# pedrosecchi67/ImmersedBoundary.jl

Measured on AMD Instinct MI355X. Metric: Mcells*iters/s residual sweep (advection-JST-MUSCL), 2D RAE2822, higher is better.
Workload: dtype f32

## Files before the change

### immersedboundary.jl_amd/_lib.py

```python
import ctypes as C
import os

_here = os.path.dirname(os.path.abspath(__file__))
LIB_PATH = os.environ.get("IBHIP_LIB") or os.path.join(_here, "libibhip.so")

c_i32p = C.POINTER(C.c_int32)
c_f32p = C.POINTER(C.c_float)
c_vp = C.c_void_p
c_i64 = C.c_int64
c_int = C.c_int


class IbhError(RuntimeError):
    pass


class ibh_fluid(C.Structure):
    _fields_ = [("R", C.c_float), ("gamma", C.c_float), ("mu_ref", C.c_float), ("Tref", C.c_float),
                ("S", C.c_float), ("nk", C.c_int32), ("k", C.c_float * 4)]


class ibh_flow_bc_spec(C.Structure):
    _fields_ = [("normal_flow", C.c_int32), ("p_inf", C.c_float), ("T_inf", C.c_float), ("u_inf", C.c_float * 3),
                ("transpiration", C.c_float), ("wall_function", C.c_int32), ("wall_params", C.c_float * 8),
                ("n_iter", C.c_int32)]


_SIGS = {
    "ibh_init": [c_int],
    "ibh_set_stream": [c_vp],
    "ibh_sync": [],
    "ibh_version": [],
    "ibh_malloc": [C.POINTER(c_vp), C.c_size_t],
    "ibh_free": [c_vp],
    "ibh_h2d": [c_vp, c_vp, C.c_size_t],
    "ibh_d2h": [c_vp, c_vp, C.c_size_t],
    "ibh_memset": [c_vp, c_int, C.c_size_t],
    "ibh_owned_device_memory": [C.POINTER(c_i64), C.POINTER(c_i64)],
    "ibh_partition_create": [C.POINTER(c_vp), c_int, C.c_int32, c_vp, c_vp, c_vp,
                             C.POINTER(c_vp), C.POINTER(c_vp), C.POINTER(c_vp), C.POINTER(c_vp),
                             C.POINTER(c_vp), C.POINTER(c_vp), C.c_int32, c_vp, c_vp, c_int, c_int],
    "ibh_partition_destroy": [c_vp],
    "ibh_partition_info": [c_vp, C.POINTER(c_i64), c_int],
    "ibh_analyze2_host": [C.POINTER(c_vp), C.c_int32, c_vp, c_vp, C.POINTER(c_vp), C.POINTER(c_vp), C.POINTER(c_vp),
                          C.POINTER(c_vp), C.POINTER(c_vp), C.POINTER(c_vp), C.c_int32, c_vp, c_vp, c_int],
    "ibh_host2d_get": [c_vp, c_int, c_int, c_vp, c_i64, C.POINTER(c_i64)],
    "ibh_host2d_destroy": [c_vp],
    "ibh_at_owners": [c_vp, c_int, c_vp, c_int, c_i64, c_vp, c_i64],
    "ibh_at_neighbors": [c_vp, c_int, c_vp, c_int, c_i64, c_vp, c_i64],
    "ibh_at_faces": [c_vp, c_int, c_vp, c_int, c_i64, c_vp, c_i64],
    "ibh_green_gauss": [c_vp, c_int, c_vp, c_int, c_i64, c_vp, c_i64, c_int],
    "ibh_cell_gradient": [c_vp, c_int, c_vp, c_int, c_i64, c_vp, c_i64],
    "ibh_cell_gradient_all": [c_vp, c_vp, c_int, c_i64, c_vp, c_i64],
    "ibh_cell_gradient_nd": [c_vp, c_vp, c_int, c_i64, c_vp, c_i64, c_vp, c_i64],
    "ibh_cell_gradient_fields": [c_vp, c_vp, c_int, c_i64, c_vp],
    "ibh_face_distance": [c_vp, c_int, c_vp],
    "ibh_owner_distance": [c_vp, c_int, c_vp],
    "ibh_neighbor_distance": [c_vp, c_int, c_vp],
    "ibh_face_gradient": [c_vp, c_int, c_vp, c_int, c_i64, c_vp, c_i64],
    "ibh_jst_sensor": [c_vp, c_int, c_vp, c_int, c_i64, c_vp, c_i64],
    "ibh_muscl": [c_vp, c_int, c_vp, c_vp, c_int, c_i64, c_vp, c_int, c_vp, c_vp, c_i64],
    "ibh_acc_create": [C.POINTER(c_vp), C.c_int32, C.c_int32, c_vp, c_vp, c_vp, c_int],
    "ibh_acc_destroy": [c_vp],
    "ibh_accumulate": [c_vp, c_vp, c_int, c_i64, c_vp, c_i64],
    "ibh_accumulate_diff_add": [c_vp, c_vp, c_vp, c_int, c_i64, c_vp, c_i64],
    "ibh_bc_create": [C.POINTER(c_vp), C.c_int32, c_vp, c_vp, c_vp, C.c_int32, c_vp, c_vp, c_vp, c_vp, c_int],
    "ibh_bc_destroy": [c_vp],
    "ibh_bc_interp": [c_vp, c_vp, c_int, c_i64, c_vp, c_i64],
    "ibh_bc_blend": [c_vp, c_vp, c_int, c_i64, c_vp, c_i64, c_vp, c_i64, c_vp],
    "ibh_bc_apply": [c_vp, c_vp, c_int, c_i64, c_int, c_vp],
    "ibh_bc_flow_info": [c_vp, C.POINTER(C.c_int32)],
    "ibh_bc_flow": [c_vp, C.POINTER(ibh_fluid), c_int, c_vp, c_i64, c_vp, c_vp, c_i64, C.POINTER(ibh_flow_bc_spec), c_int,
                    C.POINTER(c_vp), c_vp, c_vp, c_vp],
    "ibh_gather_rows": [c_vp, C.c_int32, c_vp, c_int, c_i64, c_vp, c_i64],
    "ibh_scatter_rows": [c_vp, C.c_int32, c_vp, c_int, c_i64, c_vp, c_i64],
    "ibh_copy_rows": [c_vp, c_vp, C.c_int32, c_vp, c_int, c_i64, c_vp, c_i64],
    "ibh_residual_advection": [c_vp, c_vp, c_vp, c_i64, c_vp, c_int],
    "ibh_residual_advection_n": [c_vp, c_vp, c_vp, c_i64, c_vp, c_int, c_int],
    "ibh_shear_rate_of_velocity": [c_vp, c_vp, c_i64, c_vp],
    "ibh_shear_rate_of_velocity_grad": [c_vp, c_vp, c_i64, c_vp, c_vp, c_i64],
    "ibh_wray_agarwal_of": [c_vp, c_vp, c_vp, C.c_float, C.c_float, C.c_float, c_vp, c_vp, c_vp],
    "ibh_les_of": [c_vp, c_vp, c_i64, c_vp, c_int, C.c_float, c_vp, c_vp, c_vp, c_vp, c_vp, c_i64],
    "ibh_k_epsilon_rhs": [c_vp, c_vp, c_i64, c_vp, c_vp, C.c_float, c_vp, c_vp, c_vp, c_vp, c_vp, c_vp, c_i64],
    "ibh_scalar_transport": [c_vp, c_vp, c_vp, C.c_float, c_vp, c_i64, c_vp, c_vp],
    "ibh_bcset_create": [C.POINTER(c_vp), c_int, C.POINTER(c_vp), c_vp, c_vp],
    "ibh_bcset_destroy": [c_vp],
    "ibh_bcset_info": [c_vp, C.POINTER(C.c_int32), C.POINTER(C.c_int32)],
    "ibh_bcset_apply": [c_vp, c_vp],
    "ibh_timestep_advection": [c_vp, c_vp, c_i64, C.c_float, c_vp],
    "ibh_update_dev": [c_i64, c_vp, c_vp, c_vp, c_vp],
    "ibh_step_advection": [c_vp, c_vp, c_vp, c_vp, c_i64, c_vp, c_vp],
    "ibh_step_advection_dt": [c_vp, c_vp, c_vp, c_vp, c_i64, c_vp, c_vp, C.c_float, c_vp],
    "ibh_timestep_euler": [c_vp, C.POINTER(ibh_fluid), c_vp, c_i64, C.c_float, c_vp, c_vp],
    "ibh_update_euler": [C.POINTER(ibh_fluid), c_int, c_i64, c_vp, c_i64, c_vp, c_i64, c_vp, c_int, c_vp, c_i64],
    "ibh_step_euler": [c_vp, C.POINTER(ibh_fluid), c_int, c_vp, c_i64, c_vp, c_i64, c_vp, c_int, c_vp, c_i64, c_int],
    "ibh_update_euler_stage": [C.POINTER(ibh_fluid), c_int, c_i64, c_vp, c_i64, c_vp, c_i64, c_vp, c_int, C.c_float, c_vp,
                               c_i64],
    "ibh_stage_euler": [c_vp, C.POINTER(ibh_fluid), c_int, c_vp, c_i64, c_vp, c_i64, c_vp, c_i64, c_vp, c_int, C.c_float,
                        c_vp, c_i64, c_int],
    "ibh_update_euler_ssp": [C.POINTER(ibh_fluid), c_int, c_i64, c_vp, c_i64, c_vp, c_i64, c_vp, c_i64, c_vp, c_int, C.c_float,
                             C.c_float, C.c_float, c_vp, c_i64],
    "ibh_stage_euler_ssp": [c_vp, C.POINTER(ibh_fluid), c_int, c_vp, c_i64, c_vp, c_i64, c_vp, c_i64, c_vp, c_int, C.c_float,
                            C.c_float, C.c_float, c_vp, c_i64, c_int],
    "ibh_dual_source": [C.POINTER(ibh_fluid), c_int, c_i64, c_vp, c_i64, c_vp, c_i64, C.c_float, C.c_float, c_vp, c_i64],
    "ibh_update_euler_dual": [C.POINTER(ibh_fluid), c_int, c_i64, c_vp, c_i64, c_vp, c_i64, c_vp, c_i64, c_vp, c_int, C.c_float,
                              C.c_float, c_vp, c_i64],
    "ibh_stage_euler_dual": [c_vp, C.POINTER(ibh_fluid), c_int, c_vp, c_i64, c_vp, c_i64, c_vp, c_i64, c_vp, c_i64, c_vp, c_int,
                             C.c_float, C.c_float, c_vp, c_i64, c_int],
    "ibh_restrict_euler": [c_vp, C.POINTER(ibh_fluid), c_int, c_vp, c_i64, c_vp, c_i64, c_vp, c_i64, c_vp, c_i64, c_vp, c_i64],
    "ibh_prolong_euler": [c_vp, C.POINTER(ibh_fluid), c_int, c_vp, c_vp, c_i64, c_vp, c_vp, c_i64, c_vp, c_i64],
    "ibh_restrict_euler_roles": [c_vp, C.POINTER(ibh_fluid), c_int, c_vp, c_i64, c_vp, c_i64, c_vp, c_i64, c_vp, c_vp, c_i64,
                                 c_vp, c_i64],
    "ibh_forcing_roles": [c_i64, c_int, c_vp, c_i64, c_vp, c_i64, c_vp],
    "ibh_sumsq_roles": [c_i64, c_int, c_vp, c_i64, c_vp, c_vp],
    "ibh_smooth_residual": [c_vp, c_vp, c_int, c_i64, C.c_float, c_int, c_vp, c_i64, c_vp, c_i64],
    "ibh_update_euler_smoothed": [c_vp, C.POINTER(ibh_fluid), c_int, c_vp, c_i64, c_vp, c_i64, c_vp, c_i64, c_vp, c_i64,
                                  C.c_float, c_vp, c_int, C.c_float, C.c_float, C.c_float, c_vp, c_i64],
    "ibh_ew_binary": [c_int, c_i64, c_int, c_vp, c_int, C.c_float, c_vp, c_int, C.c_float, c_vp],
    "ibh_ew_unary": [c_int, c_i64, c_vp, c_vp],
    "ibh_ew_fill": [c_i64, C.c_float, c_vp],
    "ibh_ew_reduce": [c_int, c_i64, c_vp, c_vp],
    "ibh_ew_eval": [c_i64, c_int, c_int, c_vp, c_int, c_vp, c_vp, c_int, c_vp, c_vp],
    "ibh_ew_reduce_rows": [c_i64, c_int, c_vp, c_vp],
    "ibh_set_tuning": [C.c_char_p, c_int],
    "ibh_debug_buffer": [c_vp],
    "ibh_probe_dispatch": [c_int, c_int, c_int],
    "ibh_probe_sweep": [c_vp, c_vp, c_vp, c_i64, c_vp, c_int],
    "ibh_residual_euler_hll": [c_vp, c_vp, c_i64, c_vp, c_i64, C.POINTER(ibh_fluid), c_int],
    "ibh_residual_euler_sensor": [c_vp, c_vp, c_i64, c_vp, c_vp, c_i64, C.POINTER(ibh_fluid), c_int],
    "ibh_cfd_speed_of_sound": [C.POINTER(ibh_fluid), c_i64, c_vp, c_vp],
    "ibh_cfd_dynamic_viscosity": [C.POINTER(ibh_fluid), c_i64, c_vp, c_vp],
    "ibh_cfd_heat_conductivity": [C.POINTER(ibh_fluid), c_i64, c_vp, c_vp],
    "ibh_cfd_primitive2state": [C.POINTER(ibh_fluid), c_int, c_i64, c_vp, c_i64, c_vp, c_i64],
    "ibh_cfd_state2primitive": [C.POINTER(ibh_fluid), c_int, c_i64, c_vp, c_i64, c_vp, c_i64],
    "ibh_cfd_inviscid_fluxes_hll": [C.POINTER(ibh_fluid), c_int, c_int, c_i64, c_vp, c_vp, c_i64, c_vp, c_i64],
    "ibh_cfd_inviscid_fluxes_sensor": [C.POINTER(ibh_fluid), c_int, c_int, c_i64, c_vp, c_vp, c_i64, c_vp, c_vp,
                                       c_vp, c_i64],
    "ibh_cfd_jst_sensor3": [c_i64, c_vp, c_vp, c_vp, c_vp],
    "ibh_cfd_shock_sensor": [c_int, c_i64, C.POINTER(c_vp), c_vp],
    "ibh_cfd_viscous_fluxes": [C.POINTER(ibh_fluid), c_int, c_int, c_i64, c_vp, c_i64, C.POINTER(c_vp), c_i64, c_vp,
                               C.c_float, c_vp, c_i64],
    "ibh_viscous_residual": [c_vp, C.POINTER(ibh_fluid), c_vp, c_i64, C.POINTER(c_vp), c_i64, c_int, c_vp, c_vp, c_i64],
    "ibh_cfd_flow_bc": [C.POINTER(ibh_fluid), c_int, c_i64, c_vp, c_i64, c_vp, c_i64, C.c_float, C.c_float, c_vp, c_int,
                        c_vp, c_vp, C.c_float, c_vp, c_vp, c_i64],
    "ibh_ipc_alloc": [C.POINTER(c_vp), C.c_size_t, c_int],
    "ibh_ipc_free": [c_vp],
    "ibh_ipc_export": [c_vp, c_vp],
    "ibh_ipc_import": [c_vp, C.POINTER(c_vp)],
    "ibh_ipc_close": [c_vp],
    "ibh_flag_signal": [c_vp, c_vp, c_int],
    "ibh_flag_wait": [c_vp, c_vp, c_int, C.c_uint32, c_vp],
    "ibh_halo_push": [c_vp, c_int, c_i64, c_vp, c_int, c_vp, c_vp, c_vp, c_vp],
    "ibh_halo_pull": [c_vp, c_int, c_i64, c_vp, c_vp, c_int, c_vp, c_vp, c_vp, C.c_uint32],
    "ibh_halo_exchange": [c_vp, c_int, c_i64, c_vp, c_int, c_vp, c_vp, c_vp, c_vp, c_vp, c_vp, c_vp, c_int, c_vp, c_vp,
                          c_vp, C.c_uint32],
    "ibh_step_advection_xgmi": [c_vp, c_vp, c_vp, c_i64, c_vp, c_vp, c_int, c_vp, c_vp, c_vp, c_vp, c_vp, c_vp, c_vp, c_int,
                                c_vp, c_vp, c_vp, C.c_uint32, c_vp],
    "ibh_axpy_clamped": [c_i64, C.c_float, c_vp, c_vp],
    "ibh_axpy_clamped_sumsq": [c_i64, C.c_float, c_vp, c_vp, c_vp],
    "ibh_fas_update": [c_i64, C.c_float, c_vp, c_vp, c_vp, c_vp],
    "ibh_axpy": [c_i64, C.c_float, c_vp, c_vp],
    "ibh_sumsq": [c_i64, c_vp, c_vp],
    "ibh_time_average_push": [c_i64, c_int, c_vp, c_i64, c_vp, c_vp, c_int, c_vp, c_i64, c_i64, C.c_double, C.c_double,
                              c_int],
    "ibh_domain_plan_create": [C.POINTER(c_vp), c_int, C.POINTER(c_vp), c_vp, C.POINTER(c_vp), C.POINTER(c_vp), c_vp,
                               c_i64, c_int],
    "ibh_domain_plan_destroy": [c_vp],
    "ibh_domain_plan_info": [c_vp, C.POINTER(c_i64), c_int],
    "ibh_domain_gather": [c_vp, c_int, C.POINTER(c_vp), c_vp, c_vp, C.POINTER(c_vp)],
    "ibh_domain_scatter": [c_vp, c_int, C.POINTER(c_vp), c_vp, c_vp, C.POINTER(c_vp)],
    "ibh_turb_wall_function_rey": [c_i64, c_vp, c_vp, c_int, c_vp, c_vp, c_vp, c_vp, c_vp],
    "ibh_turb_wall_function": [c_i64, c_vp, c_vp, c_vp, c_vp, c_int, c_vp, c_vp, c_vp, c_vp, c_vp, c_vp],
    "ibh_turb_shear_rate": [c_int, c_i64, c_vp, c_vp],
    "ibh_turb_smagorinsky": [c_i64, c_vp, c_vp, C.c_float, c_vp],
    "ibh_turb_k_epsilon": [c_i64, c_vp, c_vp, c_vp, c_vp, c_vp, c_vp, c_vp, c_vp, c_vp],
    "ibh_turb_wray_agarwal": [c_int, c_i64, c_vp, c_vp, c_vp, c_i64, c_vp, c_i64, C.c_float, C.c_float, C.c_float, c_vp,
                              c_vp, c_vp],
    "ibh_turb_ducros": [c_int, c_i64, c_vp, c_vp],
    "ibh_turb_wale": [c_i64, c_vp, c_vp, C.c_float, c_vp],
    "ibh_pi_rademacher": [c_i64, C.c_uint64, c_vp],
    "ibh_pi_perturb": [c_i64, c_vp, c_vp, C.c_float, c_vp],
    "ibh_pi_fd": [c_i64, c_vp, c_vp, C.c_float, c_vp],
    "ibh_pi_hutch_accum": [c_i64, c_int, c_vp, c_vp, c_vp, C.c_float, c_vp],
    "ibh_pi_div_scalar": [c_i64, C.c_float, c_vp],
    "ibh_pi_invert_blocks": [c_i64, c_int, c_vp],
    "ibh_pi_apply_blocks": [c_i64, c_int, c_vp, c_vp, c_vp],
    "ibh_dot": [c_i64, c_vp, c_vp, c_vp],
    "ibh_maxabs": [c_i64, c_vp, c_vp],
    "ibh_pi_update": [c_i64, c_vp, C.c_float, c_vp, c_vp, c_vp, c_vp],
    "ibh_pi_normalize": [c_i64, c_vp, c_vp, C.c_float, c_vp],
}

EXPORTS = sorted(list(_SIGS) + ["ibh_last_error"])

_lib = None


def load():
    global _lib
    if _lib is not None:
# ... 28 lines not shown
```

### immersedboundary.jl_amd/backend.py

```python
from __future__ import annotations

import ctypes as C

import numpy as np
import torch

from . import _lib
from ._lib import call, c_vp
from .accumulator import Accumulator
from .domain import Boundary, Partition, Surface

IBH_FORCE_GENERAL = 1
IBH_IMAGE_ONLY = 2
IBH_PASS_A_ONLY = 4
IBH_PASS_B_ONLY = 8
IBH_EXACT = 16
IBH_PHASE_INTERIOR = 32
IBH_PHASE_BOUNDARY = 64
IBH_NO_FUSE = 128
IBH_SWEEP_ONLY = 256
IBH_FORCE_MIXED = 512
IBH_NO_QUAD = 1024

_initialised = {}
# ... 37 lines not shown

def colmajor_empty(n, nv=None, dtype=torch.float32):
    dev = _dev()
    if nv is None:
        return torch.empty(n, dtype=dtype, device=dev)
    return torch.empty((nv, n), dtype=dtype, device=dev).T


def hip(a):
    dev = _dev()
    if isinstance(a, torch.Tensor):
        a = a.detach().cpu().numpy()
    a = np.asarray(a)
    if a.dtype == np.float64:
        a = a.astype(np.float32)
    if a.ndim == 1:
        return torch.from_numpy(np.ascontiguousarray(a)).to(dev)
    if a.ndim == 2:
        return torch.from_numpy(np.ascontiguousarray(a.T)).to(dev).T
    raise ValueError("hip(): only 1-D and 2-D fields are supported")


def to_host(t):
    if not isinstance(t, torch.Tensor):
        t = t.t
    return np.ascontiguousarray(t.detach().cpu().numpy())


def _hipaware(fn):
    import functools

    H = {}

    @functools.wraps(fn)
    def wrapper(*args, **kwargs):
        if not H:
            from . import hiparray
            H["A"], H["rewrap"] = hiparray.HipArray, hiparray.rewrap
        HipArray = H["A"]
        hit = False

        def un(x):
            nonlocal hit
            if isinstance(x, HipArray):
                hit = True
                return x.t
            if isinstance(x, tuple):
                return tuple(un(v) for v in x)
            return x
        if kwargs and isinstance(kwargs.get("out"), HipArray):
            kwargs["out"]._flush_readers()
        a = [un(x) for x in args]
        k = {key: un(v) for key, v in kwargs.items()} if kwargs else kwargs
        out = fn(*a, **k)
        return H["rewrap"](out, True) if hit else out
    return wrapper


def _field(t, n=None):
    if not isinstance(t, torch.Tensor) or not t.is_cuda:
        raise TypeError("expected a device array (convert with ibamd.hip); there is no CPU path")
    if t.dtype != torch.float32:
        raise TypeError("fields must be Float32")
    if t.ndim == 1:
        if t.stride(0) != 1:
            t = t.contiguous()
        nv, ld = 1, t.shape[0]
    elif t.ndim == 2:
        if t.stride(0) != 1 or (t.shape[1] > 1 and t.stride(1) < t.shape[0]):
            t = t.T.contiguous().T
        nv, ld = t.shape[1], (t.stride(1) if t.shape[1] > 1 else t.shape[0])
    else:
        raise ValueError("fields are (n,) or (n, nv)")
    if n is not None and t.shape[0] != n:
        raise ValueError(f"field has {t.shape[0]} rows, expected {n}")
    return t, nv, ld


def _field_inplace(t, n=None, what="destination"):
    f, nv, ld = _field(t, n)
    if f.data_ptr() != t.data_ptr() or f.stride() != t.stride():
        raise TypeError(f"{what} must be a column-major Float32 device array (cell index fastest, e.g. ibamd.hip(a) or "
                        f"colmajor_empty(n, nv)); got strides {tuple(t.stride())} for shape {tuple(t.shape)}: it would "
                        "be copied and the update lost")
    return f, nv, ld


def _like(t, n):
    return colmajor_empty(n) if t.ndim == 1 else colmajor_empty(n, t.shape[1])


class _Handle:
    _destroy = None
    handle = None

    def __del__(self):
        try:
            if self.handle:
                h, self.handle = self.handle, None
                getattr(_lib.load(), self._destroy)(h)
        except Exception:
            pass


class DevicePartition(_Handle):
    _destroy = "ibh_partition_destroy"

    def __init__(self, part: Partition):
        dev = _dev()
        self.host = part
        self.id = part.id
        self.nd = part.ndims
        self.nc = part.spacing.shape[0]
        nd, nc = self.nd, self.nc
        spacing = np.asfortranarray(part.spacing, dtype=np.float32)
        centers = np.asfortranarray(part.centers, dtype=np.float32)
        self.nf = [int(part.face_owners_neighbors[d + 1][0].shape[0]) for d in range(nd)]
        nf = np.array(self.nf, dtype=np.int32)
        keep = []

        def parr(arrs):
            arrs = [np.ascontiguousarray(a, dtype=np.int32) for a in arrs]
            keep.append(arrs)
            return (c_vp * nd)(*[a.ctypes.data for a in arrs])

        owners = parr([part.face_owners_neighbors[d + 1][0] for d in range(nd)])
        neighbors = parr([part.face_owners_neighbors[d + 1][1] for d in range(nd)])
        loff = parr([part.face_accumulators[(d + 1, False)].off for d in range(nd)])
        lidx = parr([part.face_accumulators[(d + 1, False)].idx for d in range(nd)])
        roff = parr([part.face_accumulators[(d + 1, True)].off for d in range(nd)])
        ridx = parr([part.face_accumulators[(d + 1, True)].idx for d in range(nd)])
        iid = np.ascontiguousarray(part.image_in_domain, dtype=np.int32)
        dom = np.ascontiguousarray(part.domain, dtype=np.int32)
        h = c_vp()
        call("ibh_partition_create", C.byref(h), nd, nc, spacing.ctypes.data_as(c_vp), centers.ctypes.data_as(c_vp),
             nf.ctypes.data_as(c_vp), owners, neighbors, loff, lidx, roff, ridx, int(iid.size), _hptr(iid),
             _hptr(dom), int(getattr(part, "block_size", 0)), 0)
        self.handle = h
        self.spacing = hip(part.spacing)
        self.centers = hip(part.centers)
        self.domain = torch.from_numpy(dom).to(dev)
        self.image = torch.from_numpy(np.ascontiguousarray(part.image, dtype=np.int32)).to(dev)
        self.image_in_domain = torch.from_numpy(iid).to(dev)
        info = (C.c_int64 * 24)()
        call("ibh_partition_info", h, info, 24)
        self.info = dict(full_blocks=info[0], irregular_cells=info[1], sides_same=info[2], sides_mirror=info[3],
                         sides_coarse=info[4], sides_fine=info[5], sides_general=info[6], interior_blocks=info[7],
                         fusable_blocks=info[8], workspace_blocks=info[9],
                         image_blocks_all_eligible=bool(info[10]), image_blocks=info[11],
                         quads=info[12] if self.nd == 2 else 0, quad_singles=info[13], image_quads=info[14],
                         image_quad_singles=info[15], row_sweep=bool(info[16]), direct_sides=info[17],
                         quad_pairs=info[18] if self.nd == 2 else 0,
                         quad_arith_half_sides=info[19] if self.nd == 2 else 0,
                         tiled=bool(info[20]),
                         rim4_rows=info[12] if self.nd == 3 else 0)

    @property
    def ndims(self):
        return self.nd


class DeviceAccumulator(_Handle):
    _destroy = "ibh_acc_destroy"

    def __init__(self, acc: Accumulator):
        _dev()
        self.n_output, self.n_input = acc.n_output, acc.n_input
        self.first_index = acc.first_index
        h = c_vp()
        w = None if acc.w is None else np.ascontiguousarray(acc.w, dtype=np.float32)
        call("ibh_acc_create", C.byref(h), acc.n_output, acc.n_input, _hptr(acc.off), _hptr(acc.idx),
             _hptr(w) if w is not None else c_vp(None), 0)
        self.handle = h

    def __call__(self, v):
        from .hiparray import HipArray
        if isinstance(v, HipArray):
            return HipArray(self(v.t))
        v, nv, ld = _field(v, self.n_input)
        out = _like(v, self.n_output)
        _stream()
        call("ibh_accumulate", self.handle, _ptr(v), nv, ld, _ptr(out), self.n_output)
        return out

    def diff_add(self, out, a, b):
        a, nv, ld = _field(a, self.n_input)
        b, nvb, ldb = _field(b, self.n_input)
        o, nvo, ldo = _field_inplace(out, self.n_output, "out")
        if nvb != nv or nvo != nv or ldb != ld:
            out += self(a - b)
            return out
        _stream()
        call("ibh_accumulate_diff_add", self.handle, _ptr(a), _ptr(b), nv, ld, _ptr(o), ldo)
        return out


class DeviceBoundary(_Handle):
    _destroy = "ibh_bc_destroy"

    def __init__(self, b: Boundary):
        self.host = b
        self.ng = int(b.ghost_indices.shape[0])
        acc = b.image_interpolator
        h = c_vp()
        gi = np.ascontiguousarray(b.ghost_indices, dtype=np.int32)
        idm = np.ascontiguousarray(b.image_domain, dtype=np.int32)
        gd = np.ascontiguousarray(b.ghost_distances, dtype=np.float32)
        idist = np.ascontiguousarray(b.image_distances, dtype=np.float32)
        _dev()
        call("ibh_bc_create", C.byref(h), self.ng, _hptr(gi), _hptr(gd), _hptr(idist), int(idm.size), _hptr(idm),
             _hptr(acc.off), _hptr(acc.idx), _hptr(np.ascontiguousarray(acc.w, dtype=np.float32)), 0)
        self.handle = h
        self.ghost_indices = torch.from_numpy(gi).to(_dev())
        self.projections = hip(b.projections)
        self.normals = hip(b.normals)
        self.image_distances = hip(b.image_distances)
        self.ghost_distances = hip(b.ghost_distances)


class DeviceSurface:

    def __init__(self, s: Surface):
        self.host = s
        self.n = int(s.points.shape[0])
        self.interpolator = DeviceAccumulator(s.interpolator)
        self.offset_interpolator = DeviceAccumulator(s.offset_interpolator)
        self.points, self.normals = hip(s.points), hip(s.normals)
        self.offsets, self.areas = hip(s.offsets), hip(s.areas)

    def __call__(self, u):
        return self.interpolator(u)


def at_offset(surf, u):
    return to_backend(surf).offset_interpolator(u)


def surface_integral(surf, u):
    from .hiparray import HipArray
    surf = to_backend(surf)
    U = u if isinstance(u, HipArray) else HipArray(u)
    if U.n != surf.n:
        raise ValueError(f"field has {U.n} rows, the surface {surf.n} control points")
    prod = U * HipArray(surf.areas)
    if U.ndim == 1:
        return np.float32(prod.sum())
    return np.array([HipArray(prod.t[:, v]).sum() for v in range(U.nv)], dtype=np.float32)


def volume_integral(dom, A):
    from .hiparray import HipArray
    U = A if isinstance(A, HipArray) else HipArray(A)
    if U.n != len(dom):
        raise ValueError("volume_integral takes a global array (one row per cell of the domain)")
    wd = getattr(dom, "_device_widths", None)
    if wd is None:
        from .mesher import get_cells
        _, widths = get_cells(dom.mesh)
        wd = dom._device_widths = [HipArray(np.ascontiguousarray(widths[d], dtype=np.float32))
                                   for d in range(widths.shape[0])]
    prod = U * wd[0]
    for w in wd[1:]:
        prod *= w
    if U.ndim == 1:
        return np.float32(prod.sum())
    return np.array([HipArray(prod.t[:, v]).sum() for v in range(U.nv)], dtype=np.float32)


def to_backend(x, converter=hip):
    if isinstance(x, (DevicePartition, DeviceAccumulator, DeviceBoundary, DeviceSurface)):
        return x
    if isinstance(x, Surface):
        if getattr(x, "_device", None) is None:
            x._device = DeviceSurface(x)
        return x._device
    if isinstance(x, Partition):
        if getattr(x, "_device", None) is None:
            x._device = DevicePartition(x)
        return x._device
    if isinstance(x, Accumulator):
        if getattr(x, "_device", None) is None:
            x._device = DeviceAccumulator(x)
        return x._device
    if isinstance(x, Boundary):
        if getattr(x, "_device", None) is None:
            x._device = DeviceBoundary(x)
        return x._device
    if isinstance(x, tuple):
        return tuple(to_backend(v, converter) for v in x)
    if isinstance(x, dict):
        return {k: to_backend(v, converter) for k, v in x.items()}
    if isinstance(x, (np.ndarray, torch.Tensor)):
        return converter(x)
    return x


def _part(p):
    if not isinstance(p, DevicePartition):
        raise TypeError("operators run on a device Partition (to_backend(part, hip)); there is no CPU path")
    return p


def _cell_to_face(name, part, u, dim):
    part = _part(part)
    u, nv, ld = _field(u, part.nc)
    out = _like(u, part.nf[dim - 1])
# ... 963 lines not shown
```

### immersedboundary.jl_amd/csrc/ibh_analyze.cpp

```cpp
#include <algorithm>
#include <array>
#include <unordered_map>

#include "ibh_common.h"

namespace {

inline int pos_own(int s, int t) { return s == 0 ? 8 * t : s == 1 ? 7 + 8 * t : s == 2 ? t : t + 56; }
inline int pos_opp(int s, int tt) { return s == 0 ? 7 + 8 * tt : s == 1 ? 8 * tt : s == 2 ? tt + 56 : tt; }
inline int tang_of_pos(int s, int pos) { return s < 2 ? pos / 8 : pos % 8; }
inline bool on_opp_edge(int s, int pos) {
    return s == 0 ? (pos % 8 == 7) : s == 1 ? (pos % 8 == 0) : s == 2 ? (pos / 8 == 7) : (pos / 8 == 0);
}

}

void ibh_analyze_blocks2(const HostPartView& v, std::vector<BlockDesc2>& blocks, std::vector<int32_t>& irr,
                         int64_t* info, const int32_t* image_in_domain, int32_t n_image, int32_t* n_phase1,
                         std::vector<int32_t>& htab, std::vector<int32_t>& etab, std::vector<char>& fus,
                         std::vector<char>& needg, std::vector<int32_t>& dtab) {
    const int32_t nc = v.nc;
    const int NPB = 64;
    const float* hx = v.spacing;
    const float* hy = v.spacing + nc;
// ... 178 lines not shown
            bool ok = a1[b];
            for (int s = 0; s < 4 && ok; ++s) {
                int ty = blocks[b].type[s];
                if (ty == SIDE_MIRROR) continue;
                if (ty == SIDE_GENERAL) { ok = false; break; }
                int nn = ty == SIDE_FINE ? 2 : 1;
                for (int k = 0; k < nn && ok; ++k) {
                    auto it = base2a1.find(blocks[b].nb[s][k]);
                    ok = it != base2a1.end() && it->second;
                }
            }
            b1[b] = ok;
        }
        std::vector<BlockDesc2> ordered;
        std::vector<std::array<int32_t, 64>> hordered;
        ordered.reserve(blocks.size());
        hordered.reserve(blocks.size());
        auto take = [&](size_t b) { ordered.push_back(blocks[b]); hordered.push_back(halos[b]); };
        for (size_t b = 0; b < blocks.size(); ++b) if (b1[b]) take(b);
        n_phase1[1] = (int32_t)ordered.size();
        for (size_t b = 0; b < blocks.size(); ++b) if (a1[b] && !b1[b]) take(b);
        n_phase1[0] = (int32_t)ordered.size();
        for (size_t b = 0; b < blocks.size(); ++b) if (!a1[b]) take(b);
        blocks.swap(ordered);
        halos.swap(hordered);
    }
    htab.resize(blocks.size() * 64);
    for (size_t bi = 0; bi < blocks.size(); ++bi)
        for (int k = 0; k < 64; ++k) htab[bi * 64 + k] = halos[bi][k];
    etab.assign(blocks.size() * 16, 0);
    fus.assign(blocks.size(), 0);
    dtab.clear();
    {
        auto faces_of = [&](int32_t c, int dim, bool right, int32_t* out) -> int {
            const std::vector<int32_t>& off = right ? v.roff[dim] : v.loff[dim];
            const std::vector<int32_t>& idx = right ? v.ridx[dim] : v.lidx[dim];
            const int n = off[c + 1] - off[c];
            if (n < 1 || n > 2) return -1;
            for (int k = 0; k < n; ++k) {
                const int32_t f = idx[off[c] + k];
                const int32_t o = v.owners[dim][f], nn = v.neighbors[dim][f];
                if ((right ? o : nn) != c) return -1;
                out[k] = right ? nn : o;
            }
            return n;
        };
        int64_t nfus = 0;
        for (size_t bi = 0; bi < blocks.size(); ++bi) {
            BlockDesc2& b = blocks[bi];
            b.dt = -1;
            bool ok = true;
            for (int k = 0; k < NPB && ok; ++k) ok = !cell_irr[b.base + k];
            int32_t deep[64];
            bool arithmetic = true;
            for (int s = 0; s < 4; ++s) {
                int32_t* e = &etab[bi * 16 + s * 4];
                e[0] = e[1] = e[2] = e[3] = b.base + pos_own(s, 0);
                for (int k = 0; k < 16; ++k) deep[s * 16 + k] = halos[bi][s * 16 + k];
                if (!ok) continue;
                const int ty = b.type[s];
                if (ty == SIDE_MIRROR) continue;
                if (ty == SIDE_GENERAL) { ok = false; continue; }
                const int d = s / 2, td = 1 - d;
                const bool low = (s % 2) == 0;
                const float* hn = d == 0 ? hx : hy;
                const float* ht = d == 0 ? hy : hx;
                const float rt = b.rt[s];
                const int delta = s == 0 ? -1 : s == 1 ? 1 : s == 2 ? -8 : 8;
                const int step = ty == SIDE_FINE ? 1 : ty == SIDE_COARSE ? 4 : 2;
                const int ncell = 16 / step;
                const int near_expected = ty == SIDE_COARSE ? 2 : 1;
                for (int q = 0; q < ncell && ok; ++q) {
                    const int32_t h = halos[bi][s * 16 + q * step];
                    if (hn[h] != hn[b.base] * rt || ht[h] != ht[b.base] * rt) { ok = false; break; }
                    int32_t cells[2];
                    int n = faces_of(h, d, low, cells);
                    if (n != near_expected) { ok = false; break; }
                    for (int k = 0; k < n; ++k)
                        if (cells[k] < b.base || cells[k] >= b.base + NPB) ok = false;
                    n = faces_of(h, d, !low, cells);
                    if (!ok || n != 1 || cells[0] == h || hn[cells[0]] != hn[h]) { ok = false; break; }
                    for (int k = 0; k < step; ++k) deep[s * 16 + q * step + k] = cells[0];
                    if (cells[0] != h + delta) arithmetic = false;
                    for (int side = 0; side < 2 && ok; ++side) {
                        n = faces_of(h, td, side == 1, cells);
                        if (n < 1) { ok = false; break; }
                        const int qn = q + (side ? 1 : -1);
                        if (qn >= 0 && qn < ncell) {
                            if (n != 1 || cells[0] != halos[bi][s * 16 + qn * step]) ok = false;
                        } else {
                            e[side * 2] = cells[0];
                            e[side * 2 + 1] = n == 2 ? cells[1] : cells[0];
                        }
                    }
                }
            }
            if (ok && !arithmetic) {
                b.dt = (int32_t)(dtab.size() / 64);
                dtab.insert(dtab.end(), deep, deep + 64);
            }
            fus[bi] = ok;
            nfus += ok;
        }
        info[8] = nfus;
    }
    needg.assign(blocks.size(), 0);
    {
        std::vector<char> mark(nc, 0);
        for (int32_t c : irr) {
            mark[c] = 1;
            for (int d = 0; d < v.nd; ++d) {
                for (int32_t k = v.loff[d][c]; k < v.loff[d][c + 1]; ++k) mark[v.owners[d][v.lidx[d][k]]] = 1;
                for (int32_t k = v.roff[d][c]; k < v.roff[d][c + 1]; ++k) mark[v.neighbors[d][v.ridx[d][k]]] = 1;
            }
        }
        for (size_t bi = 0; bi < blocks.size(); ++bi)
            if (!fus[bi])
                for (int k = 0; k < 64; ++k) mark[htab[bi * 64 + k]] = 1;
        for (size_t bi = 0; bi < blocks.size(); ++bi) {
            bool need = !fus[bi];
            for (int k = 0; k < NPB && !need; ++k) need = mark[blocks[bi].base + k];
            needg[bi] = need;
        }
    }
    info[7] = n_phase1[1];
    info[0] = (int64_t)blocks.size();
    info[1] = (int64_t)irr.size();
    for (int k = 0; k < 5; ++k) info[2 + k] = counts[k];
}

static void quad_aux_row(const int32_t* row, uint32_t cls, std::vector<int32_t>& aux) {
    const size_t a0 = aux.size();
    aux.resize(a0 + IBH_QAUX);
    for (int e = 0; e < 32; ++e) aux[a0 + e] = row[128 + e];
    for (int l = 0; l < 8; ++l) {
        const int g = l >> 1, half = l & 1;
        const uint32_t ty = (cls >> (4 * l)) & 15u;
        const int stride = (g == 0 || g == 3) ? 8 : 1;
        const int32_t* ids = row + 2 * (16 * g + 8 * half);
        int32_t orig = -1;
        if (ty == SIDE_SAME || ty == SIDE_COARSE) {
            orig = ids[0];
            for (int t = 0; t < 8 && orig >= 0; ++t) {
                const int32_t want = ids[0] + stride * (ty == SIDE_COARSE ? (t >> 1) : t);
                if (ids[2 * t] != want || ids[2 * t + 1] != want) orig = -1;
            }
        }
        aux[a0 + 32 + l] = orig;
    }
}

void ibh_build_quads2(const std::vector<BlockDesc2>& blocks, const std::vector<int32_t>& htab,
                      const std::vector<int32_t>& etab, const std::vector<char>& cand, int32_t nB1, QuadSet2& out,
                      int32_t nc) {
    out = QuadSet2();
    const int32_t nb = (int32_t)blocks.size();
    std::unordered_map<int32_t, int32_t> bybase;
    bybase.reserve(nb * 2);
    for (int32_t b = 0; b < nb; ++b) bybase[blocks[b].base] = b;
    std::vector<int32_t> order(nb);
    for (int32_t b = 0; b < nb; ++b) order[b] = b;
    std::sort(order.begin(), order.end(), [&](int32_t a, int32_t b) { return blocks[a].base < blocks[b].base; });
    std::vector<char> used(nb, 0);
    struct Q { int32_t b[4]; bool interior; };
    std::vector<Q> quads;
    auto same_to = [&](const BlockDesc2& a, int s, int32_t base) {
        return a.type[s] == SIDE_SAME && a.nb[s][0] == base;
    };
    static const int outer[4][2] = {{0, 2}, {1, 2}, {0, 3}, {1, 3}};
    for (int32_t o : order) {
        if (used[o] || !cand[o]) continue;
        const BlockDesc2& b0 = blocks[o];
        int32_t idx[4] = {o, -1, -1, -1};
        bool ok = true;
        for (int k = 1; k < 4 && ok; ++k) {
            auto it = bybase.find(b0.base + 64 * k);
            ok = it != bybase.end() && !used[it->second] && cand[it->second];
            if (ok) idx[k] = it->second;
        }
        if (!ok) continue;
        const BlockDesc2 &b1 = blocks[idx[1]], &b2 = blocks[idx[2]], &b3 = blocks[idx[3]];
        ok = same_to(b0, 1, b1.base) && same_to(b1, 0, b0.base) && same_to(b0, 3, b2.base) && same_to(b2, 2, b0.base) &&
             same_to(b1, 3, b3.base) && same_to(b3, 2, b1.base) && same_to(b2, 1, b3.base) && same_to(b3, 0, b2.base);
        for (int k = 0; k < 4 && ok; ++k) {
            const BlockDesc2& b = blocks[idx[k]];
            ok = b.dt < 0 && b.h[0] == b0.h[0] && b.h[1] == b0.h[1];
            for (int e = 0; e < 2 && ok; ++e) {
                const int s = outer[k][e];
                const int ty = b.type[s];
                ok = ty == SIDE_SAME || ty == SIDE_COARSE || ty == SIDE_FINE;
                if (ok && s >= 2)
                    for (int t = 0; t < 8 && ok; ++t) {
                        const int32_t h0 = htab[(size_t)idx[k] * 64 + (s * 8 + t) * 2], h1 = htab[(size_t)idx[k] * 64 + (s * 8 + t) * 2 + 1];
                        const int32_t dl = s == 2 ? -8 : 8;
                        ok = h0 + 1 < nc && h0 + dl >= 0 && h0 + dl + 1 < nc && (ty != SIDE_FINE || h1 == h0 + 1);
                    }
            }
        }
        if (!ok) continue;
        Q q;
        q.interior = true;
        for (int k = 0; k < 4; ++k) {
            q.b[k] = idx[k];
            used[idx[k]] = 1;
            q.interior = q.interior && idx[k] < nB1;
        }
        quads.push_back(q);
    }
    static const int side_of_g[4] = {0, 2, 3, 1};
    static const int blk_of[4][2] = {{0, 2}, {0, 1}, {2, 3}, {1, 3}};
    for (int pass = 0; pass < 2; ++pass)
        for (const Q& q : quads) {
            if (q.interior != (pass == 0)) continue;
            QuadDesc2 d;
            d.base = blocks[q.b[0]].base;
            d.rh[0] = blocks[q.b[0]].rh[0];
            d.rh[1] = blocks[q.b[0]].rh[1];
            d.cls = 0;
            const size_t row = out.qtab.size();
            out.qtab.resize(row + IBH_QROW);
            for (int g = 0; g < 4; ++g)
                for (int half = 0; half < 2; ++half) {
                    const int s = side_of_g[g], l = 2 * g + half;
                    const int32_t bi = q.b[blk_of[g][half]];
                    d.cls |= (uint32_t)blocks[bi].type[s] << (4 * l);
                    for (int t = 0; t < 8; ++t)
                        for (int k = 0; k < 2; ++k)
                            out.qtab[row + 2 * (16 * g + 8 * half + t) + k] = htab[(size_t)bi * 64 + (s * 8 + t) * 2 + k];
                    for (int e = 0; e < 4; ++e) out.qtab[row + 128 + 4 * l + e] = etab[(size_t)bi * 16 + s * 4 + e];
                }
            out.qd.push_back(d);
            quad_aux_row(out.qtab.data() + row, d.cls, out.qaux);
            if (pass == 0) out.nq_int++;
        }
    for (int pass = 0; pass < 2; ++pass)
        for (int32_t b = 0; b < nb; ++b)
            if (cand[b] && !used[b] && (b < nB1) == (pass == 0)) {
                out.singles.push_back(b);
                if (pass == 0) out.ns_int++;
            }
    if (nB1 != nb) {
        out.singles2 = out.singles;
        return;
    }
    std::vector<char> paired(nb, 0);
    auto side_ok = [&](int32_t bi, int s) {
        const BlockDesc2& b = blocks[bi];
        const int ty = b.type[s];
        bool ok = ty == SIDE_SAME || ty == SIDE_COARSE || ty == SIDE_FINE;
        if (ok && s >= 2)
            for (int t = 0; t < 8 && ok; ++t) {
                const int32_t h0 = htab[(size_t)bi * 64 + (s * 8 + t) * 2], h1 = htab[(size_t)bi * 64 + (s * 8 + t) * 2 + 1];
                const int32_t dl = s == 2 ? -8 : 8;
                ok = h0 + 1 < nc && h0 + dl >= 0 && h0 + dl + 1 < nc && (ty != SIDE_FINE || h1 == h0 + 1);
            }
        return ok;
    };
    for (int32_t o : order) {
        if (used[o] || paired[o] || !cand[o]) continue;
        const BlockDesc2& b0 = blocks[o];
        auto it = bybase.find(b0.base + 64);
        if (it == bybase.end()) continue;
        const int32_t i1 = it->second;
        if (used[i1] || paired[i1] || !cand[i1]) continue;
        const BlockDesc2& b1 = blocks[i1];
        bool ok = same_to(b0, 1, b1.base) && same_to(b1, 0, b0.base) && b0.dt < 0 && b1.dt < 0 && b1.h[0] == b0.h[0] &&
                  b1.h[1] == b0.h[1];
        ok = ok && side_ok(o, 0) && side_ok(o, 2) && side_ok(o, 3) && side_ok(i1, 1) && side_ok(i1, 2) && side_ok(i1, 3);
        if (!ok) continue;
        paired[o] = paired[i1] = 1;
        const int32_t blk_of_pair[4][2] = {{o, o}, {o, i1}, {o, i1}, {i1, i1}};
        QuadDesc2 d;
        d.base = b0.base;
        d.rh[0] = b0.rh[0];
        d.rh[1] = b0.rh[1];
        d.cls = 0;
        const size_t row = out.ptab.size();
        out.ptab.resize(row + IBH_QROW);
        for (int g = 0; g < 4; ++g)
            for (int half = 0; half < 2; ++half) {
                const int s = side_of_g[g], l = 2 * g + half;
                const int32_t bi = blk_of_pair[g][half];
                d.cls |= (uint32_t)blocks[bi].type[s] << (4 * l);
                for (int t = 0; t < 8; ++t)
                    for (int k = 0; k < 2; ++k)
                        out.ptab[row + 2 * (16 * g + 8 * half + t) + k] = htab[(size_t)bi * 64 + (s * 8 + t) * 2 + k];
                for (int e = 0; e < 4; ++e) out.ptab[row + 128 + 4 * l + e] = etab[(size_t)bi * 16 + s * 4 + e];
            }
        out.pd.push_back(d);
        quad_aux_row(out.ptab.data() + row, d.cls, out.paux);
    }
    for (int32_t b : out.singles)
        if (!paired[b]) out.singles2.push_back(b);
}
```

### immersedboundary.jl_amd/csrc/ibh_api.hip

```cpp
#include <string.h>

#include <memory>

#include "ibh_common.h"

thread_local std::string ibh_err;
thread_local hipStream_t ibh_stream = nullptr;

int ibh_fail(int code, const char* what, const char* file, int line) {
    ibh_err = std::string(what) + " (" + file + ":" + std::to_string(line) + ")";
    return code ? code : -1;
}

static std::vector<int32_t> rebased(const int32_t* p, size_t n, int base) {
    std::vector<int32_t> v(n);
    for (size_t i = 0; i < n; ++i) v[i] = p[i] - base;
    return v;
}

struct Host2D {
    std::vector<BlockDesc2> blocks;
    std::vector<int32_t> irr, htab, etab, dtab, img, fz, ng, nf;
    std::vector<char> fus, needg;
    int32_t nph[2] = {0, 0};
    int32_t n_img_int = 0, img_all_fz = 0, fuse_all = 0, rows_ok = 0, n_fz_int = 0, n_ng_int = 0, n_nf_int = 0;
    int64_t info[12] = {0};
    QuadSet2 quads[2];
};
struct ibh_host2d {
    Host2D H;
};

static void analyze2_host(const HostPartView& v, int32_t n_image, const int32_t* image_in_domain, int index_base,
                          Host2D& H) {
    const int32_t nc = v.nc;
    const bool have_img = n_image > 0 && image_in_domain;
    std::vector<int32_t> none;
    ibh_analyze_blocks2(v, H.blocks, H.irr, H.info, have_img ? image_in_domain : none.data(), have_img ? n_image : 0,
                        H.nph, H.htab, H.etab, H.fus, H.needg, H.dtab);
    const int32_t nb = (int32_t)H.blocks.size();
    H.fuse_all = nb > 0 && H.irr.empty() && H.info[8] == (int64_t)nb;
    std::vector<char> is_imgblk(nb, 0);
    if (have_img) {
        std::vector<char> is_img(nc, 0);
        for (int32_t k = 0; k < n_image; ++k) is_img[image_in_domain[k] - index_base] = 1;
        bool all = true;
        for (int32_t b = 0; b < nb; ++b)
            if (is_img[H.blocks[b].base]) {
                H.img.push_back(b);
                is_imgblk[b] = 1;
                H.n_img_int += b < H.nph[1];
                all = all && H.fus[b];
            }
        H.img_all_fz = all && (int64_t)H.img.size() * 64 == (int64_t)n_image;
        H.info[10] = H.img_all_fz;
        H.info[11] = (int64_t)H.img.size();
    }
    if (!H.fuse_all && H.info[8] > 0)
        for (int32_t b = 0; b < nb; ++b) {
            if (H.fus[b]) { H.fz.push_back(b); H.n_fz_int += b < H.nph[1]; }
            else { H.nf.push_back(b); H.n_nf_int += b < H.nph[1]; }
            if (H.needg[b]) { H.ng.push_back(b); H.n_ng_int += b < H.nph[0]; }
        }
    H.info[9] = H.fuse_all ? 0 : (int64_t)H.ng.size();
    if (H.fuse_all) ibh_build_quads2(H.blocks, H.htab, H.etab, H.fus, H.nph[1], H.quads[0], nc);
    if (H.fuse_all && H.dtab.empty()) {
        bool ok = true;
        for (int32_t b = 0; b < nb && ok; ++b) {
            const BlockDesc2& B = H.blocks[b];
            for (int s = 0; s < 4 && ok; ++s) {
                const int d = s >> 1, sd = d == 0 ? 1 : 8, st = d == 0 ? 8 : 1;
                const bool low = (s & 1) == 0;
                const int opp = low ? 7 * sd : 0, own = low ? 0 : 7 * sd;
                const int ty = B.type[s];
                if (ty == SIDE_GENERAL) { ok = false; break; }
                if (ty != SIDE_MIRROR && (B.nb[s][0] < 0 || (ty == SIDE_FINE && B.nb[s][1] < 0))) { ok = false; break; }
                for (int t = 0; t < 8 && ok; ++t)
                    for (int k = 0; k < 2; ++k) {
                        const int tt = ty == SIDE_COARSE ? (t >> 1) + 4 * B.sub[s] : ty == SIDE_FINE ? 2 * (t & 3) + k : t;
                        const int32_t nbb = (ty == SIDE_FINE && (t >> 2)) ? B.nb[s][1] : B.nb[s][0];
                        const int32_t id = ty == SIDE_MIRROR ? B.base + own + t * st : nbb + opp + tt * st;
                        if (id != H.htab[(size_t)b * 64 + (s * 8 + t) * 2 + k]) { ok = false; break; }
                    }
            }
        }
        H.rows_ok = ok;
    }
    if (H.img_all_fz && !H.fuse_all) ibh_build_quads2(H.blocks, H.htab, H.etab, is_imgblk, H.nph[1], H.quads[1], nc);
}

static int make_view(HostPartView& v, int nd, int32_t nc, const float* spacing, const int32_t* nf,
                     const int32_t* const* owners, const int32_t* const* neighbors, const int32_t* const* left_off,
                     const int32_t* const* left_idx, const int32_t* const* right_off, const int32_t* const* right_idx,
                     const int32_t* domain, int block_size, int index_base) {
    v.nd = nd;
    v.nc = nc;
    v.spacing = spacing;
    v.nf = nf;
    v.domain = domain;
    v.index_base = index_base;
    v.bs = block_size;
    v.owners.resize(nd); v.neighbors.resize(nd);
    v.loff.resize(nd); v.lidx.resize(nd); v.roff.resize(nd); v.ridx.resize(nd);
    for (int d = 0; d < nd; ++d) {
        IBH_REQUIRE(nf[d] >= 0, "ibh_partition_create: negative face count");
        v.owners[d] = rebased(owners[d], nf[d], index_base);
        v.neighbors[d] = rebased(neighbors[d], nf[d], index_base);
        int32_t ob = left_off[d][0];
        v.loff[d] = rebased(left_off[d], (size_t)nc + 1, ob);
        v.lidx[d] = rebased(left_idx[d], v.loff[d][nc], index_base);
        ob = right_off[d][0];
        v.roff[d] = rebased(right_off[d], (size_t)nc + 1, ob);
        v.ridx[d] = rebased(right_idx[d], v.roff[d][nc], index_base);
        for (int32_t f = 0; f < nf[d]; ++f)
            IBH_REQUIRE(v.owners[d][f] >= 0 && v.owners[d][f] < nc && v.neighbors[d][f] >= 0 && v.neighbors[d][f] < nc,
                        "ibh_partition_create: owner/neighbour index out of range");
        for (int32_t c = 0; c < nc; ++c)
            IBH_REQUIRE(v.loff[d][c + 1] >= v.loff[d][c] && v.roff[d][c + 1] >= v.roff[d][c],
                        "ibh_partition_create: CSR offsets not monotone");
        for (int32_t x : v.lidx[d]) IBH_REQUIRE(x >= 0 && x < nf[d], "ibh_partition_create: left face id out of range");
        for (int32_t x : v.ridx[d]) IBH_REQUIRE(x >= 0 && x < nf[d], "ibh_partition_create: right face id out of range");
    }
    return 0;
}

extern "C" {

int ibh_version(void) { return 100; }

const char* ibh_last_error(void) { return ibh_err.c_str(); }

int ibh_init(int device) {
    IBH_HIP(hipSetDevice(device));
    hipDeviceProp_t prop;
    IBH_HIP(hipGetDeviceProperties(&prop, device));
    if (strncmp(prop.gcnArchName, "gfx950", 6) != 0)
        return ibh_fail(-2, (std::string("libibhip is built for gfx950 only, device is ") + prop.gcnArchName).c_str(),
                        __FILE__, __LINE__);
    return 0;
}

int ibh_set_stream(void* s) {
    ibh_stream = (hipStream_t)s;
    return 0;
}

int ibh_sync(void) {
    IBH_HIP(hipStreamSynchronize(ibh_stream));
    return 0;
}

int ibh_malloc(void** p, size_t bytes) {
    IBH_HIP(hipMalloc(p, bytes ? bytes : 4));
    return 0;
}
int ibh_free(void* p) {
    if (p) IBH_HIP(hipFree(p));
    return 0;
}
int ibh_owned_device_memory(int64_t* bytes, int64_t* buffers) {
    if (bytes) *bytes = ibh_owned_bytes;
    if (buffers) *buffers = ibh_owned_buffers;
    return 0;
}
int ibh_h2d(void* dst, const void* src, size_t bytes) {
    IBH_HIP(hipMemcpyAsync(dst, src, bytes, hipMemcpyHostToDevice, ibh_stream));
    IBH_HIP(hipStreamSynchronize(ibh_stream));
    return 0;
}
int ibh_d2h(void* dst, const void* src, size_t bytes) {
    IBH_HIP(hipMemcpyAsync(dst, src, bytes, hipMemcpyDeviceToHost, ibh_stream));
    IBH_HIP(hipStreamSynchronize(ibh_stream));
    return 0;
}
int ibh_memset(void* dst, int value, size_t bytes) {
    IBH_HIP(hipMemsetAsync(dst, value, bytes, ibh_stream));
    return 0;
}


int ibh_partition_create(ibh_part** out, int nd, int32_t nc, const float* spacing, const float* centers,
                         const int32_t* nf, const int32_t* const* owners, const int32_t* const* neighbors,
                         const int32_t* const* left_off, const int32_t* const* left_idx,
                         const int32_t* const* right_off, const int32_t* const* right_idx, int32_t n_image,
                         const int32_t* image_in_domain, const int32_t* domain, int block_size, int index_base) {
    IBH_REQUIRE(out && spacing && nf && owners && neighbors && left_off && left_idx && right_off && right_idx,
                "ibh_partition_create: null argument");
    *out = nullptr;
    IBH_REQUIRE(nd == 2 || nd == 3, "ibh_partition_create: nd must be 2 or 3");
    IBH_REQUIRE(nc >= 0 && (index_base == 0 || index_base == 1), "ibh_partition_create: bad nc/index_base");
    HostPartView v;
    IBH_TRY(make_view(v, nd, nc, spacing, nf, owners, neighbors, left_off, left_idx, right_off, right_idx, domain,
                      block_size, index_base));
    std::unique_ptr<ibh_part> p(new ibh_part());
    p->nd = nd;
    p->nc = nc;
    IBH_TRY(p->own.upload(&p->spacing, spacing, (size_t)nc * nd));
    if (centers) IBH_TRY(p->own.upload(&p->centers, centers, (size_t)nc * nd));
    for (int d = 0; d < nd; ++d) {
        DimData& D = p->dim[d];
        D.nf = nf[d];
        IBH_TRY(p->own.upload(&D.owners, v.owners[d]));
        IBH_TRY(p->own.upload(&D.neighbors, v.neighbors[d]));
        IBH_TRY(p->own.upload(&D.loff, v.loff[d]));
        IBH_TRY(p->own.upload(&D.lidx, v.lidx[d]));
        IBH_TRY(p->own.upload(&D.roff, v.roff[d]));
        IBH_TRY(p->own.upload(&D.ridx, v.ridx[d]));
    }
    {
        std::vector<int32_t> side((size_t)2 * nd * nc);
        int64_t direct = 0;
        for (int d = 0; d < nd; ++d)
            for (int s = 0; s < 2; ++s) {
                const std::vector<int32_t>& off = s ? v.roff[d] : v.loff[d];
                const std::vector<int32_t>& idx = s ? v.ridx[d] : v.lidx[d];
                int32_t* T = side.data() + (size_t)(2 * d + s) * nc;
                for (int32_t c = 0; c < nc; ++c) {
                    const int32_t b = off[c], e = off[c + 1];
                    int32_t t = -1;
                    if (e == b) t = -2;
                    else if (e == b + 1) {
                        const int32_t f = idx[b];
                        const int32_t o = v.owners[d][f], n = v.neighbors[d][f];
                        if (s ? (o == c) : (n == c)) t = s ? n : o;
                    }
                    T[c] = t;
                    direct += t >= 0;
                }
            }
        IBH_TRY(p->own.upload(&p->side, side));
        p->info[17] = direct;
    }
    p->n_image = n_image;
    if (n_image > 0 && image_in_domain) {
        std::vector<int32_t> iid = rebased(image_in_domain, n_image, index_base);
        for (int32_t x : iid) IBH_REQUIRE(x >= 0 && x < nc, "ibh_partition_create: image_in_domain out of range");
        IBH_TRY(p->own.upload(&p->image_in_domain, iid));
    }
    p->bs = 0;
    if (domain && block_size > 0 && nd == 2 && block_size == 8) {
        Host2D H;
        analyze2_host(v, n_image, image_in_domain, index_base, H);
        for (int i = 0; i < 12; ++i) p->info[i] = H.info[i];
        IBH_TRY(p->own.upload(&p->htab, H.htab));
        IBH_TRY(p->own.upload(&p->etab, H.etab));
        IBH_TRY(p->own.upload(&p->dtab, H.dtab));
        p->n_dt = (int32_t)(H.dtab.size() / 64);
        p->fuse_all = H.fuse_all;
        p->rows_ok = H.rows_ok;
        p->info[16] = H.rows_ok;
        p->n_img = (int32_t)H.img.size();
        p->n_img_int = H.n_img_int;
        p->img_all_fz = H.img_all_fz;
        if (p->img_all_fz) IBH_TRY(p->own.upload(&p->img_list, H.img));
        if (!p->fuse_all && H.info[8] > 0) {
            p->n_fz = (int32_t)H.fz.size();
            p->n_ng = (int32_t)H.ng.size();
            p->n_nf = (int32_t)H.nf.size();
            p->n_fz_int = H.n_fz_int;
            p->n_ng_int = H.n_ng_int;
            p->n_nf_int = H.n_nf_int;
            IBH_TRY(p->own.upload(&p->fz_list, H.fz));
            IBH_TRY(p->own.upload(&p->ng_list, H.ng));
            IBH_TRY(p->own.upload(&p->nf_list, H.nf));
        }
        for (int k = 0; k < 2; ++k) {
            const QuadSet2& Q = H.quads[k];
            p->nq[k] = (int32_t)Q.qd.size();
            p->nq_int[k] = Q.nq_int;
            p->nqs[k] = (int32_t)Q.singles.size();
            p->nqs_int[k] = Q.ns_int;
            p->info[12 + 2 * k] = p->nq[k];
            p->info[13 + 2 * k] = p->nqs[k];
            if (k == 0 && !Q.pd.empty()) {
                std::vector<QuadDesc2> qd(Q.qd);
                qd.insert(qd.end(), Q.pd.begin(), Q.pd.end());
                std::vector<int32_t> qt(Q.qtab);
                qt.insert(qt.end(), Q.ptab.begin(), Q.ptab.end());
                p->npair = (int32_t)Q.pd.size();
                p->nqs2 = (int32_t)Q.singles2.size();
                p->info[18] = p->npair;
                IBH_TRY(p->own.upload(&p->qd[k], qd));
                IBH_TRY(p->own.upload(&p->qtab[k], qt));
                IBH_TRY(p->own.upload(&p->qsingles2, Q.singles2));
                std::vector<int32_t> qa(Q.qaux);
                qa.insert(qa.end(), Q.paux.begin(), Q.paux.end());
                IBH_TRY(p->own.upload(&p->qaux[k], qa));
            } else {
                IBH_TRY(p->own.upload(&p->qd[k], Q.qd));
                IBH_TRY(p->own.upload(&p->qtab[k], Q.qtab));
                IBH_TRY(p->own.upload(&p->qaux[k], Q.qaux));
            }
            {
                int64_t arith = 0;
                for (size_t i = 0; i < Q.qaux.size(); i += IBH_QAUX)
                    for (int l = 0; l < 8; ++l) arith += Q.qaux[i + 32 + l] >= 0;
                if (k == 0) p->info[19] = arith;
            }
            IBH_TRY(p->own.upload(&p->qsingles[k], Q.singles));
        }
        p->nA1 = H.nph[0];
        p->nB1 = H.nph[1];
        p->bs = block_size;
        p->nblk = (int32_t)H.blocks.size();
        p->n_irr = (int32_t)H.irr.size();
        {
            bool tiled = !H.blocks.empty() && H.irr.empty() && (int64_t)H.blocks.size() * 64 == (int64_t)nc;
            for (size_t b = 0; tiled && b < H.blocks.size(); ++b) tiled = H.blocks[b].base == (int32_t)(64 * b);
            p->info[20] = tiled ? 1 : 0;
        }
        IBH_TRY(p->own.upload(&p->blocks2, H.blocks));
        IBH_TRY(p->own.upload(&p->irr_cells, H.irr));
    } else if (domain && block_size == 8 && nd == 3) {
        std::vector<BlockDesc3> blocks;
        std::vector<int32_t> irr, htab, ftab;
        int32_t nph[2] = {0, 0};
        std::vector<int32_t> none;
        const bool have_img = n_image > 0 && image_in_domain;
        Sweep3Host sw;
        ibh_analyze_blocks3(v, blocks, irr, p->info, have_img ? image_in_domain : none.data(), have_img ? n_image : 0,
                            nph, htab, ftab, &sw);
        p->sweep3 = sw.all ? 1 : 0;
        p->info[8] = sw.all ? (int64_t)blocks.size() : 0;
        p->info[9] = sw.all ? 0 : (int64_t)blocks.size();
        p->info[12] = (int64_t)(sw.r4tab.size() / 4);
        if (sw.r4tab.empty()) sw.r4tab.assign(4, 0);
        IBH_TRY(p->own.upload(&p->rtab3, sw.rtab));
        IBH_TRY(p->own.upload(&p->r4tab3, sw.r4tab));
        IBH_TRY(p->own.upload(&p->ftab3, ftab));
        p->nA1 = nph[0];
        p->nB1 = nph[1];
        p->bs = block_size;
        p->nblk = (int32_t)blocks.size();
        p->n_irr = (int32_t)irr.size();
        {
            bool tiled = !blocks.empty() && irr.empty() && (int64_t)blocks.size() * 512 == (int64_t)nc;
            for (size_t b = 0; tiled && b < blocks.size(); ++b) tiled = blocks[b].base == (int32_t)(512 * b);
            p->info[20] = tiled ? 1 : 0;
        }
        IBH_TRY(p->own.upload(&p->blocks3, blocks));
        IBH_TRY(p->own.upload(&p->htab3, htab));
        if (have_img && !sw.all) {
            Image3Host im;
            ibh_analyze_image3(v, image_in_domain, n_image, im);
            if (im.all) {
                if (im.r4tab.empty()) im.r4tab.assign(4, 0);
                if (im.ftab.empty()) im.ftab.assign(4, 0);
                IBH_TRY(p->own.upload(&p->iblocks3, im.blocks));
                IBH_TRY(p->own.upload(&p->ihtab3, im.htab));
                IBH_TRY(p->own.upload(&p->iftab3, im.ftab));
                IBH_TRY(p->own.upload(&p->irtab3, im.rtab));
                IBH_TRY(p->own.upload(&p->ir4tab3, im.r4tab));
                IBH_TRY(p->own.upload(&p->idtab3, im.dtab));
                p->n_img3 = (int32_t)im.blocks.size();
                p->img_all3 = 1;
            }
        }
        p->info[10] = p->img_all3 || sw.all;
        p->info[11] = p->img_all3 ? p->n_img3 : (sw.all ? (int64_t)blocks.size() : 0);
        IBH_TRY(p->own.upload(&p->irr_cells, irr));
    } else {
        p->info[0] = 0;
        p->info[1] = nc;
    }
    if (p->n_irr > 0) {
        std::vector<int32_t> irr(p->n_irr);
        IBH_HIP(hipMemcpy(irr.data(), p->irr_cells, sizeof(int32_t) * p->n_irr, hipMemcpyDeviceToHost));
        const size_t n = (size_t)p->n_irr;
        std::vector<int32_t> rec((size_t)nd * 2 * 5 * n, 0);
        bool ok = true;
        for (size_t t = 0; t < n && ok; ++t) {
            const int32_t cc = irr[t];
            for (int d = 0; d < nd && ok; ++d)
                for (int side = 0; side < 2 && ok; ++side) {
                    const std::vector<int32_t>& off = side ? v.roff[d] : v.loff[d];
                    const std::vector<int32_t>& idx = side ? v.ridx[d] : v.lidx[d];
                    const int cnt = off[cc + 1] - off[cc];
                    if (cnt > 4) { ok = false; break; }
                    const size_t q = (size_t)(2 * d + side);
                    rec[(q * 5) * n + t] = cnt;
                    for (int k = 0; k < cnt; ++k) {
                        const int32_t f = idx[off[cc] + k];
                        const int32_t o = v.owners[d][f], nn = v.neighbors[d][f];
                        if ((side ? o : nn) != cc) { ok = false; break; }
                        rec[(q * 5 + 1 + k) * n + t] = side ? nn : o;
                    }
                }
        }
        if (ok) IBH_TRY(p->own.upload(&p->irr_rec, rec));
    }
    *out = p.release();
    return 0;
}

int ibh_analyze2_host(ibh_host2d** out, int32_t nc, const float* spacing, const int32_t* nf,
                      const int32_t* const* owners, const int32_t* const* neighbors, const int32_t* const* left_off,
                      const int32_t* const* left_idx, const int32_t* const* right_off, const int32_t* const* right_idx,
                      int32_t n_image, const int32_t* image_in_domain, const int32_t* domain, int index_base) {
    IBH_REQUIRE(out && spacing && nf && owners && neighbors && left_off && left_idx && right_off && right_idx && domain,
                "ibh_analyze2_host: null argument");
    HostPartView v;
    IBH_TRY(make_view(v, 2, nc, spacing, nf, owners, neighbors, left_off, left_idx, right_off, right_idx, domain, 8,
                      index_base));
    ibh_host2d* h = new ibh_host2d();
    analyze2_host(v, n_image, image_in_domain, index_base, h->H);
    *out = h;
    return 0;
}

int ibh_host2d_get(const ibh_host2d* h, int what, int set, void* dst, int64_t cap_bytes, int64_t* nbytes) {
    IBH_REQUIRE(h && nbytes && (set == 0 || set == 1), "ibh_host2d_get: bad argument");
    const Host2D& H = h->H;
    const QuadSet2& Q = H.quads[set];
    const void* src = nullptr;
    int64_t n = 0;
    int64_t counts[8] = {(int64_t)H.blocks.size(), (int64_t)Q.qd.size(), Q.nq_int, (int64_t)Q.singles.size(), Q.ns_int,
                         H.fuse_all, H.img_all_fz, H.nph[1]};
    switch (what) {
        case IBH_H2D_BLOCKS: src = H.blocks.data(); n = (int64_t)(H.blocks.size() * sizeof(BlockDesc2)); break;
        case IBH_H2D_HTAB: src = H.htab.data(); n = (int64_t)(H.htab.size() * 4); break;
        case IBH_H2D_ETAB: src = H.etab.data(); n = (int64_t)(H.etab.size() * 4); break;
        case IBH_H2D_FUSABLE: src = H.fus.data(); n = (int64_t)H.fus.size(); break;
        case IBH_H2D_QUAD_DESC: src = Q.qd.data(); n = (int64_t)(Q.qd.size() * sizeof(QuadDesc2)); break;
        case IBH_H2D_QUAD_TAB: src = Q.qtab.data(); n = (int64_t)(Q.qtab.size() * 4); break;
        case IBH_H2D_SINGLES: src = Q.singles.data(); n = (int64_t)(Q.singles.size() * 4); break;
        case IBH_H2D_PAIR_DESC: src = Q.pd.data(); n = (int64_t)(Q.pd.size() * sizeof(QuadDesc2)); break;
        case IBH_H2D_PAIR_TAB: src = Q.ptab.data(); n = (int64_t)(Q.ptab.size() * 4); break;
        case IBH_H2D_SINGLES2: src = Q.singles2.data(); n = (int64_t)(Q.singles2.size() * 4); break;
        case IBH_H2D_QUAD_AUX: src = Q.qaux.data(); n = (int64_t)(Q.qaux.size() * 4); break;
        case IBH_H2D_PAIR_AUX: src = Q.paux.data(); n = (int64_t)(Q.paux.size() * 4); break;
        case IBH_H2D_COUNTS: src = counts; n = (int64_t)sizeof(counts); break;
        case IBH_H2D_INFO: src = H.info; n = (int64_t)sizeof(H.info); break;
        default: return ibh_fail(-1, "ibh_host2d_get: unknown item", __FILE__, __LINE__);
    }
    *nbytes = n;
    if (dst) {
        IBH_REQUIRE(cap_bytes >= n, "ibh_host2d_get: destination too small");
        if (n) memcpy(dst, src, (size_t)n);
    }
    return 0;
}

int ibh_host2d_destroy(ibh_host2d* h) {
    delete h;
    return 0;
}

int ibh_partition_destroy(ibh_part* p) {
    delete p;
    return 0;
}

int ibh_partition_info(const ibh_part* p, int64_t* info, int n) {
    IBH_REQUIRE(p && info, "ibh_partition_info: null argument");
    for (int i = 0; i < n && i < 24; ++i) info[i] = p->info[i];
    return 0;
}

static int acc_fill(ibh_acc* a, int32_t n_output, int32_t n_input, const int32_t* off, const int32_t* idx,
                    const float* w, int index_base) {
    IBH_REQUIRE(off && (n_output >= 0), "ibh_acc_create: null offsets");
    int32_t ob = off[0];
    std::vector<int32_t> o = rebased(off, (size_t)n_output + 1, ob);
    for (int32_t r = 0; r < n_output; ++r) IBH_REQUIRE(o[r + 1] >= o[r], "ibh_acc_create: offsets not monotone");
    size_t nnz = o[n_output];
    IBH_REQUIRE(nnz == 0 || idx, "ibh_acc_create: null indices");
    std::vector<int32_t> ix = rebased(idx, nnz, index_base);
    for (int32_t x : ix) IBH_REQUIRE(x >= 0 && x < n_input, "ibh_acc_create: donor index out of range");
    a->n_out = n_output;
    a->n_in = n_input;
    IBH_TRY(a->own.upload(&a->off, o));
    IBH_TRY(a->own.upload(&a->idx, ix));
    if (w) IBH_TRY(a->own.upload(&a->w, w, nnz));
    return 0;
}

int ibh_acc_create(ibh_acc** out, int32_t n_output, int32_t n_input, const int32_t* off, const int32_t* idx,
                   const float* w, int index_base) {
    IBH_REQUIRE(out, "ibh_acc_create: null out");
    *out = nullptr;
    std::unique_ptr<ibh_acc> a(new ibh_acc());
    IBH_TRY(acc_fill(a.get(), n_output, n_input, off, idx, w, index_base));
    *out = a.release();
    return 0;
}

int ibh_acc_destroy(ibh_acc* a) {
    delete a;
    return 0;
}

int ibh_bc_create(ibh_bc** out, int32_t ng, const int32_t* ghost_indices, const float* ghost_distances,
                  const float* image_distances, int32_t nid, const int32_t* image_domain,
                  const int32_t* interp_off, const int32_t* interp_idx, const float* interp_w, int index_base) {
    IBH_REQUIRE(out && ghost_indices && ghost_distances && image_distances && image_domain,
                "ibh_bc_create: null argument");
    *out = nullptr;
    std::unique_ptr<ibh_bc> b(new ibh_bc());
    b->ng = ng;
    b->nid = nid;
    std::vector<int32_t> g = rebased(ghost_indices, ng, index_base);
    std::vector<int32_t> idm = rebased(image_domain, nid, index_base);
    std::vector<float> eta(ng);
    for (int32_t i = 0; i < ng; ++i) eta[i] = ghost_distances[i] / image_distances[i];
    IBH_TRY(b->own.upload(&b->ghost, g));
    IBH_TRY(b->own.upload(&b->image_domain, idm));
    IBH_TRY(b->own.upload(&b->eta, eta));
    IBH_TRY(acc_fill(&b->interp, ng, nid, interp_off, interp_idx, interp_w, index_base));
    b->h_ghost = g;
    b->h_eta = eta;
    if (ng > 0 && interp_off && interp_idx) {
        const int32_t ob = interp_off[0];
        b->h_off.resize((size_t)ng + 1);
        for (int32_t i = 0; i <= ng; ++i) b->h_off[i] = interp_off[i] - ob;
        const size_t nnz = (size_t)b->h_off[ng];
        b->h_donor.resize(nnz);
        b->h_w.resize(nnz);
        for (size_t k = 0; k < nnz; ++k) {
            const int32_t j = interp_idx[k] - index_base;
            IBH_REQUIRE(j >= 0 && j < nid, "ibh_bc_create: stencil index out of range");
            b->h_donor[k] = idm[j];
            b->h_w[k] = interp_w ? interp_w[k] : 1.0f;
        }
    }
    *out = b.release();
    return 0;
}

int ibh_bc_destroy(ibh_bc* b) {
    delete b;
    return 0;
}

}
```

### immersedboundary.jl_amd/csrc/ibh_common.h

```cpp
#pragma once
#include <hip/hip_runtime.h>
#include <stdint.h>
#include <string>
#include <type_traits>
#include <vector>

#include "../../include/ibhip.h"
#include "ibh_owner.h"

#define IBH_MAXD 3

enum : int32_t { SIDE_SAME = 0, SIDE_MIRROR = 1, SIDE_COARSE = 2, SIDE_FINE = 3, SIDE_GENERAL = 4 };

struct BlockDesc2 {
    int32_t base;
    int32_t type[4];
    int32_t nb[4][2];
    int32_t sub[4];
    float h[2];
    float rh[2];
    float q[4];
    float rt[4];
    int32_t dt;
};

struct QuadDesc2 {
    int32_t base;
    uint32_t cls;
    float rh[2];
};
#define IBH_QROW 160
#define IBH_QAUX 40
struct QuadSet2 {
    std::vector<QuadDesc2> qd;
    std::vector<int32_t> qtab;
    std::vector<int32_t> qaux, paux;
    std::vector<int32_t> singles;
    int32_t nq_int = 0, ns_int = 0;
    std::vector<QuadDesc2> pd;
    std::vector<int32_t> ptab;
    std::vector<int32_t> singles2;
};

struct BlockDesc3 {
    int32_t base;
    int32_t fine;
    int32_t type[6];
    int32_t nb[6];
    int32_t sub[6];
    float h[3];
    float rh[3];
    float q[6];
    float rt[6];
};

struct DimData {
    int32_t nf = 0;
    int32_t *owners = nullptr, *neighbors = nullptr;
    int32_t *loff = nullptr, *lidx = nullptr;
    int32_t *roff = nullptr, *ridx = nullptr;
};
static_assert(std::is_trivially_copyable<DimData>::value, "DimData is passed to kernels by value");

struct ibh_part {
    int nd = 0;
    int32_t nc = 0;
    float* spacing = nullptr;
    float* centers = nullptr;
    DimData dim[IBH_MAXD];
    int32_t* side = nullptr;
    int32_t n_image = 0;
    int32_t* image_in_domain = nullptr;
    int bs = 0;
    int32_t nblk = 0;
    int32_t nA1 = 0, nB1 = 0;
    BlockDesc2* blocks2 = nullptr;
    int32_t* htab = nullptr;
    int32_t* etab = nullptr;
    int32_t* dtab = nullptr;
    int32_t n_dt = 0;
    int32_t* img_list = nullptr;
    int32_t n_img = 0, n_img_int = 0, img_all_fz = 0;
    int32_t fuse_all = 0;
    int32_t rows_ok = 0;
    QuadDesc2* qd[2] = {nullptr, nullptr};
    int32_t* qtab[2] = {nullptr, nullptr};
    int32_t* qaux[2] = {nullptr, nullptr};
    int32_t* qsingles[2] = {nullptr, nullptr};
    int32_t nq[2] = {0, 0}, nq_int[2] = {0, 0}, nqs[2] = {0, 0}, nqs_int[2] = {0, 0};
    int32_t npair = 0, nqs2 = 0;
    int32_t* qsingles2 = nullptr;
    int32_t* fz_list = nullptr;
    int32_t* ng_list = nullptr;
    int32_t* nf_list = nullptr;
    int32_t n_fz = 0, n_fz_int = 0, n_ng = 0, n_ng_int = 0, n_nf = 0, n_nf_int = 0;
    BlockDesc3* blocks3 = nullptr;
    int32_t* htab3 = nullptr;
    int32_t* ftab3 = nullptr;
    int32_t *rtab3 = nullptr, *r4tab3 = nullptr;
    int32_t sweep3 = 0;
    BlockDesc3* iblocks3 = nullptr;
    int32_t *ihtab3 = nullptr, *iftab3 = nullptr, *irtab3 = nullptr, *ir4tab3 = nullptr, *idtab3 = nullptr;
    int32_t n_img3 = 0, img_all3 = 0;
    int32_t n_irr = 0;
    int32_t* irr_cells = nullptr;
    int32_t* irr_rec = nullptr;
    int64_t info[24] = {0};
    float* G = nullptr;
    float* march_tmp = nullptr;
    size_t march_tmp_n = 0;
    size_t G_bytes = 0;
    ibh_owner own;
};

struct ibh_acc {
    int32_t n_out = 0, n_in = 0;
    int32_t *off = nullptr, *idx = nullptr;
    float* w = nullptr;
    float* packed = nullptr;
    ibh_owner own;
};

struct ibh_bc {
    int32_t ng = 0, nid = 0;
    int32_t *ghost = nullptr, *image_domain = nullptr;
    float* eta = nullptr;
    ibh_acc interp;
    std::vector<int32_t> h_ghost, h_off, h_donor;
    std::vector<float> h_eta, h_w;
    mutable int flow_direct = -1;
    ibh_owner own;
};

#define IBH_MAX_BC 8
struct ibh_bcset {
    int nbc = 0, nlev = 0;
    int32_t ng = 0;
    int32_t seg[IBH_MAX_BC + 1] = {0};
    bool direct[IBH_MAX_BC] = {false};
    int32_t *ghost = nullptr, *off = nullptr, *donor = nullptr, *bidx = nullptr;
    float *eta = nullptr, *w = nullptr, *gval = nullptr, *value = nullptr;
    int32_t* mode = nullptr;
    ibh_owner own;
};

extern "C" int ibh_bcset_apply_with_dt(const ibh_bcset* s, float* a, ibh_part* p, const float* C, int64_t ldc, float scale,
                                       float* dt_next, int partials_done);

extern "C" {
extern int ibh_viscous_per_cell;
extern int ibh_ew_scalar_only;
extern int ibh_time_average_nt;
}

enum EulerScheme : int { EULER_HLL = 0, EULER_SENSOR = 1 };

extern thread_local std::string ibh_err;
extern thread_local hipStream_t ibh_stream;

int ibh_fail(int code, const char* what, const char* file, int line);

#define IBH_HIP(call)                                                        \
    do {                                                                     \
        hipError_t e__ = (call);                                             \
        if (e__ != hipSuccess) return ibh_fail((int)e__, hipGetErrorString(e__), __FILE__, __LINE__); \
    } while (0)
#define IBH_REQUIRE(cond, msg)                                               \
    do {                                                                     \
        if (!(cond)) return ibh_fail(-1, msg, __FILE__, __LINE__);           \
    } while (0)
#define IBH_LAUNCH_CHECK() IBH_HIP(hipGetLastError())
#define IBH_TRY(call)                                                        \
    do {                                                                     \
        if (const int rc__ = (call)) return rc__;                            \
    } while (0)

struct HostPartView {
    int nd;
    int32_t nc;
    const float* spacing;
    const int32_t* nf;
    std::vector<std::vector<int32_t>> owners, neighbors, loff, lidx, roff, ridx;
    const int32_t* domain;
    int index_base;
    int bs;
};
void ibh_analyze_blocks2(const HostPartView& v, std::vector<BlockDesc2>& blocks,
                         std::vector<int32_t>& irr_cells, int64_t* info, const int32_t* image_in_domain,
                         int32_t n_image, int32_t* n_phase1, std::vector<int32_t>& htab,
                         std::vector<int32_t>& etab, std::vector<char>& fusable, std::vector<char>& needg,
                         std::vector<int32_t>& dtab);

void ibh_build_quads2(const std::vector<BlockDesc2>& blocks, const std::vector<int32_t>& htab,
                      const std::vector<int32_t>& etab, const std::vector<char>& cand, int32_t nB1, QuadSet2& out,
                      int32_t nc);

struct Sweep3Host {
    bool all = false;
    std::vector<int32_t> rtab;
    std::vector<int32_t> r4tab;
};
struct Image3Host {
    bool all = false;
    std::vector<BlockDesc3> blocks;
    std::vector<int32_t> htab, ftab, rtab, r4tab;
    std::vector<int32_t> dtab;
};
void ibh_analyze_image3(const HostPartView& v, const int32_t* image_in_domain, int32_t n_image, Image3Host& out);
void ibh_analyze_blocks3(const HostPartView& v, std::vector<BlockDesc3>& blocks, std::vector<int32_t>& irr_cells,
                         int64_t* info, const int32_t* image_in_domain, int32_t n_image, int32_t* n_phase1,
                         std::vector<int32_t>& htab, std::vector<int32_t>& ftab, Sweep3Host* sw);

static inline int ibh_grid(int64_t n, int block) {
    int64_t g = (n + block - 1) / block;
    if (g < 1) g = 1;
    if (g > 65535 * 16) g = 65535 * 16;
    return (int)g;
}
static inline int ibh_grid_cap(int64_t n, int block, int cap) {
    const int g = ibh_grid(n, block);
    return g > cap ? cap : g;
}

enum ibh_red_region {
    IBH_RED_FAS, IBH_RED_SUMSQ, IBH_RED_DOT, IBH_RED_MAXABS, IBH_RED_EW, IBH_RED_SUMSQ_ROLES, IBH_RED_REGIONS
};
#define IBH_RED_BYTES (2048 * sizeof(double))
#define IBH_SUMSQ_ROLES_MAX_NV 8
void* ibh_red_scratch(ibh_red_region region);
void ibh_launch_sum_partials(int n, const double* part, double* out, int ncols = 1);

#ifdef __HIPCC__
__device__ __forceinline__ int32_t ibh_xcd_chunk(int32_t wg, int32_t nwg) {
    const int32_t q = nwg >> 3, r = nwg & 7, xcd = wg & 7, idx = wg >> 3;
    return (xcd < r ? xcd * (q + 1) : r * (q + 1) + (xcd - r) * q) + idx;
}
__device__ __forceinline__ int32_t xcd_remap(int32_t wg, int32_t nwg) {
#ifdef IBH_NO_XCD_REMAP
    return wg;
#else
    return ibh_xcd_chunk(wg, nwg);
#endif
}
#ifdef IBH_NO_XCD_CELLS
#define IBH_WG_X() ((int64_t)blockIdx.x)
#else
#define IBH_WG_X() ((int64_t)ibh_xcd_chunk((int32_t)blockIdx.x, (int32_t)gridDim.x))
#endif

__device__ __forceinline__ float ibh_max(float a, float b) { return (a != a || b != b) ? a + b : fmaxf(a, b); }
__device__ __forceinline__ float ibh_min(float a, float b) { return (a != a || b != b) ? a + b : fminf(a, b); }
__device__ __forceinline__ float ibh_clamp(float x, float lo, float hi) { return ibh_min(ibh_max(x, lo), hi); }
#endif
```

### immersedboundary.jl_amd/csrc/ibh_fused.hip

```cpp
#include <float.h>
#include <string.h>

#include "ibh_common.h"
#include "ibh_fused_int.h"

using namespace fused;

Tuning fused::T;

static AdvPath advection_path(const ibh_part* p, int flags) {
    if (tuned3(p, flags)) return image3(p, flags) ? ADV3_IMAGE_COLS : single3(p, flags) ? ADV3_SINGLE : ADV3_BLOCKS;
    if (fused2(p, flags)) {
        if ((flags & IBH_IMAGE_ONLY) && p->img_all_fz && !p->fuse_all) return ADV2_IMAGE;
        if (p->fuse_all) return ADV2_FUSE_ALL;
        const bool mixed_pays = p->n_fz >= 12000 || (flags & (IBH_FORCE_MIXED | IBH_SWEEP_ONLY));
        if (p->fz_list && 4 * (int64_t)p->n_fz >= p->nblk && mixed_pays) return ADV2_MIXED;
    }
    return p->nd != 2 ? ADV_GENERAL_3D : (flags & IBH_EXACT) ? ADV_GENERAL_2D_EXACT : ADV_GENERAL_2D;
}

static EulerPath euler_path(const ibh_part* p, int flags, const EulerArgs& e) {
    const bool sensor = e.scheme == EULER_SENSOR;
    if (!(sensor && e.nu)) {
        if (fused2(p, flags) && (p->fuse_all || ((flags & IBH_IMAGE_ONLY) && p->img_all_fz))) return EUL2_SINGLE;
        if (image3(p, flags)) return EUL3_IMAGE_COLS;
        if (single3(p, flags)) return EUL3_SINGLE;
    }
    if (sensor) return p->nd == 2 ? EUL2_FACE_LIST : EUL3_FACE_LIST;
    if (p->nd == 2) return tuned2(p, flags) ? EUL2_FAST : EUL2_FACE_LIST;
    return tuned3(p, flags) ? EUL3_BLOCKS : EUL3_FACE_LIST;
}

extern "C" {

int ibh_debug_buffer(void* buf) {
    unsigned long long* b = (unsigned long long*)buf;
    const int rc = debug_buffer2d(b);
    return rc ? rc : debug_buffer3d(b);
}

int ibh_set_tuning(const char* key, int value) {
    static const struct { const char* key; int* value; } keys[] = {
        {"viscous_per_cell", &ibh_viscous_per_cell}, {"ew_scalar", &ibh_ew_scalar_only},
        {"time_average_nt", &ibh_time_average_nt},
        {"quad_variant", &T.quad_variant}, {"quad_parts", &T.quad_parts}, {"quad_singles_first", &T.quad_singles_first},
        {"quad_singles_iters", &T.quad_singles_iters}, {"rows", &T.rows}, {"rows_singles", &T.rows_singles},
        {"transport_blocks", &T.transport_blocks}, {"pairs", &T.pairs}, {"arith_ids", &T.arith_ids}};
    IBH_REQUIRE(key, "ibh_set_tuning: null key");
    for (const auto& k : keys)
        if (!strcmp(key, k.key)) {
            IBH_REQUIRE(k.value != &T.quad_variant || quad_variant_known(value),
                        "ibh_set_tuning: quad_variant takes 0, 4 (wave time stamps) or 512 (thread per cell)");
            *k.value = value;
            return 0;
        }
    return ibh_fail(-1, "ibh_set_tuning: unknown key", __FILE__, __LINE__);
}

int ibh_residual_advection(ibh_part* p, const float* u, const float* C, int64_t ldc, float* ud, int flags) {
    IBH_REQUIRE(p && u && C && ud, "ibh_residual_advection: null argument");
    if (p->nc == 0) return 0;
    const Phase ph(flags);
    IBH_REQUIRE(ph.valid(), IBH_PHASES_EXCLUSIVE);
    const AdvArgs a{u, C, ldc, ud};
    const AdvPath path = advection_path(p, flags);
    int rc = 0;
    switch (path) {
    case ADV3_IMAGE_COLS: adv3_image_cols(p, a); break;
    case ADV3_SINGLE: adv3_single(p, a); break;
    case ADV3_BLOCKS: rc = adv3_blocks(p, a, flags, ph); break;
    case ADV2_IMAGE: adv2_single(p, a, flags, ph, 1); break;
    case ADV2_FUSE_ALL: adv2_single(p, a, flags, ph, 0); break;
    case ADV2_MIXED: rc = adv2_mixed(p, a, flags, ph); break;
    default: rc = adv_general(p, a, flags, ph, path);
    }
    if (!rc) IBH_LAUNCH_CHECK();
    return rc;
}

int ibh_residual_advection_n(ibh_part* p, const float* u, const float* C, int64_t ldc, float* ud, int flags, int n) {
    int rc = 0;
    for (int i = 0; i < n && !rc; ++i) rc = ibh_residual_advection(p, u, C, ldc, ud, flags);
    return rc;
}

static int residual_euler(ibh_part* p, const EulerArgs& e, int flags, const char* phase_msg) {
    if (p->nc == 0) return 0;
    const Phase ph(flags);
    const EulerPath path = euler_path(p, flags, e);
    if (path == EUL2_SINGLE) IBH_REQUIRE(ph.valid(), IBH_PHASES_EXCLUSIVE);
    else
        IBH_REQUIRE(!ph.any(), phase_msg);
    IBH_REQUIRE(!(e.scheme == EULER_SENSOR && path == EUL3_SINGLE && T.quad_variant != 0),
                "ibh_residual_euler_sensor: quad_variant 4 (wave time stamps) and 512 (thread per cell) are forms of the "
                "HLL sweep only; set quad_variant 0");
    int rc = 0;
    switch (path) {
    case EUL2_SINGLE: euler2_single(p, e, flags, ph); break;
    case EUL3_IMAGE_COLS: euler3_image_cols(p, e); break;
    case EUL3_SINGLE: euler3_single(p, e); break;
    case EUL3_BLOCKS: rc = euler3_blocks(p, e, flags); break;
    default: rc = euler_general(p, e, flags, path);
    }
    if (!rc) IBH_LAUNCH_CHECK();
    return rc;
}

int ibh_residual_euler_hll(ibh_part* p, const float* P, int64_t ldp, float* R, int64_t ldr, const ibh_fluid* fluid,
                           int flags) {
    IBH_REQUIRE(p && P && R && fluid, "ibh_residual_euler_hll: null argument");
    return residual_euler(p, EulerArgs{P, ldp, R, ldr, fluid}, flags,
                          "ibh_residual_euler_hll: overlap phases need a partition whose (image) blocks are all "
                          "eligible for the single-kernel sweep; run the sweep unphased after the exchange");
}

int ibh_residual_euler_sensor(ibh_part* p, const float* P, int64_t ldp, const float* nu, float* R, int64_t ldr,
                              const ibh_fluid* fluid, int flags) {
    IBH_REQUIRE(p && P && R && fluid, "ibh_residual_euler_sensor: null argument");
    return residual_euler(p, EulerArgs{P, ldp, R, ldr, fluid, EULER_SENSOR, nu}, flags,
                          "ibh_residual_euler_sensor: overlap phases need a partition whose (image) blocks are all "
                          "eligible for the single-kernel sweep; run the sweep unphased after the exchange");
}

static int euler_form(const char* name, ibh_part* p, int scheme, EulerArgs e, int dt_per_cell, float* work, int64_t ldw,
                      int flags) {
    const bool step = e.form == FORM_STEP, dual = e.form == FORM_DUAL;
    const char* const update = step ? "ibh_update_euler" : e.form == FORM_STAGE ? "ibh_update_euler_stage"
                               : dual ? "ibh_update_euler_dual" : "ibh_update_euler_ssp";
#define FORM_REQUIRE(cond, ...) IBH_REQUIRE(cond, (std::string(name) + __VA_ARGS__).c_str())
    FORM_REQUIRE(p && e.fluid && e.P && e.P0 && e.R && e.dt && (!dual || e.S), ": null argument");
    FORM_REQUIRE(scheme == EULER_HLL || scheme == EULER_SENSOR, ": scheme must be 0 (HLL) or 1 (sensor)");
    FORM_REQUIRE(!(flags & IBH_IMAGE_ONLY), ": IBH_IMAGE_ONLY is not taken: the update would read skirt rows that the sweep never "
                                            "wrote (the multi-GPU step is out of scope)");
    FORM_REQUIRE(!(flags & F_PHASES), ": the overlap phases IBH_PHASE_INTERIOR / IBH_PHASE_BOUNDARY are not taken: the update "
                                      "would read rows that the phase never wrote");
    FORM_REQUIRE(!(flags & (IBH_PASS_A_ONLY | IBH_PASS_B_ONLY)), ": a single pass of the sweep is no " + (step ? "step" : "stage"));
    FORM_REQUIRE(p->nd == 2 || p->nd == 3, ": nd must be 2 or 3");
    FORM_REQUIRE(e.ldp >= p->nc && e.ld0 >= p->nc && e.ldr >= p->nc, ": a leading dimension is smaller than the number of cells");
    FORM_REQUIRE(!work || (work != e.P && work != e.P0 && work != e.R && work != e.S),
                 ": work may not alias " + (step ? "P or P_out" : dual ? "P, P0, S or P_out" : "P, P0 or P_out"));
    if (dual) {
        FORM_REQUIRE(e.lds >= p->nc, ": lds is smaller than the number of cells");
        FORM_REQUIRE(e.g >= 0.0f && e.g <= FLT_MAX, ": g must be finite and >= 0");
        FORM_REQUIRE(e.S != e.R, ": S may not alias P_out");
    }
    if (p->nc == 0) return 0;
    e.scheme = scheme == EULER_SENSOR ? EULER_SENSOR : EULER_HLL;
    e.dt_cells = dt_per_cell != 0;
    if (euler_path(p, flags, e) == EUL2_SINGLE && p->fuse_all && !(step && e.dt_cells) && e.R != e.P) {
        euler2_single(p, e, flags, Phase(0));
        IBH_LAUNCH_CHECK();
        return 0;
    }
    FORM_REQUIRE(work, ": this partition / these arguments take the two-launch form (sweep into `work`, then " + update +
                           "): work must be nc x (nd + 2) floats");
    FORM_REQUIRE(ldw >= p->nc, ": ldw is smaller than the number of cells");
#undef FORM_REQUIRE
    const int rc = scheme == EULER_SENSOR ? ibh_residual_euler_sensor(p, e.P, e.ldp, nullptr, work, ldw, e.fluid, flags)
                                          : ibh_residual_euler_hll(p, e.P, e.ldp, work, ldw, e.fluid, flags);
    if (rc) return rc;
    if (step) return ibh_update_euler(e.fluid, p->nd, p->nc, e.P, e.ldp, work, ldw, e.dt, dt_per_cell, e.R, e.ldr);
    if (e.form == FORM_STAGE)
        return ibh_update_euler_stage(e.fluid, p->nd, p->nc, e.P0, e.ld0, work, ldw, e.dt, dt_per_cell, e.c, e.R, e.ldr);
    if (dual)
        return ibh_update_euler_dual(e.fluid, p->nd, p->nc, e.P0, e.ld0, work, ldw, e.S, e.lds, e.dt, dt_per_cell, e.c, e.g, e.R,
                                     e.ldr);
    return ibh_update_euler_ssp(e.fluid, p->nd, p->nc, e.P0, e.ld0, e.P, e.ldp, work, ldw, e.dt, dt_per_cell, e.a, e.b, e.c, e.R,
                                e.ldr);
}

int ibh_step_euler(ibh_part* p, const ibh_fluid* fluid, int scheme, const float* P, int64_t ldp, float* P_out, int64_t ldo,
                   const float* dt, int dt_per_cell, float* work, int64_t ldw, int flags) {
    EulerArgs e{P, ldp, P_out, ldo, fluid};
    e.form = FORM_STEP, e.dt = dt;
    e.P0 = P, e.ld0 = ldp;
    return euler_form("ibh_step_euler", p, scheme, e, dt_per_cell, work, ldw, flags);
}

int ibh_stage_euler(ibh_part* p, const ibh_fluid* fluid, int scheme, const float* P, int64_t ldp, const float* P0, int64_t ld0,
                    float* P_out, int64_t ldo, const float* dt, int dt_per_cell, float alpha, float* work, int64_t ldw,
                    int flags) {
    EulerArgs e{P, ldp, P_out, ldo, fluid};
    e.form = FORM_STAGE, e.dt = dt;
    e.P0 = P0, e.ld0 = ld0, e.c = alpha;
    return euler_form("ibh_stage_euler", p, scheme, e, dt_per_cell, work, ldw, flags);
}

int ibh_stage_euler_ssp(ibh_part* p, const ibh_fluid* fluid, int scheme, const float* P, int64_t ldp, const float* P0,
                        int64_t ld0, float* P_out, int64_t ldo, const float* dt, int dt_per_cell, float a, float b, float c,
                        float* work, int64_t ldw, int flags) {
    EulerArgs e{P, ldp, P_out, ldo, fluid};
    e.form = FORM_SSP, e.dt = dt;
    e.P0 = P0, e.ld0 = ld0, e.c = c, e.a = a, e.b = b;
    return euler_form("ibh_stage_euler_ssp", p, scheme, e, dt_per_cell, work, ldw, flags);
}

int ibh_stage_euler_dual(ibh_part* p, const ibh_fluid* fluid, int scheme, const float* P, int64_t ldp, const float* P0,
                         int64_t ld0, const float* S, int64_t lds, float* P_out, int64_t ldo, const float* dt, int dt_per_cell,
                         float alpha, float g, float* work, int64_t ldw, int flags) {
    EulerArgs e{P, ldp, P_out, ldo, fluid};
// ... 80 lines not shown
```

### immersedboundary.jl_amd/csrc/ibh_fused2d.hip

```cpp
#include <algorithm>

#include <string.h>

#include "ibh_block2d.h"
#include "ibh_sweep2d.h"
#include "ibh_quad2d.h"
#include "ibh_quad2d_euler.h"
#include "ibh_rows2d.h"
#include "ibh_halo_dev.h"
#include "ibh_fused_int.h"

using namespace fused;

namespace {

#ifndef IBH_SWEEP_WAVES
#define IBH_SWEEP_WAVES 5
#endif
template <bool DT>
__global__ __launch_bounds__(64 * WPB) __attribute__((amdgpu_waves_per_eu(IBH_SWEEP_WAVES, IBH_SWEEP_WAVES))) void k_sweep_adv(const float* __restrict__ u, const float* __restrict__ C,
                                                        uint32_t ldc, float* __restrict__ ud,
                                                        const BlockDesc2* __restrict__ blocks,
                                                        const int32_t* __restrict__ htab,
                                                        const int32_t* __restrict__ etab,
                                                        const int32_t* __restrict__ dtab, int32_t nblk, int32_t nwg,
                                                        int32_t iters, const int32_t* __restrict__ blist) {
    __shared__ float lds[WPB * BLK2_SWEEP_LDS];
    const int wave = __builtin_amdgcn_readfirstlane(threadIdx.x >> 6), lane = threadIdx.x & 63;
    const int32_t first = __builtin_amdgcn_readfirstlane(xcd_remap(blockIdx.x, nwg) * (WPB * iters) + wave);
    if (first >= nblk) return;
    const int32_t nb = __builtin_amdgcn_readfirstlane(min(iters, (nblk - first + WPB - 1) / WPB));
    blk2::sweep_adv<DT>(blocks, htab, etab, dtab, blist, first, WPB, nb, u, C, ldc, ud, lds + wave * BLK2_SWEEP_LDS, lane);
}

#define QUAD_WG_LDS (WPB * (QUAD_LDS > BLK2_SWEEP_LDS ? QUAD_LDS : BLK2_SWEEP_LDS))
__device__ unsigned long long* ibh_dbg_buf = nullptr;
__device__ __forceinline__ void dbg_stamp(int32_t slot, int k, unsigned long long v) {
    if (ibh_dbg_buf && threadIdx.x % 64 == 0) ibh_dbg_buf[(size_t)slot * 8 + k] = v;
}

template <bool DT, bool STAMP, bool STEP = false, bool RS = false>
#ifndef QS_WAVES
#define QS_WAVES 5
#endif
__global__ __launch_bounds__(64 * WPB) __attribute__((amdgpu_waves_per_eu(QS_WAVES, QS_WAVES))) void k_sweep_quad(const float* __restrict__ u, const float* __restrict__ C,
                                                         uint32_t ldc, float* __restrict__ ud,
                                                         const QuadDesc2* __restrict__ qd,
                                                         const int32_t* __restrict__ qtab, int32_t nq, int32_t nwgq,
                                                         const BlockDesc2* __restrict__ blocks,
                                                         const int32_t* __restrict__ htab,
                                                         const int32_t* __restrict__ etab,
                                                         const int32_t* __restrict__ dtab,
                                                         const int32_t* __restrict__ singles, int32_t ns, int32_t nwgs,
                                                         int32_t singles_first, int32_t siters,
                                                         const float* __restrict__ dtp = nullptr, int32_t npair = 0,
                                                         const int32_t* __restrict__ qaux = nullptr) {
    __shared__ __attribute__((aligned(16))) float lds[RS && WPB * ROWS_LDS > QUAD_WG_LDS ? WPB * ROWS_LDS : QUAD_WG_LDS];
    float dt = 0.0f;
    if constexpr (STEP) dt = *dtp;
    const int wave = __builtin_amdgcn_readfirstlane(threadIdx.x >> 6), lane = threadIdx.x & 63;
    const int32_t slot = blockIdx.x * WPB + wave;
    if constexpr (STAMP) {
        dbg_stamp(slot, 0, __builtin_amdgcn_s_memrealtime());
        dbg_stamp(slot, 2, __builtin_amdgcn_s_getreg((4 << 0) | (0 << 6) | (31 << 11)));
    }
    const int32_t wgq = singles_first ? (int32_t)blockIdx.x - nwgs : (int32_t)blockIdx.x;
    const bool isq = wgq >= 0 && wgq < nwgq;
    if (isq) {
        const int32_t q = __builtin_amdgcn_readfirstlane(xcd_remap(wgq, nwgq) * WPB + wave);
        if (q < nq)
            quad2::sweep_quad<STAMP, STEP>(qd, qtab, q, u, C, ldc, ud, lds + wave * QUAD_LDS, lane,
                                           STAMP && ibh_dbg_buf ? ibh_dbg_buf + (size_t)slot * 8 : nullptr, dt, qaux);
        else if (q < nq + npair)
            quad2::sweep_quad<STAMP, STEP, true>(qd, qtab, q, u, C, ldc, ud, lds + wave * QUAD_LDS, lane,
                                                 STAMP && ibh_dbg_buf ? ibh_dbg_buf + (size_t)slot * 8 : nullptr, dt, qaux);
    } else {
        const int32_t wgs = singles_first ? (int32_t)blockIdx.x : (int32_t)blockIdx.x - nwgq;
        if constexpr (RS) {
            const int32_t first8 = __builtin_amdgcn_readfirstlane((xcd_remap(wgs, nwgs) * WPB + wave) * 8);
            if (first8 < ns) {
                __builtin_amdgcn_s_setprio(3);
                rows2::sweep_rows(blocks, etab, first8, ns, u, C, ldc, ud, lds + wave * ROWS_LDS, lane, singles);
            }
            return;
        }
        const int32_t first = __builtin_amdgcn_readfirstlane(xcd_remap(wgs, nwgs) * (WPB * siters) + wave);
        if (first < ns) {
            const int32_t nb = __builtin_amdgcn_readfirstlane(min(siters, (ns - first + WPB - 1) / WPB));
            blk2::sweep_adv<DT, STEP>(blocks, htab, etab, dtab, singles, first, WPB, nb, u, C, ldc, ud,
                                      lds + wave * BLK2_SWEEP_LDS, lane, dt);
        }
    }
    if constexpr (STAMP) {
        __builtin_amdgcn_s_waitcnt(0);
        dbg_stamp(slot, 1, __builtin_amdgcn_s_memrealtime());
        dbg_stamp(slot, 3, (unsigned long long)isq);
    }
}

#ifndef WPBR
#define WPBR 4
#endif
__global__ __launch_bounds__(64 * WPBR) void k_sweep_rows(const float* __restrict__ u, const float* __restrict__ C,
                                                          uint32_t ldc, float* __restrict__ ud,
                                                          const BlockDesc2* __restrict__ blocks,
                                                          const int32_t* __restrict__ etab, int32_t b0, int32_t n,
                                                          int32_t nwg, const int32_t* __restrict__ list) {
    __shared__ __attribute__((aligned(16))) float lds[WPBR * ROWS_LDS];
    const int wave = __builtin_amdgcn_readfirstlane(threadIdx.x >> 6), lane = threadIdx.x & 63;
    const int32_t first = __builtin_amdgcn_readfirstlane((xcd_remap(blockIdx.x, nwg) * WPBR + wave) * 8);
    if (first < n)
        rows2::sweep_rows(blocks + b0, etab + (size_t)b0 * 16, first, n, u, C, ldc, ud, lds + wave * ROWS_LDS, lane, list);
}

template <bool DT>
__global__ __launch_bounds__(64 * WPB) void k_step_quad(float* __restrict__ u, const float* __restrict__ C, uint32_t ldc,
                                                        float* __restrict__ ud, const QuadDesc2* __restrict__ qd,
                                                        const int32_t* __restrict__ qtab, int32_t nq_int, int32_t nq,
                                                        const BlockDesc2* __restrict__ blocks,
                                                        const int32_t* __restrict__ htab,
                                                        const int32_t* __restrict__ etab,
                                                        const int32_t* __restrict__ dtab,
                                                        const int32_t* __restrict__ singles, int32_t ns_int, int32_t ns,
                                                        const int32_t* __restrict__ send_all,
                                                        const int32_t* __restrict__ recv_all,
                                                        const float* __restrict__ src0, const float* __restrict__ src1,
                                                        XchgArgs A, uint32_t* __restrict__ state, uint32_t max_spins,
                                                        int32_t E, unsigned long long* __restrict__ fstate) {
    __shared__ __attribute__((aligned(16))) float lds[QUAD_WG_LDS];
    const int32_t b0 = (int32_t)blockIdx.x;
    if (b0 < E) {
        halo_exchange_wg(u, 1, 0, send_all, recv_all, src0, src1, A, state, max_spins, b0, E);
        __threadfence();
        __syncthreads();
        if (threadIdx.x == 0) atomicAdd(&fstate[1], 1ull);
        return;
    }
    const int wave = __builtin_amdgcn_readfirstlane(threadIdx.x >> 6), lane = threadIdx.x & 63;
    const int32_t nwg_qi = (nq_int + WPB - 1) / WPB, nwg_si = (ns_int + WPB - 1) / WPB;
    const int32_t nwg_qb = (nq - nq_int + WPB - 1) / WPB, nwg_sb = (ns - ns_int + WPB - 1) / WPB;
    int32_t b = b0 - E;
    const bool boundary = b >= nwg_qi + nwg_si;
    if (boundary) {
        __shared__ unsigned long long want;
        if (threadIdx.x == 0) {
            const unsigned long long t = atomicAdd(&fstate[0], 1ull);
            want = (t / (unsigned long long)(nwg_qb + nwg_sb) + 1ull) * (unsigned long long)E;
        }
        __syncthreads();
        if (lane == 0) {
            const unsigned long long w = want;
            unsigned long long spins = 0;
            const unsigned long long bound = 4ull * (unsigned long long)max_spins;
            while (__hip_atomic_load(&fstate[1], __ATOMIC_RELAXED, __HIP_MEMORY_SCOPE_AGENT) < w) {
                if (++spins >= bound) {
                    atomicOr(&state[2], 2u);
                    break;
                }
                __builtin_amdgcn_s_sleep(4);
            }
        }
        __threadfence();
        b -= nwg_qi + nwg_si;
    }
    const int32_t nwq = boundary ? nwg_qb : nwg_qi, q0 = boundary ? nq_int : 0, q1 = boundary ? nq : nq_int;
    const int32_t nws = boundary ? nwg_sb : nwg_si, s0 = boundary ? ns_int : 0, s1 = boundary ? ns : ns_int;
    if (b < nwq) {
        const int32_t q = __builtin_amdgcn_readfirstlane(q0 + xcd_remap(b, nwq) * WPB + wave);
        if (q < q1) quad2::sweep_quad<false>(qd, qtab, q, u, C, ldc, ud, lds + wave * QUAD_LDS, lane);
    } else {
        const int32_t first = __builtin_amdgcn_readfirstlane(s0 + xcd_remap(b - nwq, nws) * WPB + wave);
        if (first < s1)
            blk2::sweep_adv<DT>(blocks, htab, etab, dtab, singles, first, WPB, 1, u, C, ldc, ud,
                                lds + wave * BLK2_SWEEP_LDS, lane);
    }
}

#ifndef WPBE
#define WPBE 4
#endif
template <int SCH = EULER_HLL, int FORM = FORM_RESIDUAL, bool DTC = false>
__global__ __launch_bounds__(64 * WPBE) void k_sweep_euler(const float* __restrict__ P, uint32_t ldp,
                                                           float* __restrict__ R, uint32_t ldr, float Rgas, float gamma,
                                                           const BlockDesc2* __restrict__ blocks,
                                                           const int32_t* __restrict__ htab,
                                                           const int32_t* __restrict__ etab,
                                                           const int32_t* __restrict__ dtab, int32_t nblk, int32_t nwg,
                                                           int32_t iters, const int32_t* __restrict__ blist,
                                                           const float* __restrict__ dtp = nullptr,
                                                           const float* P0 = nullptr, uint32_t ld0 = 0, float c = 1.0f,
                                                           float sa = 0.0f, float sb = 1.0f, const float* Sd = nullptr,
                                                           uint32_t ldsd = 0, float g = 0.0f) {
    __shared__ float lds[WPBE * BLK2_SWEEP_EULER_LDS];
    float dt = 0.0f;
    if constexpr (FORM != FORM_RESIDUAL && !DTC) dt = *dtp;
    const int wave = __builtin_amdgcn_readfirstlane(threadIdx.x >> 6), lane = threadIdx.x & 63;
    const int32_t first = __builtin_amdgcn_readfirstlane(xcd_remap(blockIdx.x, nwg) * (WPBE * iters) + wave);
    if (first >= nblk) return;
    const int32_t nb = __builtin_amdgcn_readfirstlane(min(iters, (nblk - first + WPBE - 1) / WPBE));
    blk2::sweep_euler<SCH, FORM, DTC>(blocks, htab, etab, dtab, blist, first, WPBE, nb, P, ldp, R, ldr, blk2::Gas{Rgas, gamma},
                                      lds + wave * BLK2_SWEEP_EULER_LDS, lane, dt,
                                      euler_step::FormArgs{P0, ld0, c, dtp, sa, sb, Sd, ldsd, g});
}

#define QUADE_WG_LDS (WPBE * (QE_LDS > BLK2_SWEEP_EULER_LDS ? QE_LDS : BLK2_SWEEP_EULER_LDS))
#ifndef QE_WAVES
#define QE_WAVES 3
#endif
template <int SCH = EULER_HLL, int FORM = FORM_RESIDUAL, bool DTC = false>
__global__ __launch_bounds__(64 * WPBE) __attribute__((amdgpu_waves_per_eu(QE_WAVES, QE_WAVES))) void k_sweep_quad_euler(const float* __restrict__ P, uint32_t ldp,
                                                                float* __restrict__ R, uint32_t ldr, float Rgas,
                                                                float gamma, const QuadDesc2* __restrict__ qd,
                                                                const int32_t* __restrict__ qtab, int32_t nq,
                                                                int32_t nwgq, const BlockDesc2* __restrict__ blocks,
                                                                const int32_t* __restrict__ htab,
                                                                const int32_t* __restrict__ etab,
                                                                const int32_t* __restrict__ dtab,
                                                                const int32_t* __restrict__ singles, int32_t ns,
                                                                int32_t nwgs, int32_t singles_first,
                                                                const float* __restrict__ dtp = nullptr,
                                                                const float* P0 = nullptr, uint32_t ld0 = 0,
                                                                float c = 1.0f, float sa = 0.0f,
                                                                float sb = 1.0f, const float* Sd = nullptr,
                                                                uint32_t ldsd = 0, float g = 0.0f) {
    __shared__ __attribute__((aligned(16))) float lds[QUADE_WG_LDS];
    float dt = 0.0f;
    if constexpr (FORM != FORM_RESIDUAL && !DTC) dt = *dtp;
    const euler_step::FormArgs fa{P0, ld0, c, dtp, sa, sb, Sd, ldsd, g};
    const int wave = __builtin_amdgcn_readfirstlane(threadIdx.x >> 6), lane = threadIdx.x & 63;
    const int32_t wg = singles_first ? ((int32_t)blockIdx.x < nwgs ? (int32_t)blockIdx.x + nwgq : (int32_t)blockIdx.x - nwgs)
                                     : (int32_t)blockIdx.x;
    if (wg < nwgq) {
        const int32_t q = __builtin_amdgcn_readfirstlane(xcd_remap(wg, nwgq) * WPBE + wave);
        if (q < nq)
            quad2::sweep_quad_euler<SCH, FORM, DTC>(qd, qtab, q, P, ldp, R, ldr, blk2::Gas{Rgas, gamma}, lds + wave * QE_LDS, lane,
                                                    dt, fa);
    } else {
        const int32_t first = __builtin_amdgcn_readfirstlane(xcd_remap(wg - nwgq, nwgs) * WPBE + wave);
#ifndef IBH_QE_NO_SINGLES
        if (first < ns)
            blk2::sweep_euler<SCH, FORM, DTC>(blocks, htab, etab, dtab, singles, first, WPBE, 1, P, ldp, R, ldr, blk2::Gas{Rgas, gamma},
                                              lds + wave * BLK2_SWEEP_EULER_LDS, lane, dt, fa);
#endif
    }
}


#define IBH_ROWS_SINGLES_MIN 24000

struct QuadRange { Range q, s; };
QuadRange quad_range(const ibh_part* p, int k, Phase ph) {
    QuadRange r{ph.of(p->nq_int[k], p->nq[k]), ph.of(p->nqs_int[k], p->nqs[k])};
    if (T.quad_parts == 1) r.s.last = r.s.first;
    if (T.quad_parts == 2) r.q.last = r.q.first;
    return r;
}

struct BlockList { const BlockDesc2* bl; const int32_t *ht, *et, *ls; int32_t count, iters, nwg; };
BlockList block_list(const ibh_part* p, const int32_t* list, Range r, int wpb, int max_iters) {
    const int32_t count = r.count(), iters = T.sweep_iters > 0 ? T.sweep_iters : std::min(max_iters, std::max(1, count / 6000));
    return {list ? p->blocks2 : p->blocks2 + r.first, list ? p->htab : p->htab + (size_t)r.first * 64,
            list ? p->etab : p->etab + (size_t)r.first * 16, list ? list + r.first : nullptr, count, iters,
            (count + wpb * iters - 1) / (wpb * iters)};
}

#define EULER_FORM_OF(K, S, e)                                                            \
    ((e).form == FORM_DUAL    ? ((e).dt_cells ? K<S, FORM_DUAL, true> : K<S, FORM_DUAL>)   \
     : (e).form == FORM_SSP   ? ((e).dt_cells ? K<S, FORM_SSP, true> : K<S, FORM_SSP>)     \
     : (e).form == FORM_STAGE ? ((e).dt_cells ? K<S, FORM_STAGE, true> : K<S, FORM_STAGE>) \
     : (e).form == FORM_STEP  ? K<S, FORM_STEP>                                            \
                              : K<S>)
#define EULER_KERNEL(K, e) ((e).scheme == EULER_SENSOR ? EULER_FORM_OF(K, EULER_SENSOR, e) : EULER_FORM_OF(K, EULER_HLL, e))
}

namespace fused {

void adv2_block_list(const ibh_part* p, const AdvArgs& a, const int32_t* list, Range r) {
    if (r.count() <= 0) return;
    const BlockList L = block_list(p, list, r, WPB, 6);
    hipLaunchKernelGGL(p->n_dt > 0 ? k_sweep_adv<true> : k_sweep_adv<false>, dim3(L.nwg), dim3(64 * WPB), 0, ibh_stream, a.u,
                       a.C, (uint32_t)a.ldc, a.ud, L.bl, L.ht, L.et, p->dtab, L.count, L.nwg, L.iters, L.ls);
}

static void adv2_quads(const ibh_part* p, const AdvArgs& a, int k, Phase ph) {
    const Range q = quad_range(p, k, ph).q;
    Range s = quad_range(p, k, ph).s;
    const int32_t npair = (k == 0 && T.pairs && p->npair > 0 && !ph.boundary && q.first == 0 && q.last == p->nq[k] &&
                           T.quad_parts == 3) ? p->npair : 0;
    const int32_t* slist = p->qsingles[k];
    if (npair) {
        slist = p->qsingles2;
        s = {0, p->nqs2};
    } else if (k == 0 && p->npair > 0 && ph.boundary) {
        s.last = s.first;
    }
    const bool rows_able = k == 0 && p->rows_ok && p->n_dt == 0 && T.quad_variant == 0 && s.count() > 0;
    const bool rows_inside = rows_able && T.rows_singles == 2;
    const bool rows_second = rows_able && !rows_inside &&
                             (T.rows_singles < 0 ? s.count() >= IBH_ROWS_SINGLES_MIN : T.rows_singles > 0);
    const Range rs = s;
    if (rows_second) s.last = s.first;
    const int32_t siters = T.quad_singles_iters > 0 ? T.quad_singles_iters : 1;
    const int32_t nwgq = (q.count() + npair + WPB - 1) / WPB,
                  nwgs = rows_inside ? (s.count() + WPB * 8 - 1) / (WPB * 8) : (s.count() + WPB * siters - 1) / (WPB * siters);
    auto kq = k_sweep_quad<false, false>;
    if (rows_inside) kq = k_sweep_quad<false, false, false, true>;
    else if (p->n_dt > 0) kq = k_sweep_quad<true, false>;
    else if (T.quad_variant == QV_STAMPS) kq = k_sweep_quad<false, true>;
    if (nwgq + nwgs > 0)
        hipLaunchKernelGGL(kq, dim3(nwgq + nwgs), dim3(64 * WPB), 0, ibh_stream, a.u, a.C, (uint32_t)a.ldc, a.ud,
                           p->qd[k] + q.first, p->qtab[k] + (size_t)q.first * IBH_QROW, q.count(), nwgq, p->blocks2, p->htab,
                           p->etab, p->dtab, slist + s.first, s.count(), nwgs, T.quad_singles_first, siters,
                           (const float*)nullptr, npair,
                           T.arith_ids ? p->qaux[k] + (size_t)q.first * IBH_QAUX : (const int32_t*)nullptr);
    if (rows_second) {
        const int32_t nw = (rs.count() + 7) / 8, nwgr = (nw + WPBR - 1) / WPBR;
        hipLaunchKernelGGL(k_sweep_rows, dim3(nwgr), dim3(64 * WPBR), 0, ibh_stream, a.u, a.C, (uint32_t)a.ldc, a.ud,
                           p->blocks2, p->etab, 0, rs.count(), nwgr, slist + rs.first);
    }
}

void adv2_single(const ibh_part* p, const AdvArgs& a, int flags, Phase ph, int k) {
    const Range b = k ? ph.of(p->n_img_int, p->n_img) : ph.of(p->nB1, p->nblk);
    if (k == 0 && p->rows_ok && T.rows && !(flags & IBH_NO_QUAD) && T.quad_variant == 0) {
        const int32_t nw = (b.count() + 7) / 8, nwg = (nw + WPBR - 1) / WPBR;
        if (nwg > 0)
            hipLaunchKernelGGL(k_sweep_rows, dim3(nwg), dim3(64 * WPBR), 0, ibh_stream, a.u, a.C, (uint32_t)a.ldc, a.ud,
                               p->blocks2, p->etab, b.first, b.count(), nwg, (const int32_t*)nullptr);
    } else if (quads_usable(p, k, flags)) adv2_quads(p, a, k, ph);
    else adv2_block_list(p, a, k ? p->img_list : nullptr, b);
}

void euler2_single(const ibh_part* p, const EulerArgs& e, int flags, Phase ph) {
    const int k = p->fuse_all ? 0 : 1;
    if (quads_usable(p, k, flags)) {
        const QuadRange r = quad_range(p, k, ph);
        const int32_t nwgq = (r.q.count() + WPBE - 1) / WPBE, nwgs = (r.s.count() + WPBE - 1) / WPBE;
        if (nwgq + nwgs > 0)
            hipLaunchKernelGGL(EULER_KERNEL(k_sweep_quad_euler, e), dim3(nwgq + nwgs), dim3(64 * WPBE), 0, ibh_stream, e.P,
                               (uint32_t)e.ldp, e.R, (uint32_t)e.ldr, e.fluid->R, e.fluid->gamma, p->qd[k] + r.q.first,
                               p->qtab[k] + (size_t)r.q.first * IBH_QROW, r.q.count(), nwgq, p->blocks2, p->htab, p->etab,
                               p->dtab, p->qsingles[k] + r.s.first, r.s.count(), nwgs, T.quad_singles_first, e.dt, e.P0,
                               (uint32_t)e.ld0, e.c, e.a, e.b, e.S, (uint32_t)e.lds, e.g);
        return;
    }
    const Range b = p->fuse_all ? ph.of(p->nB1, p->nblk) : ph.of(p->n_img_int, p->n_img);
    if (b.count() <= 0) return;
    const BlockList L = block_list(p, p->fuse_all ? nullptr : p->img_list, b, WPBE, 4);
    hipLaunchKernelGGL(EULER_KERNEL(k_sweep_euler, e), dim3(L.nwg), dim3(64 * WPBE), 0, ibh_stream, e.P, (uint32_t)e.ldp, e.R,
                       (uint32_t)e.ldr, e.fluid->R, e.fluid->gamma, L.bl, L.ht, L.et, p->dtab, L.count, L.nwg, L.iters, L.ls, e.dt,
                       e.P0, (uint32_t)e.ld0, e.c, e.a, e.b, e.S, (uint32_t)e.lds, e.g);
}

void adv2_step_quads(const ibh_part* p, const float* u, float* u_out, const float* C, int64_t ldc, const float* dt_dev) {
    const int32_t npair = T.pairs ? p->npair : 0;
    const int32_t nq = p->nq[0], ns = npair ? p->nqs2 : p->nqs[0];
    const int32_t nwgq = (nq + npair + WPB - 1) / WPB, nwgs = (ns + WPB - 1) / WPB;
    hipLaunchKernelGGL((k_sweep_quad<false, false, true>), dim3(nwgq + nwgs), dim3(64 * WPB), 0, ibh_stream, u, C,
                       (uint32_t)ldc, u_out, p->qd[0], p->qtab[0], nq, nwgq, p->blocks2, p->htab, p->etab, p->dtab,
                       npair ? p->qsingles2 : p->qsingles[0], ns, nwgs, T.quad_singles_first, 1, dt_dev, npair,
                       T.arith_ids ? p->qaux[0] : (const int32_t*)nullptr);
}

int debug_buffer2d(unsigned long long* buf) {
    IBH_HIP(hipMemcpyToSymbol(HIP_SYMBOL(ibh_dbg_buf), &buf, sizeof(buf)));
    return 0;
}

}

extern "C" {

int ibh_step_advection_xgmi(ibh_part* p, float* u, const float* C, int64_t ldc, float* ud, const int32_t* send_all,
                            int n_send_peers, const int32_t* send_seg, float* const* dst0, float* const* dst1,
                            uint32_t* const* send_flags, const int32_t* recv_all, const float* src0, const float* src1,
                            int n_recv_peers, const int32_t* recv_seg, const uint32_t* const* recv_flags,
                            uint32_t* state, uint32_t max_spins, unsigned long long* fstate) {
    IBH_REQUIRE(p && u && C && ud && state && fstate, "ibh_step_advection_xgmi: null argument");
    IBH_REQUIRE(fused2(p, 0) && p->img_all_fz && !p->fuse_all && quads_usable(p, 1, 0),
                "ibh_step_advection_xgmi: needs a 2-D partition with skirt fragments whose image blocks are all eligible "
                "for the quad sweep");
    IBH_REQUIRE(n_send_peers >= 0 && n_send_peers <= IBH_MAX_PEERS && n_recv_peers >= 0 && n_recv_peers <= IBH_MAX_PEERS &&
                    n_send_peers + n_recv_peers > 0,
                "ibh_step_advection_xgmi: 1 to 16 peers");
    XchgArgs A;
    memset(&A, 0, sizeof(A));
    A.ns = n_send_peers;
    A.nr = n_recv_peers;
    if (n_send_peers) {
        IBH_REQUIRE(send_all && send_seg && dst0 && dst1 && send_flags, "ibh_step_advection_xgmi: null send argument");
        for (int q = 0; q < n_send_peers; ++q) {
            A.dst[0][q] = dst0[q];
            A.dst[1][q] = dst1[q];
            A.sflag[q] = send_flags[q];
            A.sseg[q] = send_seg[q];
            IBH_REQUIRE(send_seg[q + 1] >= send_seg[q], "ibh_step_advection_xgmi: segments must ascend");
        }
        A.sseg[n_send_peers] = send_seg[n_send_peers];
    }
    if (n_recv_peers) {
        IBH_REQUIRE(recv_all && src0 && src1 && recv_seg && recv_flags, "ibh_step_advection_xgmi: null receive argument");
        for (int q = 0; q < n_recv_peers; ++q) {
            A.rflag[q] = recv_flags[q];
            A.rseg[q] = recv_seg[q];
            IBH_REQUIRE(recv_seg[q + 1] >= recv_seg[q], "ibh_step_advection_xgmi: segments must ascend");
        }
        A.rseg[n_recv_peers] = recv_seg[n_recv_peers];
    }
    const int32_t big = std::max(A.ns ? A.sseg[A.ns] : 0, A.nr ? A.rseg[A.nr] : 0);
    int E = (big + 255) / 256;
    E = E < 1 ? 1 : E > 64 ? 64 : E;
    const int32_t nq = p->nq[1], nqi = p->nq_int[1], ns = p->nqs[1], nsi = p->nqs_int[1];
    const int32_t nwg = (nqi + WPB - 1) / WPB + (nsi + WPB - 1) / WPB + (nq - nqi + WPB - 1) / WPB + (ns - nsi + WPB - 1) / WPB;
    static_assert(WPB == 4, "the exchange workgroups of k_step_quad are 256 threads");
    hipLaunchKernelGGL(p->n_dt > 0 ? k_step_quad<true> : k_step_quad<false>, dim3(E + nwg), dim3(64 * WPB), 0, ibh_stream, u, C,
                       (uint32_t)ldc, ud, p->qd[1], p->qtab[1], nqi, nq, p->blocks2, p->htab, p->etab, p->dtab, p->qsingles[1],
                       nsi, ns, send_all, recv_all, src0, src1, A, state, max_spins, E, fstate);
    IBH_LAUNCH_CHECK();
    return 0;
}

}
```

### immersedboundary.jl_amd/csrc/ibh_fused_int.h

```cpp
#pragma once
#include <stdlib.h>

#include "ibh_common.h"
#include "ibh_euler_step_dev.h"

namespace fused __attribute__((visibility("hidden"))) {

inline int env_int(const char* name, int dflt) {
    const char* s = getenv(name);
    return s ? atoi(s) : dflt;
}
enum : int {
    QV_STAMPS = 4,
    QV_THREAD_PER_CELL = 512,
};
inline bool quad_variant_known(int v) { return v == 0 || v == QV_STAMPS || v == QV_THREAD_PER_CELL; }
inline int quad_variant_or_0(int v) { return quad_variant_known(v) ? v : 0; }

struct Tuning {
    int sweep_iters = env_int("IBH_SWEEP_ITERS", 0);
    int quad = env_int("IBH_QUAD", 1);
    int rows = env_int("IBH_ROWS", 0);
    int quad_variant = quad_variant_or_0(env_int("IBH_QUAD_VARIANT", 0));
    int quad_parts = 3, quad_singles_iters = 1;
    int quad_singles_first = env_int("IBH_SINGLES_FIRST", 0);
    int pairs = env_int("IBH_PAIRS", 1);
    int arith_ids = env_int("IBH_ARITH_IDS", 1);
    int transport_blocks = 1;
    int rows_singles = env_int("IBH_ROWS_SINGLES", -1);
};
extern Tuning T;

constexpr int F_LITERAL = IBH_FORCE_GENERAL | IBH_EXACT;
constexpr int F_TWO_KERNEL = IBH_NO_FUSE | IBH_PASS_A_ONLY | IBH_PASS_B_ONLY;
constexpr int F_PHASES = IBH_PHASE_INTERIOR | IBH_PHASE_BOUNDARY;

inline bool has_blocks(const ibh_part* p) { return p->bs == 8 && p->nblk > 0 && (p->nd == 2 ? !!p->blocks2 : !!p->blocks3); }
inline bool tuned2(const ibh_part* p, int flags) { return p->nd == 2 && has_blocks(p) && !(flags & F_LITERAL); }
inline bool tuned3(const ibh_part* p, int flags) { return p->nd == 3 && has_blocks(p) && !(flags & F_LITERAL); }
inline bool fused2(const ibh_part* p, int flags) { return tuned2(p, flags) && !(flags & F_TWO_KERNEL); }
inline bool whole3(const ibh_part* p, int flags) { return tuned3(p, flags) && !(flags & (F_TWO_KERNEL | F_PHASES)); }
inline bool image3(const ibh_part* p, int flags) { return whole3(p, flags) && (flags & IBH_IMAGE_ONLY) && p->img_all3; }
inline bool single3(const ibh_part* p, int flags) { return whole3(p, flags) && !(flags & IBH_IMAGE_ONLY) && p->sweep3; }
inline bool all_blocks3(const ibh_part* p) {
    return p->nd == 3 && has_blocks(p) && p->n_irr == 0 && (int64_t)p->nblk * 512 == p->nc && p->info[6] == 0;
}
inline bool quads_usable(const ibh_part* p, int k, int flags) { return T.quad && !(flags & IBH_NO_QUAD) && p->nq[k] > 0; }

struct Range { int32_t first, last; int32_t count() const { return last - first; } };
struct Phase {
    bool interior, boundary;
    explicit Phase(int flags) : interior((flags & IBH_PHASE_INTERIOR) != 0), boundary((flags & IBH_PHASE_BOUNDARY) != 0) {}
    bool any() const { return interior || boundary; }
    bool valid() const { return !(interior && boundary); }
    Range of(int32_t n_int, int32_t n_all) const { return {boundary ? n_int : 0, interior ? n_int : n_all}; }
};
#define IBH_PHASES_EXCLUSIVE "IBH_PHASE_INTERIOR and IBH_PHASE_BOUNDARY are exclusive"

struct AdvArgs { const float *u, *C; int64_t ldc; float* ud; };
struct EulerArgs {
    const float* P; int64_t ldp; float* R; int64_t ldr; const ibh_fluid* fluid;
    EulerScheme scheme = EULER_HLL; const float* nu = nullptr;
    EulerForm form = FORM_RESIDUAL;
    const float* dt = nullptr; bool dt_cells = false;
    const float* P0 = nullptr; int64_t ld0 = 0; float c = 1.0f;
    float a = 0.0f, b = 1.0f;
    const float* S = nullptr; int64_t lds = 0; float g = 0.0f;
};

enum AdvPath {
    ADV3_IMAGE_COLS,
    ADV3_SINGLE,
    ADV3_BLOCKS,
    ADV2_IMAGE,
    ADV2_FUSE_ALL,
    ADV2_MIXED,
    ADV_GENERAL_2D,
    ADV_GENERAL_2D_EXACT,
    ADV_GENERAL_3D,
};

enum EulerPath {
    EUL2_SINGLE,
    EUL3_IMAGE_COLS,
    EUL3_SINGLE,
    EUL2_FAST,
    EUL2_FACE_LIST,
    EUL3_BLOCKS,
    EUL3_FACE_LIST,
};

void adv2_block_list(const ibh_part* p, const AdvArgs& a, const int32_t* list, Range r);
void adv2_single(const ibh_part* p, const AdvArgs& a, int flags, Phase ph, int k);
void adv2_step_quads(const ibh_part* p, const float* u, float* u_out, const float* C, int64_t ldc, const float* dt_dev);
void euler2_single(const ibh_part* p, const EulerArgs& e, int flags, Phase ph);
void adv3_image_cols(const ibh_part* p, const AdvArgs& a);
void adv3_single(const ibh_part* p, const AdvArgs& a);
int adv3_blocks(ibh_part* p, const AdvArgs& a, int flags, Phase ph);
void euler3_image_cols(const ibh_part* p, const EulerArgs& e);
void euler3_single(const ibh_part* p, const EulerArgs& e);
int euler3_blocks(ibh_part* p, const EulerArgs& e, int flags);
int ensure_G(ibh_part* p);
int adv2_mixed(ibh_part* p, const AdvArgs& a, int flags, Phase ph);
int adv_general(ibh_part* p, const AdvArgs& a, int flags, Phase ph, AdvPath path);
int euler_general(ibh_part* p, const EulerArgs& e, int flags, EulerPath path);
void euler_passB_cells(const ibh_part* p, const EulerArgs& e, const int32_t* cells, int32_t n);
int debug_buffer2d(unsigned long long* buf);
int debug_buffer3d(unsigned long long* buf);

}
```

### immersedboundary.jl_amd/csrc/ibh_quad2d.h

```cpp
#pragma once
#include "ibh_sweep2d.h"

namespace quad2 {

#pragma clang fp contract(fast)

typedef float v2f __attribute__((ext_vector_type(2)));
typedef float v4f __attribute__((ext_vector_type(4)));
typedef int v2i __attribute__((ext_vector_type(2)));
typedef float v4f_g __attribute__((ext_vector_type(4), aligned(4)));

#define QUAD_PITCH 20
#define QUAD_TILE (18 * QUAD_PITCH)
#define QUAD_OFF_EXT (4 * QUAD_TILE)
#define QUAD_OFF_RING (QUAD_OFF_EXT + 160)
#define QUAD_LDS (QUAD_OFF_RING + 2 * 64)

__device__ __forceinline__ float dpp_shr1(float old, float v) {
    return __int_as_float(__builtin_amdgcn_update_dpp(__float_as_int(old), __float_as_int(v), 0x111, 0xf, 0xf, false));
}
__device__ __forceinline__ float dpp_shl1(float old, float v) {
    return __int_as_float(__builtin_amdgcn_update_dpp(__float_as_int(old), __float_as_int(v), 0x101, 0xf, 0xf, false));
}
__device__ __forceinline__ float bperm(int byte_addr, float v) {
    return __int_as_float(__builtin_amdgcn_ds_bpermute(byte_addr, __float_as_int(v)));
}
__device__ __forceinline__ float max3(float a, float b, float c) { return fmaxf(fmaxf(a, b), c); }
__device__ __forceinline__ float lds_read(const float* p) {
    float v = *p;
    asm volatile("" : "+v"(v));
    return v;
}

__device__ __forceinline__ v4f flux_half4(v4f ua, v4f ub, v4f Sa, v4f Sb, v4f Da, v4f Db, v4f Ca, v4f Cb) {
    const v4f d = ub - ua;
    const v4f gu = Sa - 0.5f * d;
    const v4f Du = Sb - 0.5f * d;
    v4f s, Df;
#pragma unroll
    for (int c = 0; c < 4; ++c) {
        s[c] = __builtin_amdgcn_fmed3f(Du[c], gu[c], 0.0f);
        Df[c] = max3(Da[c], Db[c], 1e-7f);
    }
    const v4f t16 = (Sa - Sb) * 0.0625f;
    const v4f uf = (ua + 0.5f * d) + t16;
    const v4f A = uf - Df * t16;
    const v4f Cf = 0.5f * (Ca + Cb);
    const v4f B = Df * (s - 0.5f * d);
    const v4f CA = Cf * A;
    v4f F;
#pragma unroll
    for (int c = 0; c < 4; ++c) F[c] = fmaf(fabsf(Cf[c]), B[c], CA[c]);
    return F;
}

__device__ __forceinline__ v2f flux_w2(float ua, v2f ub, float Sa, v2f Sb, float Da, v2f Db, float Ca, v2f Cb, float wa) {
    const v2f d = ub - ua;
    const v2f gu = Sa - d * wa;
    const v2f Du = Sb - d * (1.0f - wa);
    const v2f s = v2f{__builtin_amdgcn_fmed3f(Du.x, gu.x, 0.0f), __builtin_amdgcn_fmed3f(Du.y, gu.y, 0.0f)};
    const v2f t16 = (Sa - Sb) * 0.0625f;
    const v2f uf = (ua + wa * d) + t16;
    const v2f mu = d * (0.5f - wa) - t16;
    const v2f Df = v2f{max3(Da, Db.x, 1e-7f), max3(Da, Db.y, 1e-7f)};
    const v2f A = uf + Df * mu;
    const v2f Cf = Ca + wa * (Cb - Ca);
    const v2f B = Df * (s - 0.5f * d);
    const v2f CA = Cf * A;
    return v2f{fmaf(fabsf(Cf.x), B.x, CA.x), fmaf(fabsf(Cf.y), B.y, CA.y)};
}

__device__ __forceinline__ float jst(float g, float a, float rh) {
    return fmaf(fabsf(g), rh, 1e-7f) * __builtin_amdgcn_rcpf(fmaf(a, rh, 1e-7f));
}
__device__ __forceinline__ float jst_max2(float g1, float a1, float rh1, float g2, float a2, float rh2) {
    const float n1 = fmaf(fabsf(g1), rh1, 1e-7f), d1 = fmaf(a1, rh1, 1e-7f);
    const float n2 = fmaf(fabsf(g2), rh2, 1e-7f), d2 = fmaf(a2, rh2, 1e-7f);
    return fmaxf(fmaxf(n1 * d2, n2 * d1) * __builtin_amdgcn_rcpf(d1 * d2), 1e-7f);
}

template <bool HALF>
struct QuadLaneTab {
    uint32_t w[64][8];
    constexpr QuadLaneTab() : w() {
        for (int lane = 0; lane < 64; ++lane) {
            const int g = lane >> 4, t = lane & 15, tl = lane & 7, lhs = lane >> 3;
            const int ytop = HALF ? 7 : 15;
            const bool g0 = g == 0, g3 = g == 3, lr = g0 || g3, t0 = t == 0, t15 = t == ytop;
            const int bx = g0 ? 0 : g3 ? 15 : t, by = lr ? t : g == 1 ? 0 : ytop;
            const int pos_b = (by + 1) * QUAD_PITCH + bx;
            const int pos_b1 = lr ? ((t ^ 1) + 1) * QUAD_PITCH + bx : (by + 1) * QUAD_PITCH + (t ^ 1);
            const int pos_up = t * QUAD_PITCH + 4 * g;
            const int pos_hm = g0 ? (t + 1) * QUAD_PITCH - 1 : g3 ? (t + 1) * QUAD_PITCH + 16 : g == 1 ? t : (ytop + 2) * QUAD_PITCH + t;
            const int pos_exw = g == 1 ? t : g == 2 ? (ytop + 1) * QUAD_PITCH + t : 17 * QUAD_PITCH + 19;
            const int myrow = t0 ? 0 : t15 ? 1 : 2, rowB = t0 ? 0 : 2, rowT = t15 ? 1 : 2;
            const int wrow = g == 1 ? 0 : g == 2 ? 1 : 3;
            const int eline = (lane & 31) >> 2, ee = lane & 3;
            const int epos = QUAD_OFF_EXT + eline * 20 + (ee < 2 ? ee : 16 + ee);
            const int line = QUAD_OFF_EXT + lhs * 20;
            const uint32_t f[12] = {
                (uint32_t)pos_up, (uint32_t)pos_b, (uint32_t)pos_b1, (uint32_t)epos,
                (uint32_t)(QUAD_OFF_RING + wrow * 16 + t), (uint32_t)(QUAD_OFF_RING + myrow * 16 + 4 * g),
                (uint32_t)(QUAD_OFF_RING + rowB * 16 + 4 * g), (uint32_t)(QUAD_OFF_RING + rowT * 16 + 4 * g),
                (uint32_t)(line + 2 * tl), (uint32_t)(line + 2 * (tl & ~1)), (uint32_t)pos_hm, (uint32_t)pos_exw};
            for (int k = 0; k < 6; ++k) w[lane][k] = (4u * f[2 * k]) | ((4u * f[2 * k + 1]) << 16);
            w[lane][6] = 4u * (64u * ((g >> 1) + (HALF ? 0 : 2 * (t >> 3))) + 4u * (g & 1) + 8u * (t & 7));
            w[lane][7] = (uint32_t)(g0 ? -1 : g == 1 ? -8 : g == 2 ? 8 : 0);
        }
    }
};
__device__ const QuadLaneTab<false> lane_tab = QuadLaneTab<false>();
__device__ const QuadLaneTab<true> lane_tab_half = QuadLaneTab<true>();

#define QL_MASK(m) __builtin_amdgcn_inverse_ballot_w64(m)

struct QuadLane {
    float *p_up;
    float *p_hm;
    float *p_exw;
    float *p_b;
    float *p_b1;
    float *p_epos;
    float *p_ringw;
    float *p_ringm;
    float *p_ringB;
    float *p_ringT;
    float *p_LbS;
    float *p_LbC;
    uint32_t a0off4;
    int offB;
    int lane;
    bool g0, g3, lr, dny;
    bool tl0, tl7;
    bool active;
    float sgn;
};

template <bool HALF = false>
__device__ __forceinline__ QuadLane quad_lane(float* lds, int lane) {
    QuadLane G;
    char* const L = (char*)lds;
    const uint32_t* const tab = HALF ? lane_tab_half.w[lane] : lane_tab.w[lane];
    const uint4 w0 = *(const uint4*)(tab);
    const uint4 w1 = *(const uint4*)(tab + 4);
#define QL_LO(w) ((w) & 0xffffu)
#define QL_HI(w) ((w) >> 16)
    G.p_up = (float*)(L + QL_LO(w0.x));
    G.p_b = (float*)(L + QL_HI(w0.x));
    G.p_b1 = (float*)(L + QL_LO(w0.y));
    G.p_epos = (float*)(L + QL_HI(w0.y));
    G.p_ringw = (float*)(L + QL_LO(w0.z));
    G.p_ringm = (float*)(L + QL_HI(w0.z));
    G.p_ringB = (float*)(L + QL_LO(w0.w));
    G.p_ringT = (float*)(L + QL_HI(w0.w));
    G.p_LbS = (float*)(L + QL_LO(w1.x));
    G.p_LbC = (float*)(L + QL_HI(w1.x));
    G.p_hm = (float*)(L + QL_LO(w1.y));
    G.p_exw = (float*)(L + QL_HI(w1.y));
#undef QL_LO
#undef QL_HI
    G.sgn = QL_MASK(0xffffffff00000000ull) ? 1.0f : -1.0f;
    G.a0off4 = w1.z;
    G.offB = (int)w1.w;
    G.lane = lane;
    G.g0 = QL_MASK(0x000000000000ffffull);
    G.g3 = QL_MASK(0xffff000000000000ull);
    G.lr = QL_MASK(0xffff00000000ffffull);
    G.dny = QL_MASK(0x0000ffffffff0000ull);
    G.tl0 = QL_MASK(0x0101010101010101ull);
    G.tl7 = QL_MASK(0x8080808080808080ull);
    G.active = QL_MASK(HALF ? 0x00ff00ff00ff00ffull : ~0ull);
    ((float*)(L + 4 * (QUAD_OFF_RING + 32)))[lane & 15] = 0.0f;
    ((float*)(L + 4 * (QUAD_OFF_RING + 64 + 32)))[lane & 15] = 0.5f;
    return G;
}

struct QuadTab {
    QuadDesc2 d;
    uint32_t ty;
    v2i hid;
    uint32_t eid;
};
struct QuadOwn {
    v4f U, CX, CY;
};
struct QuadHalo {
    v2f hu, hd, hc;
    float eu;
};
__device__ __forceinline__ QuadTab quad_load_tab(const QuadDesc2* __restrict__ qd, const int32_t* __restrict__ qtab,
                                                 int32_t q, int lane, const int32_t* __restrict__ qaux = nullptr) {
    QuadTab T;
    T.d = qd[q];
    T.ty = (T.d.cls >> ((lane >> 1) & 28)) & 15u;
    const int32_t* row = qtab + (size_t)q * IBH_QROW;
    if (qaux) {
        const int32_t* aux = qaux + (size_t)q * IBH_QAUX;
        const int lhs = lane >> 3, tl = lane & 7;
        const int32_t orig = aux[32 + lhs];
        T.eid = (uint32_t)aux[lane & 31];
        const bool isC = T.ty == SIDE_COARSE;
        const bool lr = QL_MASK(0xffff00000000ffffull);
        const int32_t id = orig + (lr ? 8 : 1) * (isC ? tl >> 1 : tl);
        T.hid = v2i{id, id};
        if (orig < 0) T.hid = *(const v2i*)(row + 2 * lane);
        return T;
    }
    T.hid = *(const v2i*)(row + 2 * lane);
    T.eid = (uint32_t)row[128 + (lane & 31)];
    return T;
}
__device__ __forceinline__ size_t quad_base4(const QuadTab& T) { return (size_t)(uint32_t)T.d.base << 2; }
__device__ __forceinline__ QuadOwn quad_load_own(const QuadLane& G, const QuadTab& T, const float* __restrict__ u,
                                                 const float* __restrict__ C, uint32_t ldc) {
    QuadOwn O;
    const size_t b4 = quad_base4(T);
    O.U = *(const v4f_g*)((const char*)u + b4 + G.a0off4);
    O.CX = *(const v4f_g*)((const char*)C + b4 + G.a0off4);
    O.CY = *(const v4f_g*)((const char*)(C + ldc) + b4 + G.a0off4);
    return O;
}
__device__ __forceinline__ QuadHalo quad_load_halo_paired(const QuadLane& G, const QuadTab& T, const float* __restrict__ u,
                                                          const float* __restrict__ C, uint32_t ldc) {
    using blk2::ldg;
    typedef float v2f_g __attribute__((ext_vector_type(2), aligned(4)));
    auto pair = [](const float* p, int i) { return *(const v2f_g*)((const char*)p + ((size_t)(uint32_t)i << 2)); };
    QuadHalo H;
    const float* Cn = C + (G.dny ? ldc : 0u);
    const bool isF = T.ty == SIDE_FINE;
    const v2f PA = pair(u, T.hid.x - (int)G.g0);
    const v2f PB = pair(u, (G.lr ? T.hid.y : T.hid.x) + G.offB);
    const v2f PC = pair(Cn, T.hid.x);
    H.eu = ldg(u, T.eid);
    float hc1 = 0.0f;
    if (G.lr && isF) hc1 = ldg(Cn, (uint32_t)T.hid.y);
    asm volatile("" : "+v"(hc1));
    const bool dF = G.dny && isF;
    const float a = dF ? PA.y : PA.x;
    H.hu.x = G.g0 ? PA.y : PA.x;
    H.hd.x = G.g0 ? PA.x : (G.g3 ? PA.y : PB.x);
    H.hu.y = G.g0 ? PB.y : (G.g3 ? PB.x : a);
    H.hd.y = (G.g3 || dF) ? PB.y : PB.x;
    H.hc.x = PC.x;
    H.hc.y = isF ? (G.lr ? hc1 : PC.y) : PC.x;
    return H;
}

template <bool STAMP, bool STEP = false, bool HALF = false>
__device__ __forceinline__ void quad_compute(const QuadLane& G, const QuadTab& T, const QuadOwn& O, const QuadHalo& H,
                                             float* __restrict__ ud, unsigned long long* stamps, float dt = 0.0f) {
    using blk2::wave_lds_sync;
    auto stamp = [&](int k) {
        if constexpr (STAMP) {
            __builtin_amdgcn_s_waitcnt(0);
            if (stamps && G.lane == 0) stamps[k] = __builtin_amdgcn_s_memrealtime();
        }
    };
    const v4f U = O.U, CX = O.CX, CY = O.CY;
    const v2f hu = H.hu, hd = H.hd, hc = H.hc;
    const bool g0 = G.g0, g3 = G.g3, lr = G.lr, dny = G.dny;
    const int lane = G.lane;
    const float sgn = G.sgn;
    const uint32_t ty = T.ty;
    const bool isC = ty == SIDE_COARSE, isF = ty == SIDE_FINE;
    const float qs = isC ? (1.0f / 3.0f) : isF ? (2.0f / 3.0f) : 0.5f;
    const float irt = isC ? 0.5f : isF ? 2.0f : 1.0f;
    const float rhx = T.d.rh[0], rhy = T.d.rh[1];

    float* const p_own = G.p_up + QUAD_PITCH;
    *(v4f*)p_own = U;
    *(v4f*)(p_own + 3 * QUAD_TILE) = CY;
    *(v2f*)(G.p_LbS + 2) = hu;
    *G.p_epos = H.eu;
    wave_lds_sync();
    stamp(4);
    const float m0 = lds_read(G.p_b);
    const float m1r = lds_read(G.p_b1);
    const float m1 = isC ? m1r : m0;
    const float hm = 0.5f * (hu.x + hu.y);
    const float fix = 0.5f * (fabsf(hu.x - m0) + fabsf(hu.y - m0)) - fabsf(hm - m0);
    *G.p_hm = hm;
    G.p_ringw[0] = fix;
    G.p_ringw[64] = qs;
    wave_lds_sync();
    stamp(5);

    v4f SX, SY, D;
    v4f uT;
    {
        const v4f UL = v4f{p_own[-1], U.x, U.y, U.z};
        const v4f UR = v4f{U.y, U.z, U.w, p_own[4]};
        const v4f qL = v4f{g0 ? qs : 0.5f, 0.5f, 0.5f, 0.5f};
        const v4f qR = v4f{0.5f, 0.5f, 0.5f, g3 ? qs : 0.5f};
        const v4f dR = UR - U, dL = U - UL;
#pragma unroll
        for (int c = 0; c < 4; ++c) SX[c] = fmaf(qR[c], dR[c], qL[c] * dL[c]);
        const v4f gx = dR - dL;
        const v4f rF = *(const v4f*)G.p_ringm;
        const v4f qB = *(const v4f*)(G.p_ringB + 64);
        const v4f qT = *(const v4f*)(G.p_ringT + 64);
        const v4f uB = *(const v4f*)G.p_up;
        uT = *(const v4f*)(G.p_up + 2 * QUAD_PITCH);
        const v4f dT = uT - U, dB = U - uB;
        SY = qT * dT + qB * dB;
        const v4f gy = dT - dB;
        const float fx0 = g0 ? fix : 0.0f, fx3 = g3 ? fix : 0.0f;
#pragma unroll
        for (int c = 0; c < 4; ++c) {
            float ax = fabsf(dR[c]) + fabsf(dL[c]);
            if (c == 0) ax += fx0;
            if (c == 3) ax += fx3;
            const float ay = (fabsf(dT[c]) + fabsf(dB[c])) + rF[c];
            D[c] = jst_max2(gx[c], ax, rhx, gy[c], ay, rhy);
        }
    }
    *(v4f*)(p_own + QUAD_TILE) = SY;
    *(v4f*)(p_own + 2 * QUAD_TILE) = D;

    v2f Shn, Dh;
    {
        const float ihn = (dny ? rhy : rhx) * irt, iht = (dny ? rhx : rhy) * irt;
        const v2f dm0 = m0 - hu, dm1 = m1 - hu, dde = hd - hu;
        const v2f din = 0.5f * (dm0 + dm1);
        Shn = 0.5f * dde - (1.0f - qs) * din;
        const v2f Lp = *(const v2f*)(isC ? G.p_LbC : G.p_LbS);
        const v2f Hp = *(const v2f*)((isC ? G.p_LbC + 2 : G.p_LbS) + 4);
        const bool t0l = G.tl0, t7l = G.tl7;
        const v2f lo0 = v2f{(isF && !t0l) ? Lp.y : Lp.x, isF ? hu.x : Lp.x};
        const v2f lo1 = v2f{Lp.y, isF ? hu.x : Lp.y};
        const v2f hi0 = v2f{isF ? hu.y : Hp.x, Hp.x};
        const v2f hi1 = v2f{isF ? hu.y : Hp.y, (isF && !t7l) ? Hp.x : Hp.y};
        const v2f e0 = lo0 - hu, e1 = lo1 - hu, e2 = hi0 - hu, e3 = hi1 - hu;
        const v2f gn = (dm0 + dm1) + (dde + dde);
        const v2f gt = (e0 + e1) + (e2 + e3);
        const float hn = 0.5f * ihn, ht = 0.5f * iht;
#pragma unroll
        for (int k = 0; k < 2; ++k) {
            const float an = (fabsf(dm0[k]) + fabsf(dm1[k])) + 2.0f * fabsf(dde[k]);
            const float at = (fabsf(e0[k]) + fabsf(e1[k])) + (fabsf(e2[k]) + fabsf(e3[k]));
            Dh[k] = jst_max2(gn[k], an, hn, gt[k], at, ht);
        }
    }

    wave_lds_sync();
    stamp(6);
    v4f FR, FT;
    {
        const int up = (lane + 16) << 2;
        const v4f Ub = v4f{U.y, U.z, U.w, bperm(up, U.x)};
        const v4f Sb = v4f{SX.y, SX.z, SX.w, bperm(up, SX.x)};
        const v4f Db = v4f{D.y, D.z, D.w, bperm(up, D.x)};
        const v4f Cb = v4f{CX.y, CX.z, CX.w, bperm(up, CX.x)};
        FR = flux_half4(U, Ub, SX, Sb, D, Db, CX, Cb);
        const v4f St = *(const v4f*)(p_own + QUAD_TILE + QUAD_PITCH);
        const v4f Dt = *(const v4f*)(p_own + 2 * QUAD_TILE + QUAD_PITCH);
        const v4f Ct = *(const v4f*)(p_own + 3 * QUAD_TILE + QUAD_PITCH);
        FT = flux_half4(U, uT, SY, St, D, Dt, CY, Ct);
    }
    *(v4f*)p_own = FT;

    float edge;
    {
        const float So_lr = g3 ? SX.w : SX.x, Co_lr = g3 ? CX.w : CX.x;
        const float So_bt = lds_read(G.p_b + QUAD_TILE), Do = lds_read(G.p_b + 2 * QUAD_TILE),
                    Co_bt = lds_read(G.p_b + 3 * QUAD_TILE);
        const float So = lr ? So_lr : So_bt;
        const float Co = lr ? Co_lr : Co_bt;
        const v2f F = flux_w2(m0, hu, sgn * So, Shn, Do, Dh, sgn * Co, sgn * hc, qs);
        edge = sgn * (0.5f * (F.x + F.y));
    }
    *G.p_exw = edge;
    wave_lds_sync();
    stamp(7);

    {
        const float FRm = bperm((lane - 16) << 2, FR.w);
        const v4f FL = v4f{g0 ? edge : FRm, FR.x, FR.y, FR.z};
        const v4f FRf = v4f{FR.x, FR.y, FR.z, g3 ? edge : FR.w};
        const v4f FB = *(const v4f*)G.p_up;
        const v4f FTf = *(const v4f*)p_own;
        const v4f res = -((FRf - FL) * rhx) - ((FTf - FB) * rhy);
        float* const out = (float*)((char*)ud + quad_base4(T) + G.a0off4);
#ifdef Q2_NO_NT_STORE
        if (!HALF || G.active) *(v4f_g*)out = STEP ? U + dt * res : res;
#else
        if (!HALF || G.active) {
            if constexpr (STEP) *(v4f_g*)out = U + dt * res;
            else __builtin_nontemporal_store(res, (v4f_g*)out);
        }
#endif
    }
}

template <bool STAMP, bool STEP = false, bool HALF = false>
__device__ __forceinline__ void sweep_quad(const QuadDesc2* __restrict__ qd, const int32_t* __restrict__ qtab, int32_t q,
                                           const float* __restrict__ u, const float* __restrict__ C, uint32_t ldc,
                                           float* __restrict__ ud, float* lds, int lane,
                                           unsigned long long* stamps = nullptr, float dt = 0.0f,
                                           const int32_t* __restrict__ qaux = nullptr) {
    const QuadLane G = quad_lane<HALF>(lds, lane);
    const QuadTab T = quad_load_tab(qd, qtab, q, lane, qaux);
    const QuadOwn O = quad_load_own(G, T, u, C, ldc);
    const QuadHalo H = quad_load_halo_paired(G, T, u, C, ldc);
    quad_compute<STAMP, STEP, HALF>(G, T, O, H, ud, stamps, dt);
}

#pragma clang fp contract(off)

}
```

### immersedboundary.jl_amd/hostview.py

```python
import ctypes as C

import numpy as np

from ._lib import c_vp, call

BLOCK_DTYPE = np.dtype([("base", "<i4"), ("type", "<i4", (4,)), ("nb", "<i4", (4, 2)), ("sub", "<i4", (4,)),
                        ("h", "<f4", (2,)), ("rh", "<f4", (2,)), ("q", "<f4", (4,)), ("rt", "<f4", (4,)),
                        ("dt", "<i4")])
QUAD_DTYPE = np.dtype([("base", "<i4"), ("cls", "<u4"), ("rh", "<f4", (2,))])
(BLOCKS, HTAB, ETAB, FUSABLE, QUAD_DESC, QUAD_TAB, SINGLES, COUNTS, INFO, PAIR_DESC, PAIR_TAB, SINGLES2, QUAD_AUX,
 PAIR_AUX) = range(14)
SIDE_SAME, SIDE_MIRROR, SIDE_COARSE, SIDE_FINE, SIDE_GENERAL = range(5)


def analyze2(part):
    nd = part.ndims
    assert nd == 2
    nc = part.spacing.shape[0]
    spacing = np.asfortranarray(part.spacing, dtype=np.float32)
    nf = np.array([part.face_owners_neighbors[d + 1][0].shape[0] for d in range(nd)], dtype=np.int32)
    keep = []

    def parr(arrs):
        arrs = [np.ascontiguousarray(a, dtype=np.int32) for a in arrs]
        keep.append(arrs)
        return (c_vp * nd)(*[a.ctypes.data for a in arrs])

    owners = parr([part.face_owners_neighbors[d + 1][0] for d in range(nd)])
    neighbors = parr([part.face_owners_neighbors[d + 1][1] for d in range(nd)])
    loff = parr([part.face_accumulators[(d + 1, False)].off for d in range(nd)])
    lidx = parr([part.face_accumulators[(d + 1, False)].idx for d in range(nd)])
    roff = parr([part.face_accumulators[(d + 1, True)].off for d in range(nd)])
    ridx = parr([part.face_accumulators[(d + 1, True)].idx for d in range(nd)])
    iid = np.ascontiguousarray(part.image_in_domain, dtype=np.int32)
    dom = np.ascontiguousarray(part.domain, dtype=np.int32)
    h = c_vp()
    call("ibh_analyze2_host", C.byref(h), nc, spacing.ctypes.data_as(c_vp), nf.ctypes.data_as(c_vp), owners, neighbors,
         loff, lidx, roff, ridx, int(iid.size), iid.ctypes.data_as(c_vp), dom.ctypes.data_as(c_vp), 0)

    def get(what, dtype, set_=0):
        n = C.c_int64(0)
        call("ibh_host2d_get", h, what, set_, c_vp(None), 0, C.byref(n))
        buf = np.empty(n.value, dtype=np.uint8)
        if n.value:
            call("ibh_host2d_get", h, what, set_, buf.ctypes.data_as(c_vp), n.value, C.byref(n))
        return buf.view(dtype)

    try:
        out = dict(blocks=get(BLOCKS, BLOCK_DTYPE), htab=get(HTAB, np.int32).reshape(-1, 64),
                   etab=get(ETAB, np.int32).reshape(-1, 16), fusable=get(FUSABLE, np.uint8).astype(bool),
                   info=get(INFO, np.int64))
        for k, name in ((0, "all"), (1, "image")):
            cnt = get(COUNTS, np.int64, k)
            out[f"quads_{name}"] = dict(desc=get(QUAD_DESC, QUAD_DTYPE, k), tab=get(QUAD_TAB, np.int32, k).reshape(-1, 160),
                                        singles=get(SINGLES, np.int32, k), n_interior=int(cnt[2]),
                                        n_singles_interior=int(cnt[4]),
                                        pair_desc=get(PAIR_DESC, QUAD_DTYPE, k),
                                        pair_tab=get(PAIR_TAB, np.int32, k).reshape(-1, 160),
                                        singles2=get(SINGLES2, np.int32, k),
                                        aux=get(QUAD_AUX, np.int32, k).reshape(-1, 40),
                                        pair_aux=get(PAIR_AUX, np.int32, k).reshape(-1, 40))
            out.update(fuse_all=bool(cnt[5]), img_all_fz=bool(cnt[6]), nB1=int(cnt[7]))
    finally:
        call("ibh_host2d_destroy", h)
    return out
```

### include/ibhip.h

```cpp
#ifndef IBHIP_H
#define IBHIP_H

#include <stddef.h>
#include <stdint.h>

#ifdef __cplusplus
extern "C" {
#endif

typedef struct ibh_part ibh_part;
typedef struct ibh_acc ibh_acc;
typedef struct ibh_bc ibh_bc;

typedef struct ibh_fluid {
    float R;
    float gamma;
    float mu_ref;
    float Tref;
    float S;
    int32_t nk;
    float k[4];
} ibh_fluid;

int ibh_init(int device);
const char* ibh_last_error(void);
int ibh_set_stream(void* hip_stream);
int ibh_sync(void);
int ibh_version(void);

int ibh_malloc(void** dptr, size_t bytes);
int ibh_free(void* dptr);
int ibh_h2d(void* dst, const void* src, size_t bytes);
int ibh_d2h(void* dst, const void* src, size_t bytes);
int ibh_memset(void* dst, int value, size_t bytes);
int ibh_owned_device_memory(int64_t* bytes, int64_t* buffers);

int ibh_partition_create(ibh_part** out, int nd, int32_t nc,
                         const float* spacing, const float* centers,
                         const int32_t* nf,
                         const int32_t* const* owners, const int32_t* const* neighbors,
                         const int32_t* const* left_off, const int32_t* const* left_idx,
                         const int32_t* const* right_off, const int32_t* const* right_idx,
                         int32_t n_image, const int32_t* image_in_domain,
                         const int32_t* domain, int block_size, int index_base);
int ibh_partition_destroy(ibh_part* part);
int ibh_partition_info(const ibh_part* part, int64_t* info, int n);

enum { IBH_EW_ADD = 0, IBH_EW_SUB = 1, IBH_EW_MUL = 2, IBH_EW_DIV = 3, IBH_EW_MAX = 4, IBH_EW_MIN = 5, IBH_EW_SUM = 6 };
enum { IBH_EW_ABS = 16, IBH_EW_NEG = 17, IBH_EW_SQRT = 18, IBH_EW_COPY = 19 };
int ibh_ew_binary(int op, int64_t n, int nv, const float* a, int nva, float sa, const float* b, int nvb, float sb,
                  float* out);
int ibh_ew_unary(int op, int64_t total, const float* a, float* out);
int ibh_ew_fill(int64_t total, float value, float* out);
int ibh_ew_reduce(int op, int64_t total, const float* a, float* out_device);
enum { IBH_EW_PUSH_ARRAY = 32, IBH_EW_PUSH_SCALAR = 33 };
int ibh_ew_eval(int64_t n, int nv, int nprog, const int32_t* prog, int narr, const float* const* arrays,
                const int32_t* arr_nv, int nscal, const float* scalars, float* out);
enum { IBH_EW_PUSH_ROW = 34 };
enum { IBH_EW_LT = 64, IBH_EW_LE = 65, IBH_EW_GT = 66, IBH_EW_GE = 67, IBH_EW_EQ = 68, IBH_EW_NE = 69, IBH_EW_AND = 70,
       IBH_EW_OR = 71, IBH_EW_POW = 72, IBH_EW_COPYSIGN = 73, IBH_EW_ATAN2 = 74, IBH_EW_BMUL = 75 };
enum { IBH_EW_EXP = 80, IBH_EW_EXP2 = 81, IBH_EW_LOG = 82, IBH_EW_LOG2 = 83, IBH_EW_LOG10 = 84, IBH_EW_SIN = 85,
       IBH_EW_COS = 86, IBH_EW_TANH = 87, IBH_EW_ATAN = 88, IBH_EW_SIGN = 89, IBH_EW_INV = 90, IBH_EW_NOT = 91,
       IBH_EW_POW0 = 92, IBH_EW_SQR = 93, IBH_EW_CUBE = 94, IBH_EW_INVSQR = 95 };
enum { IBH_EW_CLAMP = 112, IBH_EW_IFELSE = 113 };
int ibh_ew_reduce_rows(int64_t n, int nv, const float* a, float* out);

int ibh_set_tuning(const char* key, int value);
int ibh_debug_buffer(void* device_buffer);

int ibh_probe_sweep(ibh_part* part, const float* u, const float* C, int64_t ldc, float* ud, int mode);
int ibh_probe_dispatch(int nwg, int threads, int lds_bytes);

typedef struct ibh_host2d ibh_host2d;
enum {
    IBH_H2D_BLOCKS = 0,
    IBH_H2D_HTAB = 1,
    IBH_H2D_ETAB = 2,
    IBH_H2D_FUSABLE = 3,
    IBH_H2D_QUAD_DESC = 4,
    IBH_H2D_QUAD_TAB = 5,
    IBH_H2D_SINGLES = 6,
    IBH_H2D_COUNTS = 7,
    IBH_H2D_INFO = 8,
    IBH_H2D_PAIR_DESC = 9,
    IBH_H2D_PAIR_TAB = 10,
    IBH_H2D_SINGLES2 = 11,
    IBH_H2D_QUAD_AUX = 12,
    IBH_H2D_PAIR_AUX = 13
};
int ibh_analyze2_host(ibh_host2d** out, int32_t nc, const float* spacing, const int32_t* nf,
                      const int32_t* const* owners, const int32_t* const* neighbors,
                      const int32_t* const* left_off, const int32_t* const* left_idx,
                      const int32_t* const* right_off, const int32_t* const* right_idx,
                      int32_t n_image, const int32_t* image_in_domain, const int32_t* domain, int index_base);
int ibh_host2d_get(const ibh_host2d* h, int what, int set, void* dst, int64_t cap_bytes, int64_t* nbytes);
int ibh_host2d_destroy(ibh_host2d* h);

int ibh_at_owners(const ibh_part*, int dim, const float* u, int nv, int64_t ldu, float* out, int64_t ldo);
int ibh_at_neighbors(const ibh_part*, int dim, const float* u, int nv, int64_t ldu, float* out, int64_t ldo);
int ibh_at_faces(const ibh_part*, int dim, const float* u, int nv, int64_t ldu, float* out, int64_t ldo);
int ibh_green_gauss(const ibh_part*, int dim, const float* uf, int nv, int64_t ldf, float* out, int64_t ldo,
                    int unsigned_sum);
int ibh_cell_gradient(const ibh_part*, int dim, const float* u, int nv, int64_t ldu, float* out, int64_t ldo);
int ibh_cell_gradient_all(const ibh_part*, const float* u, int nv, int64_t ldu, float* out, int64_t ldo);
int ibh_cell_gradient_nd(ibh_part*, const float* u, int nv, int64_t ldu, float* out, int64_t ldo, float* sensor,
                         int64_t lds);
int ibh_cell_gradient_fields(ibh_part*, const float* u, int nv, int64_t ldu, float* out);
int ibh_face_distance(const ibh_part*, int dim, float* out);
int ibh_owner_distance(const ibh_part*, int dim, float* out);
int ibh_neighbor_distance(const ibh_part*, int dim, float* out);
int ibh_face_gradient(const ibh_part*, int dim, const float* u, int nv, int64_t ldu, float* out, int64_t ldo);
int ibh_jst_sensor(const ibh_part*, int dim, const float* p, int nv, int64_t ldp, float* out, int64_t ldo);
int ibh_muscl(const ibh_part*, int dim, const float* u, const float* du, int nv, int64_t ld,
              const float* D, int high_order, float* uL, float* uR, int64_t ldf);

int ibh_acc_create(ibh_acc** out, int32_t n_output, int32_t n_input,
                   const int32_t* off, const int32_t* idx, const float* w, int index_base);
int ibh_acc_destroy(ibh_acc*);
int ibh_accumulate(const ibh_acc*, const float* v, int nv, int64_t ldv, float* out, int64_t ldo);
int ibh_accumulate_diff_add(const ibh_acc*, const float* v, const float* v2, int nv, int64_t ldv, float* out, int64_t ldo);

int ibh_bc_create(ibh_bc** out, int32_t n_ghost, const int32_t* ghost_indices,
                  const float* ghost_distances, const float* image_distances,
                  int32_t n_image_domain, const int32_t* image_domain,
                  const int32_t* interp_off, const int32_t* interp_idx, const float* interp_w,
                  int index_base);
int ibh_bc_destroy(ibh_bc*);
int ibh_bc_interp(const ibh_bc*, const float* a, int nv, int64_t lda, float* ia, int64_t ldi);
int ibh_bc_blend(const ibh_bc*, float* a, int nv, int64_t lda, const float* ia, int64_t ldi,
                 const float* ba, int64_t ldb, const float* ba_const);
int ibh_bc_apply(const ibh_bc*, float* a, int nv, int64_t lda, int mode, const float* ba_const);

int ibh_gather_rows(const int32_t* rows, int32_t n, const float* src, int nv, int64_t lds, float* dst, int64_t ldd);
int ibh_scatter_rows(const int32_t* rows, int32_t n, const float* src, int nv, int64_t lds, float* dst, int64_t ldd);
int ibh_copy_rows(const int32_t* dst_rows, const int32_t* src_rows, int32_t n,
                  const float* src, int nv, int64_t lds, float* dst, int64_t ldd);

#define IBH_FORCE_GENERAL 1
#define IBH_IMAGE_ONLY 2
#define IBH_PASS_A_ONLY 4
#define IBH_PASS_B_ONLY 8
#define IBH_PHASE_INTERIOR 32
#define IBH_PHASE_BOUNDARY 64
#define IBH_NO_FUSE 128
#define IBH_FORCE_MIXED 512
#define IBH_SWEEP_ONLY 256
#define IBH_NO_QUAD 1024
#define IBH_EXACT 16
int ibh_residual_advection(ibh_part*, const float* u, const float* C, int64_t ldc, float* ud, int flags);
int ibh_residual_advection_n(ibh_part*, const float* u, const float* C, int64_t ldc, float* ud, int flags, int n);
int ibh_residual_euler_hll(ibh_part*, const float* P, int64_t ldp, float* R, int64_t ldr,
                           const ibh_fluid* fluid, int flags);
int ibh_residual_euler_sensor(ibh_part*, const float* P, int64_t ldp, const float* nu ,
                              float* R, int64_t ldr, const ibh_fluid* fluid, int flags);

int ibh_cfd_speed_of_sound(const ibh_fluid*, int64_t n, const float* T, float* a);
int ibh_cfd_dynamic_viscosity(const ibh_fluid*, int64_t n, const float* T, float* mu);
int ibh_cfd_heat_conductivity(const ibh_fluid*, int64_t n, const float* T, float* k);
int ibh_cfd_primitive2state(const ibh_fluid*, int nd, int64_t n, const float* P, int64_t ldp,
                            float* Q, int64_t ldq);
int ibh_cfd_state2primitive(const ibh_fluid*, int nd, int64_t n, const float* Q, int64_t ldq,
                            float* P, int64_t ldp);
int ibh_cfd_inviscid_fluxes_hll(const ibh_fluid*, int nd, int dim, int64_t n, const float* PL, const float* PR,
                                int64_t ld, float* F, int64_t ldf);
int ibh_cfd_inviscid_fluxes_sensor(const ibh_fluid*, int nd, int dim, int64_t n, const float* PL, const float* PR,
                                   int64_t ld, const float* nuL, const float* nuR, float* F, int64_t ldf);
int ibh_cfd_jst_sensor3(int64_t n, const float* Pim1, const float* Pi, const float* Pip1, float* out);
int ibh_cfd_shock_sensor(int nd, int64_t n, const float* const* velocity_gradients, float* out);
int ibh_cfd_viscous_fluxes(const ibh_fluid*, int nd, int dim, int64_t n, const float* P, int64_t ldp,
                           const float* const* Pgrad, int64_t ldg, const float* mu_t, float mu_t_const,
                           float* F, int64_t ldf);
int ibh_viscous_residual(const ibh_part*, const ibh_fluid*, const float* P, int64_t ldp, const float* const* Pgrad,
                         int64_t ldg, int grad_vel_col, const float* mu_t, float* R, int64_t ldr);

int ibh_ipc_alloc(void** dptr, size_t bytes, int fine_grained);
int ibh_ipc_free(void* dptr);
int ibh_ipc_export(void* dptr, void* handle64);
int ibh_ipc_import(const void* handle64, void** dptr);
int ibh_ipc_close(void* dptr);
int ibh_flag_signal(uint32_t* counter, uint32_t* const* slots, int n);
int ibh_flag_wait(uint32_t* counter, const uint32_t* const* slots, int n, uint32_t max_spins, uint32_t* status);
int ibh_halo_push(const float* f, int nv, int64_t ld, const int32_t* send_all, int n_peers, const int32_t* seg,
                  float* const* dst, uint32_t* const* flags, uint32_t* state);
int ibh_halo_pull(float* f, int nv, int64_t ld, const int32_t* recv_all, const float* src, int n_peers,
                  const int32_t* seg, const uint32_t* const* flags, uint32_t* state, uint32_t max_spins);
int ibh_halo_exchange(float* f, int nv, int64_t ld, const int32_t* send_all, int n_send_peers, const int32_t* send_seg,
                      float* const* dst0, float* const* dst1, uint32_t* const* send_flags, const int32_t* recv_all,
                      const float* src0, const float* src1, int n_recv_peers, const int32_t* recv_seg,
                      const uint32_t* const* recv_flags, uint32_t* state, uint32_t max_spins);
int ibh_step_advection_xgmi(ibh_part*, float* u, const float* C, int64_t ldc, float* ud, const int32_t* send_all,
                            int n_send_peers, const int32_t* send_seg, float* const* dst0, float* const* dst1,
                            uint32_t* const* send_flags, const int32_t* recv_all, const float* src0, const float* src1,
                            int n_recv_peers, const int32_t* recv_seg, const uint32_t* const* recv_flags,
                            uint32_t* state, uint32_t max_spins, unsigned long long* fstate);

typedef struct ibh_bcset ibh_bcset;
int ibh_bcset_create(ibh_bcset** out, int n_bc, const ibh_bc* const* bcs, const int32_t* modes, const float* values);
int ibh_bcset_destroy(ibh_bcset*);
int ibh_bcset_info(const ibh_bcset*, int32_t* n_ghost, int32_t* n_levels);
int ibh_bcset_apply(const ibh_bcset*, float* a);
int ibh_timestep_advection(ibh_part*, const float* C, int64_t ldc, float scale, float* dt_device);
int ibh_update_dev(int64_t n, const float* dt_device, const float* u, const float* r, float* out);
int ibh_step_advection(ibh_part*, const float* u, float* u_out, const float* C, int64_t ldc, const float* dt_device,
                       const ibh_bcset* bcs );
int ibh_step_advection_dt(ibh_part* p, const float* u, float* u_out, const float* C, int64_t ldc, const float* dt_dev,
                          const ibh_bcset* bcs, float scale, float* dt_next);
#define IBH_EULER_HLL 0
#define IBH_EULER_SENSOR 1
int ibh_timestep_euler(ibh_part*, const ibh_fluid*, const float* P, int64_t ldp, float scale,
                       float* dt_device , float* dt_cells );
int ibh_update_euler(const ibh_fluid*, int nd, int64_t n, const float* P, int64_t ldp, const float* R, int64_t ldr,
                     const float* dt, int dt_per_cell, float* P_out, int64_t ldo);
int ibh_step_euler(ibh_part*, const ibh_fluid*, int scheme , const float* P, int64_t ldp,
                   float* P_out, int64_t ldo, const float* dt, int dt_per_cell, float* work ,
                   int64_t ldw, int flags);
int ibh_update_euler_stage(const ibh_fluid*, int nd, int64_t n, const float* P0, int64_t ld0, const float* R, int64_t ldr,
                           const float* dt, int dt_per_cell, float alpha, float* P_out, int64_t ldo);
int ibh_stage_euler(ibh_part*, const ibh_fluid*, int scheme , const float* P, int64_t ldp,
                    const float* P0, int64_t ld0, float* P_out, int64_t ldo, const float* dt, int dt_per_cell, float alpha,
                    float* work , int64_t ldw, int flags);
int ibh_update_euler_ssp(const ibh_fluid*, int nd, int64_t n, const float* P0, int64_t ld0, const float* P, int64_t ldp,
                         const float* R, int64_t ldr, const float* dt, int dt_per_cell, float a, float b, float c,
                         float* P_out, int64_t ldo);
int ibh_stage_euler_ssp(ibh_part*, const ibh_fluid*, int scheme , const float* P,
                        int64_t ldp, const float* P0, int64_t ld0, float* P_out, int64_t ldo, const float* dt, int dt_per_cell,
                        float a, float b, float c, float* work , int64_t ldw, int flags);
int ibh_smooth_residual(const ibh_part*, const float* R, int nv, int64_t ldr, float eps, int n_iter, float* S, int64_t lds,
                        float* tmp , int64_t ldt);
int ibh_update_euler_smoothed(const ibh_part*, const ibh_fluid*, int blend , const float* P0,
                              int64_t ld0, const float* P, int64_t ldp, const float* R, int64_t ldr, const float* Sprev,
                              int64_t lds, float eps, const float* dt, int dt_per_cell, float a, float b, float c,
                              float* P_out, int64_t ldo);
int ibh_dual_source(const ibh_fluid*, int nd, int64_t n, const float* Pn, int64_t ldn, const float* Pm ,
                    int64_t ldm, float cn, float cm, float* S, int64_t lds);
int ibh_update_euler_dual(const ibh_fluid*, int nd, int64_t n, const float* P0, int64_t ld0, const float* R, int64_t ldr,
                          const float* S, int64_t lds, const float* dt, int dt_per_cell, float alpha, float g, float* P_out,
                          int64_t ldo);
int ibh_stage_euler_dual(ibh_part*, const ibh_fluid*, int scheme , const float* P,
                         int64_t ldp, const float* P0, int64_t ld0, const float* S, int64_t lds, float* P_out, int64_t ldo,
                         const float* dt, int dt_per_cell, float alpha, float g, float* work ,
                         int64_t ldw, int flags);
int ibh_restrict_euler(const ibh_acc* coarsener, const ibh_fluid*, int nd, const float* P_f, int64_t ldpf, const float* R_f,
                       int64_t ldrf, const float* S_f , int64_t ldsf, float* P_c, int64_t ldpc, float* D_c,
                       int64_t lddc);
int ibh_prolong_euler(const ibh_acc* prolongator, const ibh_fluid*, int nd, const float* Pc_new, const float* Pc_old,
                      int64_t ldc, float* pack , const float* P_f, int64_t ldpf,
                      float* P_out, int64_t ldo);
#define IBH_ROLE_FLUID 0
#define IBH_ROLE_GHOST 1
// ... 99 lines not shown
```

Before: 134,200.

## Add specialized no-fine-side quad sweep path and class-ordered quad scheduling

Adds a specialised quad sweep (ONE/FORMS) for quads with no fine-resolution sides. These quads load one halo value per face instead of two and skip the averaging and fix-up arithmetic. Quads and pairs can also be reordered at analysis time so general (fine) quads come first, and a class-aware workgroup remap spreads each class evenly across XCDs. Both features are gated by tuning knobs (quad_one_slot, quad_order), which adds template variants and code-size or divergence risk.

New measurement: 131,200. 2.2% lower.

```diff
diff --git a/immersedboundary.jl_amd/_lib.py b/immersedboundary.jl_amd/_lib.py
--- a/immersedboundary.jl_amd/_lib.py
+++ b/immersedboundary.jl_amd/_lib.py
@@ -46,6 +46,7 @@
                           C.POINTER(c_vp), C.POINTER(c_vp), C.POINTER(c_vp), C.c_int32, c_vp, c_vp, c_int],
     "ibh_host2d_get": [c_vp, c_int, c_int, c_vp, c_i64, C.POINTER(c_i64)],
     "ibh_host2d_destroy": [c_vp],
+    "ibh_quad_wg_map": [c_vp, c_vp, c_vp, C.c_int32, c_vp],
     "ibh_at_owners": [c_vp, c_int, c_vp, c_int, c_i64, c_vp, c_i64],
     "ibh_at_neighbors": [c_vp, c_int, c_vp, c_int, c_i64, c_vp, c_i64],
     "ibh_at_faces": [c_vp, c_int, c_vp, c_int, c_i64, c_vp, c_i64],
diff --git a/immersedboundary.jl_amd/backend.py b/immersedboundary.jl_amd/backend.py
--- a/immersedboundary.jl_amd/backend.py
+++ b/immersedboundary.jl_amd/backend.py
@@ -213,6 +213,7 @@
                          image_quad_singles=info[15], row_sweep=bool(info[16]), direct_sides=info[17],
                          quad_pairs=info[18] if self.nd == 2 else 0,
                          quad_arith_half_sides=info[19] if self.nd == 2 else 0,
+                         quads_no_fine=info[21] if self.nd == 2 else 0, quad_pairs_no_fine=info[22] if self.nd == 2 else 0,
                          tiled=bool(info[20]),
                          rim4_rows=info[12] if self.nd == 3 else 0)
 
diff --git a/immersedboundary.jl_amd/csrc/ibh_analyze.cpp b/immersedboundary.jl_amd/csrc/ibh_analyze.cpp
--- a/immersedboundary.jl_amd/csrc/ibh_analyze.cpp
+++ b/immersedboundary.jl_amd/csrc/ibh_analyze.cpp
@@ -354,8 +354,9 @@
 
 void ibh_build_quads2(const std::vector<BlockDesc2>& blocks, const std::vector<int32_t>& htab,
                       const std::vector<int32_t>& etab, const std::vector<char>& cand, int32_t nB1, QuadSet2& out,
-                      int32_t nc) {
+                      int32_t nc, bool fine_first) {
     out = QuadSet2();
+    out.ordered = fine_first ? 1 : 0;
     const int32_t nb = (int32_t)blocks.size();
     std::unordered_map<int32_t, int32_t> bybase;
     bybase.reserve(nb * 2);
@@ -411,9 +412,19 @@
     }
     static const int side_of_g[4] = {0, 2, 3, 1};
     static const int blk_of[4][2] = {{0, 2}, {0, 1}, {2, 3}, {1, 3}};
+    auto quad_cls = [&](const Q& q) {
+        uint32_t cls = 0;
+        for (int g = 0; g < 4; ++g)
+            for (int half = 0; half < 2; ++half)
+                cls |= (uint32_t)blocks[q.b[blk_of[g][half]]].type[side_of_g[g]] << (4 * (2 * g + half));
+        return cls;
+    };
     for (int pass = 0; pass < 2; ++pass)
+      for (int general = 1; general >= (fine_first ? 0 : 1); --general)
         for (const Q& q : quads) {
             if (q.interior != (pass == 0)) continue;
+            if (fine_first && quad_no_fine(quad_cls(q)) == (general == 1)) continue;
+            if (fine_first && general) ++(pass == 0 ? out.nqf_int : out.nqf_bnd);
             QuadDesc2 d;
             d.base = blocks[q.b[0]].base;
             d.rh[0] = blocks[q.b[0]].rh[0];
@@ -492,6 +503,20 @@
         out.pd.push_back(d);
         quad_aux_row(out.ptab.data() + row, d.cls, out.paux);
     }
+    if (fine_first) {
+        QuadSet2 o;
+        for (int general = 1; general >= 0; --general)
+            for (size_t i = 0; i < out.pd.size(); ++i) {
+                if (quad_no_fine(out.pd[i].cls) == (general == 1)) continue;
+                o.pd.push_back(out.pd[i]);
+                o.ptab.insert(o.ptab.end(), out.ptab.begin() + i * IBH_QROW, out.ptab.begin() + (i + 1) * IBH_QROW);
+                o.paux.insert(o.paux.end(), out.paux.begin() + i * IBH_QAUX, out.paux.begin() + (i + 1) * IBH_QAUX);
+                out.npf += general;
+            }
+        out.pd.swap(o.pd);
+        out.ptab.swap(o.ptab);
+        out.paux.swap(o.paux);
+    }
     for (int32_t b : out.singles)
         if (!paired[b]) out.singles2.push_back(b);
 }
diff --git a/immersedboundary.jl_amd/csrc/ibh_api.hip b/immersedboundary.jl_amd/csrc/ibh_api.hip
--- a/immersedboundary.jl_amd/csrc/ibh_api.hip
+++ b/immersedboundary.jl_amd/csrc/ibh_api.hip
@@ -63,7 +63,7 @@
             if (H.needg[b]) { H.ng.push_back(b); H.n_ng_int += b < H.nph[0]; }
         }
     H.info[9] = H.fuse_all ? 0 : (int64_t)H.ng.size();
-    if (H.fuse_all) ibh_build_quads2(H.blocks, H.htab, H.etab, H.fus, H.nph[1], H.quads[0], nc);
+    if (H.fuse_all) ibh_build_quads2(H.blocks, H.htab, H.etab, H.fus, H.nph[1], H.quads[0], nc, ibh_quad_order_enabled());
     if (H.fuse_all && H.dtab.empty()) {
         bool ok = true;
         for (int32_t b = 0; b < nb && ok; ++b) {
@@ -86,7 +86,8 @@
         }
         H.rows_ok = ok;
     }
-    if (H.img_all_fz && !H.fuse_all) ibh_build_quads2(H.blocks, H.htab, H.etab, is_imgblk, H.nph[1], H.quads[1], nc);
+    if (H.img_all_fz && !H.fuse_all)
+        ibh_build_quads2(H.blocks, H.htab, H.etab, is_imgblk, H.nph[1], H.quads[1], nc, ibh_quad_order_enabled());
 }
 
 static int make_view(HostPartView& v, int nd, int32_t nc, const float* spacing, const int32_t* nf,
@@ -270,6 +271,11 @@
             p->nq_int[k] = Q.nq_int;
             p->nqs[k] = (int32_t)Q.singles.size();
             p->nqs_int[k] = Q.ns_int;
+            p->quad_ordered[k] = Q.ordered;
+            p->nqf_int[k] = Q.nqf_int;
+            p->nqf_bnd[k] = Q.nqf_bnd;
+            for (const QuadDesc2& d : Q.qd) p->info[21] += quad_no_fine(d.cls);
+            for (const QuadDesc2& d : Q.pd) p->info[22] += quad_no_fine(d.cls);
             p->info[12 + 2 * k] = p->nq[k];
             p->info[13 + 2 * k] = p->nqs[k];
             if (k == 0 && !Q.pd.empty()) {
@@ -414,8 +420,8 @@
     const QuadSet2& Q = H.quads[set];
     const void* src = nullptr;
     int64_t n = 0;
-    int64_t counts[8] = {(int64_t)H.blocks.size(), (int64_t)Q.qd.size(), Q.nq_int, (int64_t)Q.singles.size(), Q.ns_int,
-                         H.fuse_all, H.img_all_fz, H.nph[1]};
+    int64_t counts[12] = {(int64_t)H.blocks.size(), (int64_t)Q.qd.size(), Q.nq_int, (int64_t)Q.singles.size(), Q.ns_int,
+                          H.fuse_all, H.img_all_fz, H.nph[1], Q.ordered, Q.nqf_int, Q.nqf_bnd, Q.npf};
     switch (what) {
         case IBH_H2D_BLOCKS: src = H.blocks.data(); n = (int64_t)(H.blocks.size() * sizeof(BlockDesc2)); break;
         case IBH_H2D_HTAB: src = H.htab.data(); n = (int64_t)(H.htab.size() * 4); break;
diff --git a/immersedboundary.jl_amd/csrc/ibh_common.h b/immersedboundary.jl_amd/csrc/ibh_common.h
--- a/immersedboundary.jl_amd/csrc/ibh_common.h
+++ b/immersedboundary.jl_amd/csrc/ibh_common.h
@@ -29,6 +29,7 @@
     uint32_t cls;
     float rh[2];
 };
+__host__ __device__ inline bool quad_no_fine(uint32_t cls) { return ((cls & (cls >> 1)) & 0x11111111u) == 0; }
 #define IBH_QROW 160
 #define IBH_QAUX 40
 struct QuadSet2 {
@@ -37,6 +38,7 @@
     std::vector<int32_t> qaux, paux;
     std::vector<int32_t> singles;
     int32_t nq_int = 0, ns_int = 0;
+    int32_t ordered = 0, nqf_int = 0, nqf_bnd = 0, npf = 0;
     std::vector<QuadDesc2> pd;
     std::vector<int32_t> ptab;
     std::vector<int32_t> singles2;
@@ -88,6 +90,7 @@
     int32_t* qaux[2] = {nullptr, nullptr};
     int32_t* qsingles[2] = {nullptr, nullptr};
     int32_t nq[2] = {0, 0}, nq_int[2] = {0, 0}, nqs[2] = {0, 0}, nqs_int[2] = {0, 0};
+    int32_t quad_ordered[2] = {0, 0}, nqf_int[2] = {0, 0}, nqf_bnd[2] = {0, 0};
     int32_t npair = 0, nqs2 = 0;
     int32_t* qsingles2 = nullptr;
     int32_t* fz_list = nullptr;
@@ -193,7 +196,8 @@
 
 void ibh_build_quads2(const std::vector<BlockDesc2>& blocks, const std::vector<int32_t>& htab,
                       const std::vector<int32_t>& etab, const std::vector<char>& cand, int32_t nB1, QuadSet2& out,
-                      int32_t nc);
+                      int32_t nc, bool fine_first);
+bool ibh_quad_order_enabled();
 
 struct Sweep3Host {
     bool all = false;
@@ -231,7 +235,7 @@
 void ibh_launch_sum_partials(int n, const double* part, double* out, int ncols = 1);
 
 #ifdef __HIPCC__
-__device__ __forceinline__ int32_t ibh_xcd_chunk(int32_t wg, int32_t nwg) {
+__host__ __device__ __forceinline__ int32_t ibh_xcd_chunk(int32_t wg, int32_t nwg) {
     const int32_t q = nwg >> 3, r = nwg & 7, xcd = wg & 7, idx = wg >> 3;
     return (xcd < r ? xcd * (q + 1) : r * (q + 1) + (xcd - r) * q) + idx;
 }
@@ -242,6 +246,25 @@
     return ibh_xcd_chunk(wg, nwg);
 #endif
 }
+#define IBH_NCLASS 3
+__host__ __device__ __forceinline__ int32_t ibh_class_wgs(const int32_t n[IBH_NCLASS], int32_t wpb) {
+    int32_t t = 0;
+    for (int c = 0; c < IBH_NCLASS; ++c) t += (n[c] + wpb - 1) / wpb;
+    return t;
+}
+struct IbhClassWg { int32_t cls, pos; };
+__host__ __device__ __forceinline__ IbhClassWg ibh_class_remap(int32_t wg, const int32_t n[IBH_NCLASS], int32_t wpb) {
+    const int32_t x = wg & 7;
+    int32_t idx = wg >> 3, start = 0;
+    for (int c = 0; c < IBH_NCLASS; ++c) {
+        const int32_t nw = (n[c] + wpb - 1) / wpb, r = nw & 7, xr = (x - start) & 7;
+        const int32_t share = (nw >> 3) + (xr < r ? 1 : 0);
+        if (idx < share) return {c, ibh_xcd_chunk(xr + 8 * idx, nw)};
+        idx -= share;
+        start = (start + r) & 7;
+    }
+    return {IBH_NCLASS, 0};
+}
 #ifdef IBH_NO_XCD_CELLS
 #define IBH_WG_X() ((int64_t)blockIdx.x)
 #else
diff --git a/immersedboundary.jl_amd/csrc/ibh_fused.hip b/immersedboundary.jl_amd/csrc/ibh_fused.hip
--- a/immersedboundary.jl_amd/csrc/ibh_fused.hip
+++ b/immersedboundary.jl_amd/csrc/ibh_fused.hip
@@ -31,6 +31,8 @@
     return tuned3(p, flags) ? EUL3_BLOCKS : EUL3_FACE_LIST;
 }
 
+bool ibh_quad_order_enabled() { return T.quad_order != 0; }
+
 extern "C" {
 
 int ibh_debug_buffer(void* buf) {
@@ -45,7 +47,8 @@
         {"time_average_nt", &ibh_time_average_nt},
         {"quad_variant", &T.quad_variant}, {"quad_parts", &T.quad_parts}, {"quad_singles_first", &T.quad_singles_first},
         {"quad_singles_iters", &T.quad_singles_iters}, {"rows", &T.rows}, {"rows_singles", &T.rows_singles},
-        {"transport_blocks", &T.transport_blocks}, {"pairs", &T.pairs}, {"arith_ids", &T.arith_ids}};
+        {"transport_blocks", &T.transport_blocks}, {"pairs", &T.pairs}, {"arith_ids", &T.arith_ids},
+        {"quad_one_slot", &T.quad_one_slot}, {"quad_order", &T.quad_order}};
     IBH_REQUIRE(key, "ibh_set_tuning: null key");
     for (const auto& k : keys)
         if (!strcmp(key, k.key)) {
diff --git a/immersedboundary.jl_amd/csrc/ibh_fused2d.hip b/immersedboundary.jl_amd/csrc/ibh_fused2d.hip
--- a/immersedboundary.jl_amd/csrc/ibh_fused2d.hip
+++ b/immersedboundary.jl_amd/csrc/ibh_fused2d.hip
@@ -39,7 +39,7 @@
     if (ibh_dbg_buf && threadIdx.x % 64 == 0) ibh_dbg_buf[(size_t)slot * 8 + k] = v;
 }
 
-template <bool DT, bool STAMP, bool STEP = false, bool RS = false>
+template <bool DT, bool STAMP, bool STEP = false, bool RS = false, bool FORMS = false, bool ORD = false>
 #ifndef QS_WAVES
 #define QS_WAVES 5
 #endif
@@ -54,7 +54,8 @@
                                                          const int32_t* __restrict__ singles, int32_t ns, int32_t nwgs,
                                                          int32_t singles_first, int32_t siters,
                                                          const float* __restrict__ dtp = nullptr, int32_t npair = 0,
-                                                         const int32_t* __restrict__ qaux = nullptr) {
+                                                         const int32_t* __restrict__ qaux = nullptr, int32_t nqf = -1,
+                                                         int32_t pairs_second = 0) {
     __shared__ __attribute__((aligned(16))) float lds[RS && WPB * ROWS_LDS > QUAD_WG_LDS ? WPB * ROWS_LDS : QUAD_WG_LDS];
     float dt = 0.0f;
     if constexpr (STEP) dt = *dtp;
@@ -62,18 +63,37 @@
     const int32_t slot = blockIdx.x * WPB + wave;
     if constexpr (STAMP) {
         dbg_stamp(slot, 0, __builtin_amdgcn_s_memrealtime());
-        dbg_stamp(slot, 2, __builtin_amdgcn_s_getreg((4 << 0) | (0 << 6) | (31 << 11)));
+        dbg_stamp(slot, 2, (unsigned long long)__builtin_amdgcn_s_getreg((4 << 0) | (0 << 6) | (31 << 11)) |
+                               ((unsigned long long)__builtin_amdgcn_s_getreg((20 << 0) | (0 << 6) | (3 << 11)) << 32));
     }
     const int32_t wgq = singles_first ? (int32_t)blockIdx.x - nwgs : (int32_t)blockIdx.x;
     const bool isq = wgq >= 0 && wgq < nwgq;
+    int32_t qrow = -1;
     if (isq) {
-        const int32_t q = __builtin_amdgcn_readfirstlane(xcd_remap(wgq, nwgq) * WPB + wave);
-        if (q < nq)
-            quad2::sweep_quad<STAMP, STEP>(qd, qtab, q, u, C, ldc, ud, lds + wave * QUAD_LDS, lane,
-                                           STAMP && ibh_dbg_buf ? ibh_dbg_buf + (size_t)slot * 8 : nullptr, dt, qaux);
-        else if (q < nq + npair)
-            quad2::sweep_quad<STAMP, STEP, true>(qd, qtab, q, u, C, ldc, ud, lds + wave * QUAD_LDS, lane,
-                                                 STAMP && ibh_dbg_buf ? ibh_dbg_buf + (size_t)slot * 8 : nullptr, dt, qaux);
+        if constexpr (!ORD) {
+            const int32_t q = __builtin_amdgcn_readfirstlane(xcd_remap(wgq, nwgq) * WPB + wave);
+            if (q < nq)
+                quad2::sweep_quad<STAMP, STEP, false, FORMS>(qd, qtab, q, u, C, ldc, ud, lds + wave * QUAD_LDS, lane,
+                                                             STAMP && ibh_dbg_buf ? ibh_dbg_buf + (size_t)slot * 8 : nullptr, dt, qaux);
+            else if (q < nq + npair)
+                quad2::sweep_quad<STAMP, STEP, true, FORMS>(qd, qtab, q, u, C, ldc, ud, lds + wave * QUAD_LDS, lane,
+                                                            STAMP && ibh_dbg_buf ? ibh_dbg_buf + (size_t)slot * 8 : nullptr, dt, qaux);
+            if constexpr (STAMP) qrow = q < nq + npair ? q : -1;
+        } else {
+            const int32_t n[IBH_NCLASS] = {nqf, pairs_second ? npair : nq - nqf, pairs_second ? nq - nqf : npair};
+            const IbhClassWg w = ibh_class_remap(wgq, n, WPB);
+            const bool others = w.cls == (pairs_second ? 2 : 1);
+            const int32_t q = __builtin_amdgcn_readfirstlane((w.cls == 0 ? 0 : others ? nqf : nq) + w.pos * WPB + wave);
+            const int32_t qend = w.cls == 0 ? nqf : others ? nq : nq + npair;
+            if (q >= qend) {
+            } else if (q < nq)
+                quad2::sweep_quad<STAMP, STEP, false, FORMS>(qd, qtab, q, u, C, ldc, ud, lds + wave * QUAD_LDS, lane,
+                                                             STAMP && ibh_dbg_buf ? ibh_dbg_buf + (size_t)slot * 8 : nullptr, dt, qaux);
+            else
+                quad2::sweep_quad<STAMP, STEP, true, FORMS>(qd, qtab, q, u, C, ldc, ud, lds + wave * QUAD_LDS, lane,
+                                                            STAMP && ibh_dbg_buf ? ibh_dbg_buf + (size_t)slot * 8 : nullptr, dt, qaux);
+            if constexpr (STAMP) qrow = q < qend ? q : -1;
+        }
     } else {
         const int32_t wgs = singles_first ? (int32_t)blockIdx.x : (int32_t)blockIdx.x - nwgq;
         if constexpr (RS) {
@@ -94,7 +114,7 @@
     if constexpr (STAMP) {
         __builtin_amdgcn_s_waitcnt(0);
         dbg_stamp(slot, 1, __builtin_amdgcn_s_memrealtime());
-        dbg_stamp(slot, 3, (unsigned long long)isq);
+        dbg_stamp(slot, 3, (unsigned long long)(isq ? 2 + qrow : 0));
     }
 }
 
@@ -113,7 +133,7 @@
         rows2::sweep_rows(blocks + b0, etab + (size_t)b0 * 16, first, n, u, C, ldc, ud, lds + wave * ROWS_LDS, lane, list);
 }
 
-template <bool DT>
+template <bool DT, bool FORMS = false>
 __global__ __launch_bounds__(64 * WPB) void k_step_quad(float* __restrict__ u, const float* __restrict__ C, uint32_t ldc,
                                                         float* __restrict__ ud, const QuadDesc2* __restrict__ qd,
                                                         const int32_t* __restrict__ qtab, int32_t nq_int, int32_t nq,
@@ -167,7 +187,7 @@
     const int32_t nws = boundary ? nwg_sb : nwg_si, s0 = boundary ? ns_int : 0, s1 = boundary ? ns : ns_int;
     if (b < nwq) {
         const int32_t q = __builtin_amdgcn_readfirstlane(q0 + xcd_remap(b, nwq) * WPB + wave);
-        if (q < q1) quad2::sweep_quad<false>(qd, qtab, q, u, C, ldc, ud, lds + wave * QUAD_LDS, lane);
+        if (q < q1) quad2::sweep_quad<false, false, false, FORMS>(qd, qtab, q, u, C, ldc, ud, lds + wave * QUAD_LDS, lane);
     } else {
         const int32_t first = __builtin_amdgcn_readfirstlane(s0 + xcd_remap(b - nwq, nws) * WPB + wave);
         if (first < s1)
@@ -256,6 +276,21 @@
     return r;
 }
 
+int32_t general_quads(const ibh_part* p, int k, Range q) {
+    if (!T.quad_order || !p->quad_ordered[k]) return -1;
+    if (q.count() <= 0) return 0;
+    if (q.first == 0 && q.last == p->nq_int[k]) return p->nqf_int[k];
+    if (q.first == p->nq_int[k] && q.last == p->nq[k]) return p->nqf_bnd[k];
+    return -1;
+}
+#define QUAD_KERNEL(DT, STAMP, STEP, forms, ord)                                                                       \
+    ((forms) ? ((ord) ? k_sweep_quad<DT, STAMP, STEP, false, true, true> : k_sweep_quad<DT, STAMP, STEP, false, true>) \
+             : ((ord) ? k_sweep_quad<DT, STAMP, STEP, false, false, true> : k_sweep_quad<DT, STAMP, STEP>))
+int32_t quad_wgs(int32_t nq, int32_t nqf, int32_t npair) {
+    const int32_t n[IBH_NCLASS] = {nqf, nq - nqf, npair};
+    return nqf >= 0 ? ibh_class_wgs(n, WPB) : (nq + npair + WPB - 1) / WPB;
+}
+
 struct BlockList { const BlockDesc2* bl; const int32_t *ht, *et, *ls; int32_t count, iters, nwg; };
 BlockList block_list(const ibh_part* p, const int32_t* list, Range r, int wpb, int max_iters) {
     const int32_t count = r.count(), iters = T.sweep_iters > 0 ? T.sweep_iters : std::min(max_iters, std::max(1, count / 6000));
@@ -301,18 +336,21 @@
     const Range rs = s;
     if (rows_second) s.last = s.first;
     const int32_t siters = T.quad_singles_iters > 0 ? T.quad_singles_iters : 1;
-    const int32_t nwgq = (q.count() + npair + WPB - 1) / WPB,
+    const int32_t nqf = rows_inside || p->n_dt > 0 ? -1 : general_quads(p, k, q);
+    const int32_t nwgq = quad_wgs(q.count(), nqf, npair),
                   nwgs = rows_inside ? (s.count() + WPB * 8 - 1) / (WPB * 8) : (s.count() + WPB * siters - 1) / (WPB * siters);
-    auto kq = k_sweep_quad<false, false>;
+    const bool forms = T.quad_one_slot != 0;
+    auto kq = QUAD_KERNEL(false, false, false, forms, nqf >= 0);
     if (rows_inside) kq = k_sweep_quad<false, false, false, true>;
-    else if (p->n_dt > 0) kq = k_sweep_quad<true, false>;
-    else if (T.quad_variant == QV_STAMPS) kq = k_sweep_quad<false, true>;
+    else if (p->n_dt > 0) kq = forms ? k_sweep_quad<true, false, false, false, true> : k_sweep_quad<true, false>;
+    else if (T.quad_variant == QV_STAMPS) kq = QUAD_KERNEL(false, true, false, forms, nqf >= 0);
     if (nwgq + nwgs > 0)
         hipLaunchKernelGGL(kq, dim3(nwgq + nwgs), dim3(64 * WPB), 0, ibh_stream, a.u, a.C, (uint32_t)a.ldc, a.ud,
                            p->qd[k] + q.first, p->qtab[k] + (size_t)q.first * IBH_QROW, q.count(), nwgq, p->blocks2, p->htab,
                            p->etab, p->dtab, slist + s.first, s.count(), nwgs, T.quad_singles_first, siters,
                            (const float*)nullptr, npair,
-                           T.arith_ids ? p->qaux[k] + (size_t)q.first * IBH_QAUX : (const int32_t*)nullptr);
+                           T.arith_ids ? p->qaux[k] + (size_t)q.first * IBH_QAUX : (const int32_t*)nullptr, nqf,
+                           T.quad_order == 2 ? 1 : 0);
     if (rows_second) {
         const int32_t nw = (rs.count() + 7) / 8, nwgr = (nw + WPBR - 1) / WPBR;
         hipLaunchKernelGGL(k_sweep_rows, dim3(nwgr), dim3(64 * WPBR), 0, ibh_stream, a.u, a.C, (uint32_t)a.ldc, a.ud,
@@ -355,11 +393,12 @@
 void adv2_step_quads(const ibh_part* p, const float* u, float* u_out, const float* C, int64_t ldc, const float* dt_dev) {
     const int32_t npair = T.pairs ? p->npair : 0;
     const int32_t nq = p->nq[0], ns = npair ? p->nqs2 : p->nqs[0];
-    const int32_t nwgq = (nq + npair + WPB - 1) / WPB, nwgs = (ns + WPB - 1) / WPB;
-    hipLaunchKernelGGL((k_sweep_quad<false, false, true>), dim3(nwgq + nwgs), dim3(64 * WPB), 0, ibh_stream, u, C,
+    const int32_t nqf = general_quads(p, 0, Range{0, nq});
+    const int32_t nwgq = quad_wgs(nq, nqf, npair), nwgs = (ns + WPB - 1) / WPB;
+    hipLaunchKernelGGL(QUAD_KERNEL(false, false, true, T.quad_one_slot != 0, nqf >= 0), dim3(nwgq + nwgs), dim3(64 * WPB), 0, ibh_stream, u, C,
                        (uint32_t)ldc, u_out, p->qd[0], p->qtab[0], nq, nwgq, p->blocks2, p->htab, p->etab, p->dtab,
                        npair ? p->qsingles2 : p->qsingles[0], ns, nwgs, T.quad_singles_first, 1, dt_dev, npair,
-                       T.arith_ids ? p->qaux[0] : (const int32_t*)nullptr);
+                       T.arith_ids ? p->qaux[0] : (const int32_t*)nullptr, nqf, T.quad_order == 2 ? 1 : 0);
 }
 
 int debug_buffer2d(unsigned long long* buf) {
@@ -370,6 +409,17 @@
 }
 
 extern "C" {
+
+int ibh_quad_wg_map(const int32_t* n, int32_t* cls, int32_t* pos, int32_t cap, int32_t* nwg) {
+    IBH_REQUIRE(n && cls && pos && nwg && cap >= 0 && n[0] >= 0 && n[1] >= 0 && n[2] >= 0, "ibh_quad_wg_map: bad argument");
+    *nwg = ibh_class_wgs(n, WPB);
+    for (int32_t wg = 0; wg < *nwg && wg < cap; ++wg) {
+        const IbhClassWg w = ibh_class_remap(wg, n, WPB);
+        cls[wg] = w.cls;
+        pos[wg] = w.pos;
+    }
+    return 0;
+}
 
 int ibh_step_advection_xgmi(ibh_part* p, float* u, const float* C, int64_t ldc, float* ud, const int32_t* send_all,
                             int n_send_peers, const int32_t* send_seg, float* const* dst0, float* const* dst1,
@@ -413,7 +463,9 @@
     const int32_t nq = p->nq[1], nqi = p->nq_int[1], ns = p->nqs[1], nsi = p->nqs_int[1];
     const int32_t nwg = (nqi + WPB - 1) / WPB + (nsi + WPB - 1) / WPB + (nq - nqi + WPB - 1) / WPB + (ns - nsi + WPB - 1) / WPB;
     static_assert(WPB == 4, "the exchange workgroups of k_step_quad are 256 threads");
-    hipLaunchKernelGGL(p->n_dt > 0 ? k_step_quad<true> : k_step_quad<false>, dim3(E + nwg), dim3(64 * WPB), 0, ibh_stream, u, C,
+    auto ks = p->n_dt > 0 ? (T.quad_one_slot ? k_step_quad<true, true> : k_step_quad<true>)
+                          : (T.quad_one_slot ? k_step_quad<false, true> : k_step_quad<false>);
+    hipLaunchKernelGGL(ks, dim3(E + nwg), dim3(64 * WPB), 0, ibh_stream, u, C,
                        (uint32_t)ldc, ud, p->qd[1], p->qtab[1], nqi, nq, p->blocks2, p->htab, p->etab, p->dtab, p->qsingles[1],
                        nsi, ns, send_all, recv_all, src0, src1, A, state, max_spins, E, fstate);
     IBH_LAUNCH_CHECK();
diff --git a/immersedboundary.jl_amd/csrc/ibh_fused_int.h b/immersedboundary.jl_amd/csrc/ibh_fused_int.h
--- a/immersedboundary.jl_amd/csrc/ibh_fused_int.h
+++ b/immersedboundary.jl_amd/csrc/ibh_fused_int.h
@@ -26,6 +26,8 @@
     int quad_singles_first = env_int("IBH_SINGLES_FIRST", 0);
     int pairs = env_int("IBH_PAIRS", 1);
     int arith_ids = env_int("IBH_ARITH_IDS", 1);
+    int quad_one_slot = env_int("IBH_QUAD_ONE_SLOT", 0);
+    int quad_order = env_int("IBH_QUAD_ORDER", 0);
     int transport_blocks = 1;
     int rows_singles = env_int("IBH_ROWS_SINGLES", -1);
 };
diff --git a/immersedboundary.jl_amd/csrc/ibh_quad2d.h b/immersedboundary.jl_amd/csrc/ibh_quad2d.h
--- a/immersedboundary.jl_amd/csrc/ibh_quad2d.h
+++ b/immersedboundary.jl_amd/csrc/ibh_quad2d.h
@@ -68,6 +68,23 @@
     const v2f B = Df * (s - 0.5f * d);
     const v2f CA = Cf * A;
     return v2f{fmaf(fabsf(Cf.x), B.x, CA.x), fmaf(fabsf(Cf.y), B.y, CA.y)};
+}
+
+__device__ __forceinline__ float flux_w1(float ua, float ub, float Sa, float Sb, float Da, float Db, float Ca, float Cb, float wa) {
+    const float d = ub - ua;
+    const float gu = fmaf(-d, wa, Sa);
+    const float Du = fmaf(-d, 1.0f - wa, Sb);
+    const float s = __builtin_amdgcn_fmed3f(Du, gu, 0.0f);
+    const float dS = Sa - Sb;
+    const float t16 = dS * 0.0625f;
+    const float uf = fmaf(dS, 0.0625f, fmaf(d, wa, ua));
+    const float mu = fmaf(d, 0.5f - wa, -t16);
+    const float Df = max3(Da, Db, 1e-7f);
+    const float A = fmaf(Df, mu, uf);
+    const float Cf = fmaf(Cb - Ca, wa, Ca);
+    const float B = Df * fmaf(d, -0.5f, s);
+    const float CA = Cf * A;
+    return fmaf(fabsf(Cf), B, CA);
 }
 
 __device__ __forceinline__ float jst(float g, float a, float rh) {
@@ -220,6 +237,7 @@
     O.CY = *(const v4f_g*)((const char*)(C + ldc) + b4 + G.a0off4);
     return O;
 }
+template <bool ONE = false>
 __device__ __forceinline__ QuadHalo quad_load_halo_paired(const QuadLane& G, const QuadTab& T, const float* __restrict__ u,
                                                           const float* __restrict__ C, uint32_t ldc) {
     using blk2::ldg;
@@ -227,6 +245,18 @@
     auto pair = [](const float* p, int i) { return *(const v2f_g*)((const char*)p + ((size_t)(uint32_t)i << 2)); };
     QuadHalo H;
     const float* Cn = C + (G.dny ? ldc : 0u);
+    if constexpr (ONE) {
+        const v2f PA = pair(u, T.hid.x - (int)G.g0);
+        const v2f PB = pair(u, T.hid.x + G.offB);
+        const v2f PC = pair(Cn, T.hid.x);
+        H.eu = ldg(u, T.eid);
+        const float hu = G.g0 ? PA.y : PA.x;
+        const float hd = G.g0 ? PA.x : (G.g3 ? PA.y : PB.x);
+        H.hu = v2f{hu, hu};
+        H.hd = v2f{hd, hd};
+        H.hc = v2f{PC.x, PC.x};
+        return H;
+    }
     const bool isF = T.ty == SIDE_FINE;
     const v2f PA = pair(u, T.hid.x - (int)G.g0);
     const v2f PB = pair(u, (G.lr ? T.hid.y : T.hid.x) + G.offB);
@@ -246,7 +276,7 @@
     return H;
 }
 
-template <bool STAMP, bool STEP = false, bool HALF = false>
+template <bool STAMP, bool STEP = false, bool HALF = false, bool ONE = false>
 __device__ __forceinline__ void quad_compute(const QuadLane& G, const QuadTab& T, const QuadOwn& O, const QuadHalo& H,
                                              float* __restrict__ ud, unsigned long long* stamps, float dt = 0.0f) {
     using blk2::wave_lds_sync;
@@ -262,7 +292,7 @@
     const int lane = G.lane;
     const float sgn = G.sgn;
     const uint32_t ty = T.ty;
-    const bool isC = ty == SIDE_COARSE, isF = ty == SIDE_FINE;
+    const bool isC = ty == SIDE_COARSE, isF = !ONE && ty == SIDE_FINE;
     const float qs = isC ? (1.0f / 3.0f) : isF ? (2.0f / 3.0f) : 0.5f;
     const float irt = isC ? 0.5f : isF ? 2.0f : 1.0f;
     const float rhx = T.d.rh[0], rhy = T.d.rh[1];
@@ -277,8 +307,8 @@
     const float m0 = lds_read(G.p_b);
     const float m1r = lds_read(G.p_b1);
     const float m1 = isC ? m1r : m0;
-    const float hm = 0.5f * (hu.x + hu.y);
-    const float fix = 0.5f * (fabsf(hu.x - m0) + fabsf(hu.y - m0)) - fabsf(hm - m0);
+    const float hm = ONE ? hu.x : 0.5f * (hu.x + hu.y);
+    const float fix = ONE ? 0.0f : 0.5f * (fabsf(hu.x - m0) + fabsf(hu.y - m0)) - fabsf(hm - m0);
     *G.p_hm = hm;
     G.p_ringw[0] = fix;
     G.p_ringw[64] = qs;
@@ -308,8 +338,8 @@
 #pragma unroll
         for (int c = 0; c < 4; ++c) {
             float ax = fabsf(dR[c]) + fabsf(dL[c]);
-            if (c == 0) ax += fx0;
-            if (c == 3) ax += fx3;
+            if (!ONE && c == 0) ax += fx0;
+            if (!ONE && c == 3) ax += fx3;
             const float ay = (fabsf(dT[c]) + fabsf(dB[c])) + rF[c];
             D[c] = jst_max2(gx[c], ax, rhx, gy[c], ay, rhy);
         }
@@ -318,7 +348,24 @@
     *(v4f*)(p_own + 2 * QUAD_TILE) = D;
 
     v2f Shn, Dh;
-    {
+    if constexpr (ONE) {
+        const float ihn = (dny ? rhy : rhx) * irt, iht = (dny ? rhx : rhy) * irt;
+        const float h0 = hu.x;
+        const float dm0 = m0 - h0, dm1 = m1 - h0, dde = hd.x - h0;
+        const float din = 0.5f * (dm0 + dm1);
+        const float S1 = fmaf(0.5f, dde, -((1.0f - qs) * din));
+        const v2f Lp = *(const v2f*)(isC ? G.p_LbC : G.p_LbS);
+        const v2f Hp = *(const v2f*)((isC ? G.p_LbC + 2 : G.p_LbS) + 4);
+        const float e0 = Lp.x - h0, e1 = Lp.y - h0, e2 = Hp.x - h0, e3 = Hp.y - h0;
+        const float gn = (dm0 + dm1) + (dde + dde);
+        const float gt = (e0 + e1) + (e2 + e3);
+        const float hn = 0.5f * ihn, ht = 0.5f * iht;
+        const float an = (fabsf(dm0) + fabsf(dm1)) + 2.0f * fabsf(dde);
+        const float at = (fabsf(e0) + fabsf(e1)) + (fabsf(e2) + fabsf(e3));
+        const float D1 = jst_max2(gn, an, hn, gt, at, ht);
+        Shn = v2f{S1, S1};
+        Dh = v2f{D1, D1};
+    } else {
         const float ihn = (dny ? rhy : rhx) * irt, iht = (dny ? rhx : rhy) * irt;
         const v2f dm0 = m0 - hu, dm1 = m1 - hu, dde = hd - hu;
         const v2f din = 0.5f * (dm0 + dm1);
@@ -366,8 +413,12 @@
                     Co_bt = lds_read(G.p_b + 3 * QUAD_TILE);
         const float So = lr ? So_lr : So_bt;
         const float Co = lr ? Co_lr : Co_bt;
-        const v2f F = flux_w2(m0, hu, sgn * So, Shn, Do, Dh, sgn * Co, sgn * hc, qs);
-        edge = sgn * (0.5f * (F.x + F.y));
+        if constexpr (ONE) {
+            edge = sgn * flux_w1(m0, hu.x, sgn * So, Shn.x, Do, Dh.x, sgn * Co, sgn * hc.x, qs);
+        } else {
+            const v2f F = flux_w2(m0, hu, sgn * So, Shn, Do, Dh, sgn * Co, sgn * hc, qs);
+            edge = sgn * (0.5f * (F.x + F.y));
+        }
     }
     *G.p_exw = edge;
     wave_lds_sync();
@@ -392,7 +443,7 @@
     }
 }
 
-template <bool STAMP, bool STEP = false, bool HALF = false>
+template <bool STAMP, bool STEP = false, bool HALF = false, bool FORMS = false>
 __device__ __forceinline__ void sweep_quad(const QuadDesc2* __restrict__ qd, const int32_t* __restrict__ qtab, int32_t q,
                                            const float* __restrict__ u, const float* __restrict__ C, uint32_t ldc,
                                            float* __restrict__ ud, float* lds, int lane,
@@ -401,6 +452,13 @@
     const QuadLane G = quad_lane<HALF>(lds, lane);
     const QuadTab T = quad_load_tab(qd, qtab, q, lane, qaux);
     const QuadOwn O = quad_load_own(G, T, u, C, ldc);
+    if constexpr (FORMS) {
+        if (quad_no_fine(T.d.cls)) {
+            const QuadHalo H = quad_load_halo_paired<true>(G, T, u, C, ldc);
+            quad_compute<STAMP, STEP, HALF, true>(G, T, O, H, ud, stamps, dt);
+            return;
+        }
+    }
     const QuadHalo H = quad_load_halo_paired(G, T, u, C, ldc);
     quad_compute<STAMP, STEP, HALF>(G, T, O, H, ud, stamps, dt);
 }
diff --git a/immersedboundary.jl_amd/hostview.py b/immersedboundary.jl_amd/hostview.py
--- a/immersedboundary.jl_amd/hostview.py
+++ b/immersedboundary.jl_amd/hostview.py
@@ -55,6 +55,8 @@
             out[f"quads_{name}"] = dict(desc=get(QUAD_DESC, QUAD_DTYPE, k), tab=get(QUAD_TAB, np.int32, k).reshape(-1, 160),
                                         singles=get(SINGLES, np.int32, k), n_interior=int(cnt[2]),
                                         n_singles_interior=int(cnt[4]),
+                                        ordered=bool(cnt[8]), n_fine_interior=int(cnt[9]), n_fine_boundary=int(cnt[10]),
+                                        n_pair_fine=int(cnt[11]),
                                         pair_desc=get(PAIR_DESC, QUAD_DTYPE, k),
                                         pair_tab=get(PAIR_TAB, np.int32, k).reshape(-1, 160),
                                         singles2=get(SINGLES2, np.int32, k),
diff --git a/include/ibhip.h b/include/ibhip.h
--- a/include/ibhip.h
+++ b/include/ibhip.h
@@ -95,6 +95,7 @@
                       int32_t n_image, const int32_t* image_in_domain, const int32_t* domain, int index_base);
 int ibh_host2d_get(const ibh_host2d* h, int what, int set, void* dst, int64_t cap_bytes, int64_t* nbytes);
 int ibh_host2d_destroy(ibh_host2d* h);
+int ibh_quad_wg_map(const int32_t* n, int32_t* cls, int32_t* pos, int32_t cap, int32_t* nwg);
 
 int ibh_at_owners(const ibh_part*, int dim, const float* u, int nv, int64_t ldu, float* out, int64_t ldo);
 int ibh_at_neighbors(const ibh_part*, int dim, const float* u, int nv, int64_t ldu, float* out, int64_t ldo);
```
